# BharathMasetty/DPG-SLAM

Hardware: AMD Instinct MI355X
Metric: ICP edges/sec + ms/GN-iter on 5k-node/20k-edge synthetic graph, 1->8 GPU (higher is better)
Workload: dtype fp32 (ICP) + fp64 (GN)

## Files before the change

dpg-slam_amd/csrc/dpg_chol.hip:

```cpp
#include "dpg_chol_dev.h"

using namespace dpg_chol;

namespace {
void take_sym(CholDev* c, dpg_chol_sym* S) {
    c->has_factor = false;
    if (c->track && c->sym_is_fac) {
        std::swap(c->fac_sym, c->sym);
        c->fac_G.swap(c->plan.cur_G);
        c->sym_is_fac = false;
    }
    std::swap(c->sym, *S);
}

int chol_upload(CholDev* c) {
    const dpg_chol_sym& S = c->sym;
    const CholPlan& H = c->plan;
    const int64_t n = H.n;
    ++c->build_gen;
    c->has_factor = false;
    auto al = [](size_t b) { return (b + 255) & ~size_t(255); };
    struct Piece { void** d; const void* h; size_t bytes; };
    Piece pieces[24];
    int np = 0;
// ... 212 lines not shown
    int64_t* gat = reinterpret_cast<int64_t*>(c->pstage.p + keep_bytes);
    int64_t* sca = gat + 4 * nruns;
    for (int64_t r = 0, off = 0; r < nruns; ++r) {
        const int64_t* q = K.runs.data() + 4 * r;
        const int64_t g4[4] = {q[0], off, q[2], q[3]}, s4[4] = {off, q[1], q[2], q[3]};
        std::copy(g4, g4 + 4, gat + 4 * r);
        std::copy(s4, s4 + 4, sca + 4 * r);
        off += q[2];
    }
    if (c->pev.ensure(hipEventDisableTiming)) return DPG_ERR_HIP;
    if (hipMemcpyAsync(c->dpart.p, c->pstage.p, bytes, hipMemcpyHostToDevice, st) != hipSuccess ||
        hipEventRecord(c->pev.e, st) != hipSuccess)
        return DPG_ERR_HIP;
    c->pev_set = true;
    const uint8_t* keep_dev = reinterpret_cast<const uint8_t*>(c->dpart.p);
    const int64_t* gat_dev = reinterpret_cast<const int64_t*>(c->dpart.p + keep_bytes);
    launch_copy_runs(c, st, gat_dev, gat_dev + 4 * nruns, nruns, K.max_run);
    if (hipMemsetAsync(c->status.p, 0, sizeof(int32_t), st) != hipSuccess ||
        hipMemsetAsync(c->sync.p, 0, P.sync_bytes, st) != hipSuccess)
        return DPG_ERR_HIP;
    launch_factor(c, st, hb, nullptr, keep_dev);
    launch_backward(c, st, nullptr, nullptr, nullptr, nullptr, nullptr);
    note_factored(c, ns - K.kept, K.kept, K.moved, (int64_t)((now_ms() - t_pick) * 1e6));
    c->inv_valid = false;
    return hipGetLastError() == hipSuccess ? DPG_OK : DPG_ERR_HIP;
}

extern "C" int dpg_chol_resolve(void* h, const double* hb, void* stream) {
    CholDev* c = reinterpret_cast<CholDev*>(h);
    hipStream_t st = reinterpret_cast<hipStream_t>(stream);
    if (hipMemsetAsync(c->sync.p, 0, c->plan.sync_bytes, st) != hipSuccess) return DPG_ERR_HIP;
    const double* di = c->plan.use_dinv ? c->dinv.p : nullptr;
    const double* li = c->inv_valid ? c->linv.p : nullptr;
    launch_forward(c, st, hb, di, nullptr, li);
    launch_backward(c, st, di, nullptr, nullptr, nullptr, li);
    return hipGetLastError() == hipSuccess ? DPG_OK : DPG_ERR_HIP;
}

extern "C" int dpg_chol_gated_ok(void* h) {
    const CholDev* c = reinterpret_cast<const CholDev*>(h);
    return c && c->plan.fused && !(c->plan.use_dinv && c->plan.n_dblocks > 0) ? 1 : 0;
}

extern "C" void dpg_chol_sync_dev(void* h, int32_t** sync, int64_t* n_words) {
    CholDev* c = reinterpret_cast<CholDev*>(h);
    *sync = c->sync.p;
    *n_words = (int64_t)(c->plan.sync_bytes / sizeof(int32_t));
}

extern "C" int dpg_chol_solve_gated(void* h, const double* hb, const int32_t* gate, int prezeroed, double* X,
                                    double* max_out, void* stream) {
    CholDev* c = reinterpret_cast<CholDev*>(h);
    if (!dpg_chol_gated_ok(h)) return DPG_ERR_STATE;
    c->fac_valid = false;
    c->has_factor = true;
    hipStream_t st = reinterpret_cast<hipStream_t>(stream);
    if (!prezeroed && (hipMemsetAsync(c->status.p, 0, sizeof(int32_t), st) != hipSuccess ||
                       hipMemsetAsync(c->sync.p, 0, c->plan.sync_bytes, st) != hipSuccess))
        return DPG_ERR_HIP;
    const bool inv = c->plan.n_inv_tasks > 0;
    if (inv) {
        if (!c->aux.s) {
            if (hipStreamCreateWithFlags(&c->aux.s, hipStreamNonBlocking) != hipSuccess ||
                c->ev_fac.ensure(hipEventDisableTiming) || c->ev_inv[0].ensure(hipEventDisableTiming) ||
                c->ev_inv[1].ensure(hipEventDisableTiming) || hipEventRecord(c->ev_inv[0].e, c->aux.s) != hipSuccess ||
                hipEventRecord(c->ev_inv[1].e, c->aux.s) != hipSuccess)
                return DPG_ERR_HIP;
        }
        if (hipStreamWaitEvent(st, c->ev_inv[c->inv_par ^ 1].e, 0) != hipSuccess) return DPG_ERR_HIP;
    }
    launch_factor(c, st, hb, gate, nullptr);
    if (inv) {
        if (hipEventRecord(c->ev_fac.e, st) != hipSuccess || hipStreamWaitEvent(c->aux.s, c->ev_fac.e, 0) != hipSuccess)
            return DPG_ERR_HIP;
        launch_inv(c, c->aux.s, gate);
        if (hipEventRecord(c->ev_inv[c->inv_par].e, c->aux.s) != hipSuccess) return DPG_ERR_HIP;
        c->inv_par ^= 1;
    }
    launch_forward(c, st, hb, nullptr, gate, c->linv.p);
    launch_backward(c, st, nullptr, gate, X, max_out, c->linv.p);
    return hipGetLastError() == hipSuccess ? DPG_OK : DPG_ERR_HIP;
}

extern "C" void dpg_chol_keep_inverse(void* h, int on) {
    if (h) reinterpret_cast<CholDev*>(h)->keep_inv = on != 0;
}

extern "C" int dpg_chol_join_aux(void* h, void* stream) {
    CholDev* c = reinterpret_cast<CholDev*>(h);
    if (!c || !c->aux.s) return DPG_OK;
    return hipStreamWaitEvent(reinterpret_cast<hipStream_t>(stream), c->ev_inv[c->inv_par ^ 1].e, 0) == hipSuccess ? DPG_OK
                                                                                                       : DPG_ERR_HIP;
}

extern "C" const int32_t* dpg_chol_pos_dev(void* h) { return reinterpret_cast<CholDev*>(h)->pos; }
extern "C" const double* dpg_chol_x_dev(void* h) { return reinterpret_cast<CholDev*>(h)->xsol.p; }
extern "C" const int32_t* dpg_chol_status_dev(void* h) { return reinterpret_cast<CholDev*>(h)->status.p; }
extern "C" void dpg_chol_stats(void* h, double out[6]) {
    const dpg_chol_sym& S = reinterpret_cast<CholDev*>(h)->sym;
    out[0] = S.ns;
    out[1] = S.n_levels;
    out[2] = S.max_front;
    out[3] = S.flops;
    out[4] = (double)S.front_off[(size_t)S.ns] * 8.0;
    out[5] = (double)S.n;
}

#ifdef DPG_CHOL_TIMING
extern "C" void dpg_chol_tree(void* h, int32_t* parent, int32_t* m3, int32_t* k3) {
    const dpg_chol_sym& S = reinterpret_cast<CholDev*>(h)->sym;
    for (int32_t s = 0; s < S.ns; ++s) {
        parent[s] = S.sn_parent[(size_t)s];
        k3[s] = 3 * (S.sn_c0[(size_t)s + 1] - S.sn_c0[(size_t)s]);
        m3[s] = k3[s] + 3 * (int32_t)(S.sn_rows_ptr[(size_t)s + 1] - S.sn_rows_ptr[(size_t)s]);
    }
}
#endif
```

dpg-slam_amd/csrc/dpg_ctx.h:

```cpp
#ifndef DPG_CTX_H
#define DPG_CTX_H

#include <hip/hip_runtime.h>
#include <rccl/rccl.h>
#include <string.h>
#include <time.h>

#include <algorithm>
#include <atomic>
#include <condition_variable>
#include <deque>
#include <memory>
#include <mutex>
#include <thread>
#include <unordered_map>
#include <utility>
#include <vector>

#include "../../include/dpg_slam_c.h"
#include "dpg_buf.h"
#include "dpg_chol.h"
#include "dpg_gn_pipe.h"
#include "dpg_internal.h"

// ... 6 lines not shown
        hipError_t _e = (expr);                                                              \
        if (_e != hipSuccess) return fail(DPG_ERR_HIP, "%s: %s", #expr, hipGetErrorString(_e)); \
    } while (0)

inline double now_ms() {
    struct timespec ts;
    clock_gettime(CLOCK_MONOTONIC, &ts);
    return (double)ts.tv_sec * 1e3 + (double)ts.tv_nsec * 1e-6;
}

template <typename T>
T or_default(const T* p, void (*def)(T*)) {
    T v;
    if (p) v = *p;
    else def(&v);
    return v;
}

struct DevMem {
    typedef hipStream_t stream_t;
    static int alloc(void** p, size_t bytes) { return hipMalloc(p, bytes) != hipSuccess; }
    static void free(void* p) { (void)hipFree(p); }
    static int copy(void* dst, const void* src, size_t bytes, hipStream_t s) {
        return hipMemcpyAsync(dst, src, bytes, hipMemcpyDeviceToDevice, s) != hipSuccess ||
               hipStreamSynchronize(s) != hipSuccess;
    }
};
struct PinMem {
    typedef hipStream_t stream_t;
    static int alloc(void** p, size_t bytes) { return hipHostMalloc(p, bytes, hipHostMallocDefault) != hipSuccess; }
    static void free(void* p) { (void)hipHostFree(p); }
    static int copy(void* dst, const void* src, size_t bytes, hipStream_t) {
        memcpy(dst, src, bytes);
        return 0;
    }
};
struct MappedMem : PinMem {
    static int alloc(void** p, size_t bytes) { return hipHostMalloc(p, bytes, hipHostMallocMapped | hipHostMallocCoherent) != hipSuccess; }
};
template <typename T>
using DevBuf = OwnedBuf<T, DevMem>;
template <typename T>
using PinBuf = OwnedBuf<T, PinMem>;
template <typename T>
using MappedBuf = OwnedBuf<T, MappedMem>;

struct DevEvent {
    hipEvent_t e = nullptr;
    DevEvent() = default;
    DevEvent(const DevEvent&) = delete;
    DevEvent& operator=(const DevEvent&) = delete;
    DevEvent(DevEvent&& o) noexcept : e(o.e) { o.e = nullptr; }
    DevEvent& operator=(DevEvent&& o) noexcept {
        std::swap(e, o.e);
        return *this;
    }
    ~DevEvent() {
        if (e) (void)hipEventDestroy(e);
    }
    int ensure(unsigned flags) { return e || hipEventCreateWithFlags(&e, flags) == hipSuccess ? 0 : -1; }
};
struct DevStream {
    hipStream_t s = nullptr;
    DevStream() = default;
    DevStream(const DevStream&) = delete;
    DevStream& operator=(const DevStream&) = delete;
    ~DevStream() { release(); }
    void release() {
        if (s) (void)hipStreamDestroy(s);
        s = nullptr;
    }
};
struct CholDestroy { void operator()(void* h) const { dpg_chol_destroy(h); } };
typedef std::unique_ptr<void, CholDestroy> CholPtr;

struct GnGraph {
    dpg_gn_dev v{};
    DevBuf<dpg_factor> factors;
    DevBuf<int32_t> up_cptr, up_clist, rowptr, colidx, src_up;
    DevBuf<double> bsr, minv, poses, x, r, z, p0, p1, q, partials, scal, hb_own, scal3;
    PinBuf<double> scal3_host;
    DevBuf<uint8_t> mine;
    DevBuf<double> hb_part;
    CholPtr chol;
    int build(int64_t n_nodes, const dpg_factor* factors, int64_t n_factors, int64_t shard_begin, int64_t shard_end,
              const dpg_chol_opts* opts, hipStream_t sync_stream);
};

struct dpg_ctx {
    int device = 0;
    DevStream own;
    hipStream_t stream = nullptr;
    DevStream aux;
    DevEvent ev[8];
    bool cov_pending = false, cov_on_aux = false;
    int32_t icp_variant = DPG_ICP_ANGULAR;
    int32_t defer_cap = 256;
    int32_t cov_wg = 256;
    int32_t kernel_variant = 0;
    float map_ms = 0.f;
    DevEvent map_ev[2];
    DevBuf<float> full, ds;
    DevBuf<int64_t> ds_off_dev;
    DevBuf<int64_t> full_off_dev;
    DevBuf<float> tree_pts;
    DevBuf<uint16_t> tree_idx;
    DevBuf<uint16_t> buckets;
    DevBuf<unsigned char> icp_scratch;
    std::vector<int64_t> full_off, ds_off;
    int64_t n_nodes = 0;
    int64_t idx_valid = 0;
    int32_t ratio = 1;
    int32_t max_ds = 0;
    std::vector<dpg_icp_edge> h_edges;
    DevBuf<dpg_icp_edge> edges;
    DevBuf<dpg_icp_result> res;
    DevBuf<double> hess;
    DevBuf<int32_t> trace;
    int64_t n_edges = 0;
    int32_t max_src = 0, max_tgt = 0;
    int32_t trace_iters = 0;
    dpg_icp_kparams kp{};
    bool have_cov = false;
    DevBuf<float> s_pts;
    DevBuf<dpg_icp_edge> s_edge;
    DevBuf<dpg_icp_result> s_res;
    DevBuf<double> s_hess;
    DevBuf<int64_t> s_off;
    DevBuf<float> s_tree_pts;
    DevBuf<uint16_t> s_tree_idx;
    DevBuf<uint16_t> s_buckets;
    GnGraph gn;
    bool gn_ready = false;
    dpg_gn_params gp{};
    float asm_ms = 0.f, solve_ms = 0.f;
    std::vector<uint64_t> gn_pairs;
    bool gn_pairs_valid = false;
    DevBuf<dpg_gn_ctl> pipe_ctl;
    MappedBuf<dpg_gn_slot> pipe_slot;
    uint32_t pipe_loop = 0;
    std::vector<dpg_ctx*> peers;
    std::vector<std::pair<void*, void (*)(void*)>> children;
    std::vector<ncclComm_t> comms;
    dpg_coll_ops host_ops{};
    std::vector<double> host_hb;
    struct HostColl;
    std::unique_ptr<HostColl> hc;
    int32_t coll = 0;
    int32_t world = 1, rank0 = 0;
    int32_t rank = 0;
    std::vector<dpg_icp_edge> batch;
    std::vector<int32_t> batch_owner;
    std::vector<std::vector<int64_t>> shard;
    bool batch_measured = false;
    int32_t batch_runs = 0;
    int32_t schedule = DPG_ICP_SCHEDULE_MEASURED;
    std::unordered_map<uint64_t, float> cost;
    DevBuf<int32_t> shard_idx;
    DevBuf<float> cost_dev;
    dpg_chol_opts copts;
    DevBuf<dpg_csm_pair> csm_pairs;
    DevBuf<float> csm_rot;
    DevBuf<int32_t> csm_stencil;
    DevBuf<dpg_csm_result> csm_res;
    DevBuf<int32_t> csm_diag;
    DevEvent csm_ev[2];
    bool csm_timed = false;
};

struct dpg_ctx::HostColl {
    PinBuf<double> buf;
    MappedBuf<uint32_t> flag;
    DevEvent ev[2];
    uint32_t next_tag = 0;
    std::thread th;
    std::mutex mu;
    std::condition_variable cv;
    std::deque<std::pair<uint32_t, hipEvent_t>> jobs;
    size_t count = 0;
    uint64_t posted = 0, done = 0;
    bool stop = false;
    std::atomic<int> failed{0};
    static int create(const dpg_ctx* c, std::unique_ptr<HostColl>& out);
    ~HostColl();
};

enum { kCollNone = 0, kCollRccl = 1, kCollVirtual = 2, kCollHost = 3, kMaxVirtual = 16 };
inline int n_dev(const dpg_ctx* c) { return 1 + (int)c->peers.size(); }
inline bool is_rank_form(const dpg_ctx* c) {
    return (c->coll == kCollRccl || c->coll == kCollHost) && c->peers.empty() && c->world > 1;
}
inline dpg_ctx* dev_ctx(dpg_ctx* c, int k) { return k == 0 ? c : c->peers[(size_t)k - 1]; }
inline bool is_multi(const dpg_ctx* c) { return c->coll != kCollNone; }
inline int join_cov(dpg_ctx* c) {
    if (!c->cov_pending) return DPG_OK;
    c->cov_pending = false;
    return hipStreamWaitEvent(c->stream, c->ev[2].e, 0) == hipSuccess ? DPG_OK : DPG_ERR_HIP;
}

extern dpg_ctx* g_default_ctx;
void scans_truncate(dpg_ctx* c, int64_t V);
int icp_batch_run_from(dpg_ctx* c, int64_t tree_from);
int batch_fetch(dpg_ctx* c, dpg_icp_result* results, double* hess, bool learn);
int gn_loop(dpg_ctx* c, const dpg_gn_params& P, double* poses, double t0, double t1, dpg_gn_stats* st);

#pragma GCC visibility pop

#endif
```

dpg-slam_amd/csrc/dpg_ctx.hip:

```cpp

#include <stdarg.h>
#include <stdio.h>
#include <string.h>

#include <string>

#include "dpg_ctx.h"

namespace {
thread_local std::string g_err;
}

int fail(int code, const char* fmt, ...) {
    char buf[512];
    va_list ap;
    va_start(ap, fmt);
    vsnprintf(buf, sizeof(buf), fmt, ap);
    va_end(ap);
    g_err = buf;
    return code;
}

dpg_ctx* g_default_ctx = nullptr;

// ... 203 lines not shown
    if (!c || !o || o->order < DPG_ORDER_AUTO || o->order > DPG_ORDER_ND || o->max_supernode_cols < 1 || o->solve_inv_cols < 0 ||
        !(o->relax_fraction >= 0.0))
        return fail(DPG_ERR_ARG, "bad solver options");
    for (int k = 0; k < n_dev(c); ++k) {
        dpg_chol_opts& d = dev_ctx(c, k)->copts;
        d.order = o->order;
        d.fused = o->fused ? 1 : 0;
        d.solve_stage = o->solve_stage;
        d.solve_maxseg = o->solve_maxseg;
        d.solve_dinv = o->solve_dinv ? 1 : 0;
        d.merge_single = o->merge_single ? 1 : 0;
        d.max_supernode_cols = o->max_supernode_cols;
        d.relax_fraction = o->relax_fraction;
        d.solve_inv_cols = o->solve_inv_cols;
    }
    return DPG_OK;
}

int dpg_ctx_set_icp_schedule(dpg_ctx* c, int32_t schedule) {
    if (!c || (schedule != DPG_ICP_SCHEDULE_CALLER && schedule != DPG_ICP_SCHEDULE_MEASURED))
        return fail(DPG_ERR_ARG, "bad ICP schedule");
    c->schedule = schedule;
    return DPG_OK;
}

int dpg_ctx_set_icp_variant(dpg_ctx* c, int32_t variant) {
    if (!c || (variant != DPG_ICP_ANGULAR && variant != DPG_ICP_KDTREE && variant != DPG_ICP_GRID))
        return fail(DPG_ERR_ARG, "bad ICP variant");
    for (int k = 0; k < n_dev(c); ++k) {
        if (dev_ctx(c, k)->icp_variant != variant) dev_ctx(c, k)->idx_valid = 0;
        dev_ctx(c, k)->icp_variant = variant;
    }
    return DPG_OK;
}

int dpg_ctx_set_icp_defer_cap(dpg_ctx* c, int32_t cap) {
    if (!c || cap < 0) return fail(DPG_ERR_ARG, "bad defer cap");
    for (int k = 0; k < n_dev(c); ++k) dev_ctx(c, k)->defer_cap = cap;
    return DPG_OK;
}

int dpg_ctx_set_cov_workgroups(dpg_ctx* c, int32_t n) {
    if (!c || n < 0) return fail(DPG_ERR_ARG, "bad covariance workgroup count");
    for (int k = 0; k < n_dev(c); ++k) dev_ctx(c, k)->cov_wg = n;
    return DPG_OK;
}

int dpg_ctx_set_icp_kernel_variant(dpg_ctx* c, int32_t v) {
    if (!c || v < 0) return fail(DPG_ERR_ARG, "bad kernel variant");
    for (int k = 0; k < n_dev(c); ++k) {
        if ((dev_ctx(c, k)->kernel_variant == 2) != (v == 2)) dev_ctx(c, k)->idx_valid = 0;
        dev_ctx(c, k)->kernel_variant = v;
    }
    return DPG_OK;
}

void dpg_ctx_adopt(dpg_ctx* c, void* child, void (*destroy)(void*)) {
    if (c && child) c->children.emplace_back(child, destroy);
}
void dpg_ctx_release_child(dpg_ctx* c, void* child) {
    if (!c) return;
    for (size_t k = 0; k < c->children.size(); ++k)
        if (c->children[k].first == child) {
            c->children.erase(c->children.begin() + (std::ptrdiff_t)k);
            return;
        }
}

void dpg_ctx_destroy(dpg_ctx* c) {
    if (!c) return;
    while (!c->children.empty()) {
        const auto ch = c->children.back();
        ch.second(ch.first);
        if (!c->children.empty() && c->children.back().first == ch.first) c->children.pop_back();
    }
    if (c->coll == kCollVirtual) (void)hipStreamSynchronize(c->stream);
    for (dpg_ctx* q : c->peers) dpg_ctx_destroy(q);
    c->peers.clear();
    for (ncclComm_t m : c->comms)
        if (m) (void)ncclCommDestroy(m);
    c->comms.clear();
    (void)hipSetDevice(c->device);
    (void)join_cov(c);
    (void)hipStreamSynchronize(c->stream);
    c->hc.reset();
    if (c == g_default_ctx) g_default_ctx = nullptr;
    delete c;
}

int dpg_ctx_set_stream(dpg_ctx* c, void* s) {
    if (!c) return fail(DPG_ERR_ARG, "ctx is NULL");
    if (join_cov(c)) return fail(DPG_ERR_HIP, "stream wait failed");
    HIP_TRY(hipStreamSynchronize(c->stream));
    c->own.release();
    c->stream = reinterpret_cast<hipStream_t>(s);
    if (c->coll == kCollVirtual)
        for (dpg_ctx* q : c->peers) q->stream = c->stream;
    return DPG_OK;
}

int dpg_ctx_synchronize(dpg_ctx* c) {
    if (!c) return fail(DPG_ERR_ARG, "ctx is NULL");
    for (int k = 0; k < n_dev(c); ++k) {
        HIP_TRY(hipSetDevice(dev_ctx(c, k)->device));
        if (join_cov(dev_ctx(c, k))) return fail(DPG_ERR_HIP, "stream wait failed");
        HIP_TRY(hipStreamSynchronize(dev_ctx(c, k)->stream));
    }
    HIP_TRY(hipSetDevice(c->device));
    return DPG_OK;
}

}
```

dpg-slam_amd/csrc/dpg_gn.hip:

```cpp

#include <hip/hip_runtime.h>
#include <math.h>
#include <stdint.h>
#include <stdlib.h>
#include <string.h>

#include <algorithm>
#include <future>
#include <vector>

#include "dpg_ctx.h"

namespace {

constexpr int kRowThreads = 256;

__device__ __forceinline__ void between_lin(const double* a, const double* b, double h[4], double H1[9]) {
    const double c1 = cos(a[2]), s1 = sin(a[2]), c2 = cos(b[2]), s2 = sin(b[2]);
    const double c = c1 * c2 + s1 * s2, s = -s1 * c2 + c1 * s2;
    const double dx = b[0] - a[0], dy = b[1] - a[1];
    h[0] = c1 * dx + s1 * dy;
    h[1] = -s1 * dx + c1 * dy;
    h[2] = c;
    h[3] = s;
// ... 279 lines not shown
            const double* B = bsr + 9 * (int64_t)s;
            acc[0] += B[0] * pc[0] + B[1] * pc[1] + B[2] * pc[2];
            acc[1] += B[3] * pc[0] + B[4] * pc[1] + B[5] * pc[2];
            acc[2] += B[6] * pc[0] + B[7] * pc[1] + B[8] * pc[2];
        }
#pragma unroll
        for (int k = 0; k < 3; ++k) {
            const double pv = it > 0 ? z[3 * v + k] + beta * p_old[3 * v + k] : p_old[3 * v + k];
            p_new[3 * v + k] = pv;
            q[3 * v + k] = acc[k];
            pq += pv * acc[k];
        }
    }
    pq = block_sum(pq, red);
    if (threadIdx.x == 0) part_pq[blockIdx.x] = pq;
}

__global__ void pcg_update_kernel(int it, int64_t n, const double* __restrict__ minv,
                                  const double* __restrict__ p, const double* __restrict__ q,
                                  double* __restrict__ x, double* __restrict__ r, double* __restrict__ z,
                                  const double* __restrict__ part_rz_in, const double* __restrict__ part_pq,
                                  double* __restrict__ part_rz_out, double* __restrict__ part_rr, int nb) {
    __shared__ double red[16];
    const double rz = sum_partials(part_rz_in, nb);
    const double pq = sum_partials(part_pq, nb);
    const double alpha = pq != 0.0 ? rz / pq : 0.0;
    const int64_t v = (int64_t)blockIdx.x * blockDim.x + threadIdx.x;
    double rz_n = 0.0, rr = 0.0;
    if (v < n) {
        double rv[3], zv[3];
#pragma unroll
        for (int k = 0; k < 3; ++k) {
            x[3 * v + k] += alpha * p[3 * v + k];
            rv[k] = r[3 * v + k] - alpha * q[3 * v + k];
            r[3 * v + k] = rv[k];
        }
        mv3(minv + 9 * v, rv, zv);
#pragma unroll
        for (int k = 0; k < 3; ++k) {
            z[3 * v + k] = zv[k];
            rz_n += rv[k] * zv[k];
            rr += rv[k] * rv[k];
        }
    }
    rz_n = block_sum(rz_n, red);
    rr = block_sum(rr, red);
    if (threadIdx.x == 0) { part_rz_out[blockIdx.x] = rz_n; part_rr[blockIdx.x] = rr; }
}

__global__ void retract_kernel(double* __restrict__ X, const double* __restrict__ d, int64_t n,
                               const int32_t* __restrict__ pos, double* __restrict__ max_out, const int32_t* gate) {
    if (gate && !gate[0]) return;
    const int64_t v = (int64_t)blockIdx.x * blockDim.x + threadIdx.x;
    double m = 0.0;
    if (v < n) {
        const int64_t di = 3 * (int64_t)(pos ? pos[v] : v);
        m = pose_retract(X + 3 * v, d[di], d[di + 1], d[di + 2]);
    }
#pragma unroll
    for (int off = 32; off >= 1; off >>= 1) m = fmax(m, __shfl_down(m, off, 64));
    if ((threadIdx.x & 63) == 0)
        atomicMax(reinterpret_cast<unsigned long long*>(max_out), (unsigned long long)__double_as_longlong(m));
}

__global__ void scalars_kernel(const double* __restrict__ chi2, const int32_t* __restrict__ status,
                               double* __restrict__ scal3) {
    scal3[1] = *chi2;
    scal3[2] = status ? (double)*status : 0.0;
}

__device__ __forceinline__ void icp_factor_write(dpg_factor& f, const dpg_icp_result& r, int64_t e, int64_t n_always,
                                                 double ix, double iy, double ith) {
    const bool keep = e < n_always || (r.converged && r.status == DPG_ICP_OK);
    f.z[0] = r.z[0];
    f.z[1] = r.z[1];
    f.z[2] = r.z[2];
    f.info[0] = keep ? ix : 0.0;
    f.info[1] = keep ? iy : 0.0;
    f.info[2] = keep ? ith : 0.0;
}

__global__ void icp_to_factor_kernel(const dpg_icp_result* __restrict__ res, dpg_factor* __restrict__ F,
                                     int64_t first, int64_t count, int64_t n_always, double ix, double iy,
                                     double ith) {
    const int64_t e = (int64_t)blockIdx.x * blockDim.x + threadIdx.x;
    if (e >= count) return;
    dpg_factor& f = F[first + e];
    const dpg_icp_result r = res[e];
    icp_factor_write(f, r, e, n_always, ix, iy, ith);
}

template <typename B, typename T>
int take(B& b, T*& view, size_t n) {
    const int rc = b.reserve(n);
    view = b.p;
    return rc;
}

template <typename T>
int up(T* dst, const std::vector<T>& src) {
    if (src.empty()) return 0;
    return hipMemcpy(dst, src.data(), src.size() * sizeof(T), hipMemcpyHostToDevice) == hipSuccess ? 0 : DPG_ERR_HIP;
}

inline unsigned nblk(int64_t n) { return (unsigned)((n + kRowThreads - 1) / kRowThreads); }

}

extern "C" int64_t dpg_gn_dev_vote_offset(const dpg_gn_dev* g) { return 9 * g->nnzb_upper + 3 * g->n_nodes + 2; }
extern "C" int64_t dpg_gn_dev_hb_size(const dpg_gn_dev* g) { return dpg_gn_dev_vote_offset(g) + g->n_vote; }

int GnGraph::build(int64_t n, const dpg_factor* F, int64_t nf, int64_t shard_begin, int64_t shard_end,
                   const dpg_chol_opts* opts, hipStream_t sync_stream) {
    dpg_gn_dev* g = &v;
    if (n <= 0 || nf < 0 || n > (int64_t)1 << 28) return DPG_ERR_ARG;
    const double t0 = now_ms();
    std::vector<uint64_t> fkey((size_t)nf, ~0ull);
    std::vector<uint64_t> pk;
    pk.reserve((size_t)nf);
    for (int64_t k = 0; k < nf; ++k) {
        const dpg_factor& f = F[k];
        if (f.kind == DPG_FACTOR_PRIOR) {
            if (f.i < 0 || f.i >= n) return DPG_ERR_ARG;
            continue;
        }
        if (f.kind != DPG_FACTOR_BETWEEN || f.i < 0 || f.j < 0 || f.i >= n || f.j >= n || f.i == f.j)
            return DPG_ERR_ARG;
        fkey[(size_t)k] = (uint64_t)std::min(f.i, f.j) << 32 | (uint64_t)std::max(f.i, f.j);
        pk.push_back(fkey[(size_t)k]);
    }
    const size_t n_between = pk.size();
    std::sort(pk.begin(), pk.end());
    pk.erase(std::unique(pk.begin(), pk.end()), pk.end());
    const int64_t P = (int64_t)pk.size();
    const int64_t nu = n + P;
    std::vector<int32_t> plo((size_t)P), phi((size_t)P);
    for (int64_t p = 0; p < P; ++p) { plo[(size_t)p] = (int32_t)(pk[(size_t)p] >> 32); phi[(size_t)p] = (int32_t)(pk[(size_t)p] & 0xffffffffu); }
    const dpg_chol_opts copt = opts ? *opts : dpg_chol_opts{};
    double sym_ms = 0.0;
    std::future<void*> sym_job = std::async(std::launch::async, [&]() -> void* {
        const double ts = now_ms();
        void* ch = nullptr;
        dpg_chol_opts o = copt;
        dpg_chol_sym S;
        if (dpg_chol_symbolic(n, plo.data(), phi.data(), P, &o, &S) ||
            dpg_chol_create_sym_plan(&ch, n, plo.data(), phi.data(), P, &S, &o))
            ch = nullptr;
        sym_ms = now_ms() - ts;
        return ch;
    });
    std::vector<int32_t> fpair((size_t)nf, -1);
    for (int64_t k = 0; k < nf; ++k)
        if (fkey[(size_t)k] != ~0ull)
            fpair[(size_t)k] = (int32_t)(std::lower_bound(pk.begin(), pk.end(), fkey[(size_t)k]) - pk.begin());
    std::vector<int32_t> cptr((size_t)nu + 1), clist((size_t)nf + 2 * n_between);
    dpg_contribution_lists(F, nf, n, fpair.data(), P, cptr.data(), clist.data());
    std::vector<int32_t> rowptr((size_t)n + 1, 0);
    for (int64_t v = 0; v < n; ++v) rowptr[(size_t)v + 1] = 1;
    for (uint64_t key : pk) { rowptr[(size_t)(key >> 32) + 1]++; rowptr[(size_t)(key & 0xffffffffu) + 1]++; }
    for (int64_t v = 0; v < n; ++v) rowptr[(size_t)v + 1] += rowptr[(size_t)v];
    std::vector<int32_t> colidx((size_t)rowptr[(size_t)n]), srcup((size_t)rowptr[(size_t)n]);
    {
        std::vector<int32_t> at(rowptr.begin(), rowptr.end() - 1);
        for (int64_t p = 0; p < P; ++p) {
            const int32_t lo = (int32_t)(pk[(size_t)p] >> 32), hi = (int32_t)(pk[(size_t)p] & 0xffffffffu);
            colidx[(size_t)at[(size_t)hi]] = lo;
            srcup[(size_t)at[(size_t)hi]++] = (int32_t)(-1 - (n + p));
        }
        for (int64_t v = 0; v < n; ++v) {
            colidx[(size_t)at[(size_t)v]] = (int32_t)v;
            srcup[(size_t)at[(size_t)v]++] = (int32_t)v;
        }
        for (int64_t p = 0; p < P; ++p) {
            const int32_t lo = (int32_t)(pk[(size_t)p] >> 32), hi = (int32_t)(pk[(size_t)p] & 0xffffffffu);
            colidx[(size_t)at[(size_t)lo]] = hi;
            srcup[(size_t)at[(size_t)lo]++] = (int32_t)(n + p);
        }
    }
    const double t1 = now_ms();
    CholPtr ch(sym_job.get());
    const double t2 = now_ms();
    if (sync_stream && hipStreamSynchronize(sync_stream) != hipSuccess) return DPG_ERR_HIP;
    g->n_nodes = n;
    g->n_factors = nf;
    g->nnzb_upper = nu;
    g->nnzb_full = (int64_t)colidx.size();
    g->shard_begin = shard_begin < 0 ? 0 : shard_begin;
    g->shard_end = shard_end > nf ? nf : shard_end;
    g->n_blocks_rows = (int32_t)nblk(n);
    int rc = 0;
    rc |= take(factors, g->factors, std::max<size_t>((size_t)nf, 1));
    rc |= take(up_cptr, g->up_cptr, cptr.size());
    rc |= take(up_clist, g->up_clist, std::max<size_t>(clist.size(), 1));
    rc |= take(this->rowptr, g->rowptr, rowptr.size());
    rc |= take(this->colidx, g->colidx, colidx.size());
    rc |= take(src_up, g->src_up, srcup.size());
    rc |= take(bsr, g->bsr, 9 * colidx.size());
    rc |= take(minv, g->minv, 9 * (size_t)n);
    rc |= take(poses, g->poses, 3 * (size_t)n);
    rc |= take(x, g->x, 3 * (size_t)n);
    rc |= take(r, g->r, 3 * (size_t)n);
    rc |= take(z, g->z, 3 * (size_t)n);
    rc |= take(p0, g->p0, 3 * (size_t)n);
    rc |= take(p1, g->p1, 3 * (size_t)n);
    rc |= take(q, g->q, 3 * (size_t)n);
    rc |= take(partials, g->partials, 6 * (size_t)g->n_blocks_rows + (size_t)n);
    rc |= take(scal, g->scal, 2 * (size_t)65536);
    rc |= take(hb_own, g->hb_own, (size_t)dpg_gn_dev_hb_size(g));
    rc |= take(scal3, g->scal3, 4);
    rc |= take(scal3_host, g->scal3_host, 4);
    if (!rc && nf && hipMemcpy(g->factors, F, (size_t)nf * sizeof(dpg_factor), hipMemcpyHostToDevice) != hipSuccess) rc = -1;
    if (!rc)
        rc = up(g->up_cptr, cptr) | up(g->up_clist, clist) | up(g->rowptr, rowptr) | up(g->colidx, colidx) |
             up(g->src_up, srcup);
    if (rc) { *this = GnGraph(); return DPG_ERR_HIP; }
    g->chol = ch.release();
    if (g->chol && dpg_chol_create_sym_upload(&g->chol)) g->chol = nullptr;
    chol.reset(g->chol);
    if (g->chol) dpg_chol_keep_inverse(g->chol, 1);
    const double t3 = now_ms();
    double bt[2] = {0.0, 0.0};
    if (g->chol) dpg_chol_build_times(g->chol, bt);
    g->setup_ms[0] = t1 - t0;
    g->setup_ms[1] = std::max(0.0, sym_ms - bt[0]);
    g->setup_ms[2] = bt[0];
    g->setup_ms[3] = std::max(0.0, (t3 - t2) - bt[1]);
    g->setup_ms[4] = bt[1];
    return DPG_OK;
}

extern "C" int dpg_gn_dev_icp_to_factors(dpg_gn_dev* g, const dpg_icp_result* res, int64_t first, int64_t count,
                                         int64_t n_always, double ix, double iy, double ith, void* stream) {
    if (count <= 0) return DPG_OK;
    if (first < 0 || first + count > g->n_factors) return DPG_ERR_ARG;
    hipLaunchKernelGGL(icp_to_factor_kernel, dim3(nblk(count)), dim3(kRowThreads), 0,
                       reinterpret_cast<hipStream_t>(stream), res, g->factors, first, count, n_always, ix, iy, ith);
    return hipGetLastError() == hipSuccess ? DPG_OK : DPG_ERR_HIP;
}

static int assemble_gated(dpg_gn_dev* g, double* hb, hipStream_t s, const int32_t* gate, bool chi2 = true) {
    double* chi2_node = g->partials + 6 * (size_t)g->n_blocks_rows;
    const int64_t ng = lg_groups(g->n_nodes, g->nnzb_upper);
    if (ng > 0)
        hipLaunchKernelGGL(lin_gather_kernel, dim3((unsigned)ng), dim3(kLgLanes), 0, s, g->factors, g->poses, g->up_cptr,
                           g->up_clist, g->n_nodes, g->nnzb_upper, g->shard_begin, g->shard_end, g->mine, hb, chi2_node, gate);
    if (chi2) {
        const bool vote = hb == g->hb_part && g->n_vote > 0;
        hipLaunchKernelGGL(chi2_kernel, dim3(1), dim3(1024), 0, s, chi2_node, g->n_nodes,
                           hb + 9 * g->nnzb_upper + 3 * g->n_nodes, gate, vote ? hb + dpg_gn_dev_vote_offset(g) : nullptr,
                           g->scal3, vote && g->chol ? dpg_chol_status_dev(g->chol) : nullptr, g->world, g->rank);
    }
    return hipGetLastError() == hipSuccess ? DPG_OK : DPG_ERR_HIP;
}

extern "C" int dpg_gn_dev_assemble(dpg_gn_dev* g, double* hb, void* stream) {
    return assemble_gated(g, hb, reinterpret_cast<hipStream_t>(stream), nullptr);
}

__global__ void own_kernel(uint8_t* __restrict__ mine, int64_t nf, int32_t world, int32_t rank) {
    const int64_t f = (int64_t)blockIdx.x * blockDim.x + threadIdx.x;
    if (f < nf) mine[f] = (f % world) == rank ? 1 : 0;
}

__global__ void icp_to_factor_scatter_kernel(const dpg_icp_result* __restrict__ res, const int32_t* __restrict__ idx,
                                             dpg_factor* __restrict__ F, uint8_t* __restrict__ mine, int64_t first,
                                             int64_t n_local, int64_t n_always, double ix, double iy, double ith) {
    const int64_t j = (int64_t)blockIdx.x * blockDim.x + threadIdx.x;
    if (j >= n_local) return;
    const int64_t e = idx[j];
    dpg_factor& f = F[first + e];
    const dpg_icp_result r = res[j];
    icp_factor_write(f, r, e, n_always, ix, iy, ith);
    mine[first + e] = 1;
}

struct VsumArgs {
    const double* parts[16];
    double* outs[16];
};
__global__ void vsum_kernel(VsumArgs a, int32_t k, int64_t n) {
    for (int64_t i = (int64_t)blockIdx.x * blockDim.x + threadIdx.x; i < n; i += (int64_t)gridDim.x * blockDim.x) {
        double s = a.parts[0][i];
        for (int32_t q = 1; q < k; ++q) s += a.parts[q][i];
        for (int32_t q = 0; q < k; ++q) a.outs[q][i] = s;
    }
}

extern "C" int dpg_gn_dev_set_ownership(GnGraph* o, int32_t world, int32_t rank, void* stream) {
    if (world < 1 || rank < 0 || rank >= world) return DPG_ERR_ARG;
    dpg_gn_dev* g = &o->v;
    hipStream_t s = reinterpret_cast<hipStream_t>(stream);
    const int32_t nv = world > 1 ? 2 * world : 0;
    if (nv != g->n_vote) {
        if (hipStreamSynchronize(s) != hipSuccess) return DPG_ERR_HIP;
        o->hb_own.release();
        o->hb_part.release();
        g->hb_part = nullptr;
        g->n_vote = nv;
        if (take(o->hb_own, g->hb_own, (size_t)dpg_gn_dev_hb_size(g))) return DPG_ERR_HIP;
    }
    if (!o->mine.p && take(o->mine, g->mine, std::max<size_t>((size_t)g->n_factors, 1))) return DPG_ERR_HIP;
    if (!o->hb_part.p && take(o->hb_part, g->hb_part, (size_t)dpg_gn_dev_hb_size(g))) return DPG_ERR_HIP;
    if (hipMemsetAsync(g->hb_part, 0, sizeof(double) * (size_t)dpg_gn_dev_hb_size(g), s) != hipSuccess) return DPG_ERR_HIP;
    g->world = world;
    g->rank = rank;
    if (g->n_factors > 0)
        hipLaunchKernelGGL(own_kernel, dim3(nblk(g->n_factors)), dim3(kRowThreads), 0, reinterpret_cast<hipStream_t>(stream),
                           g->mine, g->n_factors, world, rank);
    return hipGetLastError() == hipSuccess ? DPG_OK : DPG_ERR_HIP;
}

extern "C" int dpg_gn_dev_icp_to_factors_scatter(dpg_gn_dev* g, const dpg_icp_result* res, const int32_t* idx,
                                                 int64_t n_local, int64_t first, int64_t count, int64_t n_always,
                                                 double ix, double iy, double ith, void* stream) {
    if (!g->mine || first < 0 || count < n_local || first + count > g->n_factors) return DPG_ERR_ARG;
    hipStream_t s = reinterpret_cast<hipStream_t>(stream);
    if (count > 0 && hipMemsetAsync(g->mine + first, 0, (size_t)count, s) != hipSuccess) return DPG_ERR_HIP;
    if (n_local > 0)
        hipLaunchKernelGGL(icp_to_factor_scatter_kernel, dim3(nblk(n_local)), dim3(kRowThreads), 0, s, res, idx, g->factors,
                           g->mine, first, n_local, n_always, ix, iy, ith);
    return hipGetLastError() == hipSuccess ? DPG_OK : DPG_ERR_HIP;
}

extern "C" int dpg_gn_dev_assemble_part(dpg_gn_dev* g, const int32_t* gate, void* stream) {
    if (!g->hb_part) return DPG_ERR_STATE;
    return assemble_gated(g, g->hb_part, reinterpret_cast<hipStream_t>(stream), gate, true);
}

extern "C" int dpg_launch_vsum(const double* const* parts, double* const* outs, int32_t k, int64_t n, void* stream) {
    if (k < 1 || k > 16 || n <= 0) return k >= 1 && k <= 16 ? DPG_OK : DPG_ERR_ARG;
    VsumArgs a;
    for (int q = 0; q < 16; ++q) {
        a.parts[q] = q < k ? parts[q] : nullptr;
        a.outs[q] = q < k ? outs[q] : nullptr;
    }
    const unsigned blocks = (unsigned)std::min<int64_t>((n + 1023) / 1024, 2048);
    hipLaunchKernelGGL(vsum_kernel, dim3(blocks), dim3(1024), 0, reinterpret_cast<hipStream_t>(stream), a, k, n);
    return hipGetLastError() == hipSuccess ? DPG_OK : DPG_ERR_HIP;
}

static int pcg_solve(dpg_gn_dev* g, const double* hb, const dpg_gn_params* gp, hipStream_t s);

extern "C" int dpg_gn_dev_solve_async(dpg_gn_dev* g, const double* hb, const dpg_gn_params* gp, void* stream) {
    hipStream_t s = reinterpret_cast<hipStream_t>(stream);
    const double* xout = g->x;
    const int32_t* xpos = nullptr;
    g->last_pcg_iters = 0;
    g->last_used_chol = gp->linear_solver == DPG_SOLVER_CHOLESKY && g->chol;
    if (g->last_used_chol) {
        const bool slow = g->last_was_chord && g->last_delta_inf > 0.1 * g->prev_delta_inf;
        const bool reuse = gp->reuse_factorization && g->have_factor && g->last_delta_inf < gp->refactor_delta && !slow;
        g->last_was_chord = reuse ? 1 : 0;
        const int rc = reuse ? dpg_chol_resolve(g->chol, hb, stream) : dpg_chol_solve(g->chol, hb, stream);
        if (rc) return rc;
        if (!reuse) {
            g->have_factor = 1;
            ++g->n_factorizations;
        }
        xout = dpg_chol_x_dev(g->chol);
        xpos = dpg_chol_pos_dev(g->chol);
    } else {
        const int it = pcg_solve(g, hb, gp, s);
        if (it < 0) return DPG_ERR_HIP;
        g->last_pcg_iters = it;
    }
    if (hipMemsetAsync(g->scal3, 0, sizeof(double), s) != hipSuccess) return DPG_ERR_HIP;
    hipLaunchKernelGGL(retract_kernel, dim3(g->n_blocks_rows), dim3(kRowThreads), 0, s, g->poses, xout, g->n_nodes,
                       xpos, g->scal3, nullptr);
    return hipGetLastError() == hipSuccess ? DPG_OK : DPG_ERR_HIP;
}

__device__ __forceinline__ void clear_sync(int32_t* sync, int64_t n_words, int32_t* status) {
    int4* s4 = reinterpret_cast<int4*>(sync);
    for (int64_t k = threadIdx.x; k < n_words / 4; k += blockDim.x) s4[k] = make_int4(0, 0, 0, 0);
    if (threadIdx.x == 0) *status = 0;
}

__device__ __forceinline__ void sys_st64(void* p, uint64_t v) {
    __hip_atomic_store(reinterpret_cast<uint64_t*>(p), v, __ATOMIC_RELAXED, __HIP_MEMORY_SCOPE_SYSTEM);
}
static_assert(offsetof(dpg_gn_slot, reuse) == 24 && offsetof(dpg_gn_slot, active) == 28 &&
              offsetof(dpg_gn_slot, final_) == 32 && offsetof(dpg_gn_slot, it) == 36 && offsetof(dpg_gn_slot, tag) == 40,
              "post_slot stores the int pairs as 8-byte words");
__device__ __forceinline__ void post_slot(dpg_gn_slot* slot, const dpg_gn_slot& o, uint64_t tag) {
    sys_st64(&slot->dinf, (uint64_t)__double_as_longlong(o.dinf));
    sys_st64(&slot->error, (uint64_t)__double_as_longlong(o.error));
    sys_st64(&slot->status, (uint64_t)__double_as_longlong(o.status));
    sys_st64(&slot->reuse, (uint64_t)(uint32_t)o.reuse | (uint64_t)(uint32_t)o.active << 32);
    sys_st64(&slot->final_, (uint64_t)(uint32_t)o.final_ | (uint64_t)(uint32_t)o.it << 32);
    asm volatile("s_waitcnt vmcnt(0)" ::: "memory");
    sys_st64(&slot->tag, tag);
}

__global__ void pipe_init_kernel(dpg_gn_ctl* ctl, int32_t reuse, int32_t last_was_chord, int32_t have_factor,
                                 double last_dinf, double prev_dinf, const double* cur_dev, dpg_gn_slot* init,
                                 double* max_out, int32_t* sync, int64_t n_words, int32_t* status, uint32_t loop) {
    clear_sync(sync, n_words, status);
    if (threadIdx.x != 0) return;
    const double cur = *cur_dev;
    {
        dpg_gn_slot o{};
        o.error = cur;
        post_slot(init, o, (uint64_t)loop << 32);
    }
    ctl->loop = loop;
    ctl->active = !(cur <= 0.0) ? 1 : 0;
    ctl->reuse = reuse;
    ctl->last_was_chord = last_was_chord;
    ctl->have_factor = have_factor;
    ctl->it = 0;
    ctl->last_dinf = last_dinf;
    ctl->prev_dinf = prev_dinf;
    ctl->cur_error = cur;
    *max_out = 0.0;
}

__global__ __launch_bounds__(1024) void pipe_ctl_kernel(dpg_gn_ctl* ctl, const double* __restrict__ chi2_node, int64_t n,
                                                        double* chi2, const double* chi2_sum, int32_t* status,
                                                        double* max_out, dpg_gn_params P, dpg_gn_slot* slot,
                                                        int32_t* sync, int64_t n_words, const double* __restrict__ vote,
                                                        int32_t world) {
    __shared__ double red[16];
    if (!ctl->active) return;
    double sum = 0.0;
    if (chi2_sum) {
        sum = *chi2_sum;
    } else {
        sum = block_sum(strided_sum(chi2_node, n, threadIdx.x, blockDim.x), red);
    }
    const double st_word = (double)*status;
    __syncthreads();
    clear_sync(sync, n_words, status);
    if (threadIdx.x != 0) return;
    *chi2 = sum;
    dpg_gn_slot o;
    o.reuse = ctl->reuse;
    o.active = ctl->active;
    o.it = ctl->it;
    o.final_ = 1;
    o.dinf = 0.0;
    o.error = 0.0;
    o.status = 0.0;
    if (ctl->active) {
        double dinf = *max_out, st = st_word;
        if (vote) {
            const unsigned long long d0 = (unsigned long long)__double_as_longlong(vote[0]);
            bool diverged = false;
            dinf = vote[0];
            st = vote[world];
            for (int32_t r = 1; r < world; ++r) {
                diverged |= (unsigned long long)__double_as_longlong(vote[r]) != d0;
                dinf = fmax(dinf, vote[r]);
                st = fmax(st, vote[world + r]);
            }
            if (diverged) st = (double)DPG_GN_STATUS_DIVERGED;
        }
        const double nw = sum;
        const int it = ctl->it + 1;
        o.dinf = dinf;
        o.error = nw;
        o.status = st;
        o.it = it;
        bool fin = st != 0.0 || it >= P.max_iterations;
        if (!fin) {
            const double cur = ctl->cur_error;
            if (P.use_error_criteria) {
                bool conv = nw <= 0.0;
                if (!conv) {
                    const double abs_dec = cur - nw, rel_dec = abs_dec / cur;
                    conv = (P.relative_error_tol != 0.0 && rel_dec <= P.relative_error_tol) ||
                           abs_dec <= P.absolute_error_tol;
                }
                fin = conv || !isfinite(cur);
            } else {
                fin = dinf < P.delta_tol;
            }
        }
        o.final_ = fin ? 1 : 0;
        ctl->prev_dinf = ctl->last_dinf;
        ctl->last_dinf = dinf;
        ctl->last_was_chord = ctl->reuse;
        ctl->have_factor = 1;
        ctl->cur_error = nw;
        ctl->it = it;
        const bool slow = ctl->last_was_chord && ctl->last_dinf > 0.1 * ctl->prev_dinf;
        ctl->reuse = (P.reuse_factorization && ctl->have_factor && ctl->last_dinf < P.refactor_delta && !slow) ? 1 : 0;
        ctl->active = fin ? 0 : 1;
        *max_out = 0.0;
    }
    post_slot(slot, o, ((uint64_t)ctl->loop << 32) | (uint32_t)o.it);
}

extern "C" int dpg_gn_pipe_init(dpg_gn_dev* g, const dpg_gn_params* gp, dpg_gn_ctl* ctl, const double* cur_dev,
                                dpg_gn_slot* init, uint32_t loop, void* stream) {
    hipStream_t s = reinterpret_cast<hipStream_t>(stream);
    const bool slow = g->last_was_chord && g->last_delta_inf > 0.1 * g->prev_delta_inf;
    const bool reuse = gp->reuse_factorization && g->have_factor && g->last_delta_inf < gp->refactor_delta && !slow;
    int32_t* sync;
    int64_t n_words;
    dpg_chol_sync_dev(g->chol, &sync, &n_words);
    hipLaunchKernelGGL(pipe_init_kernel, dim3(1), dim3(1024), 0, s, ctl, reuse ? 1 : 0, g->last_was_chord, g->have_factor,
                       g->last_delta_inf, g->prev_delta_inf, cur_dev, init, g->scal3, sync, n_words,
                       const_cast<int32_t*>(dpg_chol_status_dev(g->chol)), loop);
    return hipGetLastError() == hipSuccess ? DPG_OK : DPG_ERR_HIP;
}

extern "C" int dpg_gn_pipe_issue_solve(dpg_gn_dev* g, dpg_gn_ctl* ctl, int part, void* stream) {
    hipStream_t s = reinterpret_cast<hipStream_t>(stream);
    const int32_t* gate = &ctl->active;
    if (!g->chol || !dpg_chol_gated_ok(g->chol) || (part && !g->hb_part)) return DPG_ERR_STATE;
    int rc = dpg_chol_solve_gated(g->chol, g->hb_own, gate, 1, g->poses, g->scal3, stream);
    if (rc) return rc;
    return part ? assemble_gated(g, g->hb_part, s, gate, true) : assemble_gated(g, g->hb_own, s, gate, false);
}

extern "C" int dpg_gn_pipe_issue_ctl(dpg_gn_dev* g, const dpg_gn_params* gp, dpg_gn_ctl* ctl, dpg_gn_slot* slot,
                                     int part, void* stream) {
    hipStream_t s = reinterpret_cast<hipStream_t>(stream);
    int32_t* sync;
    int64_t n_words;
    if (dpg_chol_join_aux(g->chol, stream)) return DPG_ERR_HIP;
    dpg_chol_sync_dev(g->chol, &sync, &n_words);
    double* chi2 = g->hb_own + 9 * g->nnzb_upper + 3 * g->n_nodes;
    hipLaunchKernelGGL(pipe_ctl_kernel, dim3(1), dim3(1024), 0, s, ctl, g->partials + 6 * (size_t)g->n_blocks_rows,
                       g->n_nodes, chi2, part ? chi2 : nullptr, const_cast<int32_t*>(dpg_chol_status_dev(g->chol)),
                       g->scal3, *gp, slot, sync, n_words,
                       part && g->n_vote > 0 ? g->hb_own + dpg_gn_dev_vote_offset(g) : nullptr, g->world);
    return hipGetLastError() == hipSuccess ? DPG_OK : DPG_ERR_HIP;
}

extern "C" int dpg_gn_pipe_issue(dpg_gn_dev* g, const dpg_gn_params* gp, dpg_gn_ctl* ctl, dpg_gn_slot* slot,
                                 void* stream) {
    const int rc = dpg_gn_pipe_issue_solve(g, ctl, 0, stream);
    return rc ? rc : dpg_gn_pipe_issue_ctl(g, gp, ctl, slot, 0, stream);
}

extern "C" int dpg_gn_dev_fetch(dpg_gn_dev* g, const double* hb, void* stream, double out[3]) {
    hipStream_t s = reinterpret_cast<hipStream_t>(stream);
    const bool chol = g->chol != nullptr && g->last_used_chol;
    hipLaunchKernelGGL(scalars_kernel, dim3(1), dim3(1), 0, s, hb + 9 * g->nnzb_upper + 3 * g->n_nodes,
                       chol ? dpg_chol_status_dev(g->chol) : nullptr, g->scal3);
    if (hipMemcpyAsync(g->scal3_host, g->scal3, 3 * sizeof(double), hipMemcpyDeviceToHost, s) != hipSuccess ||
        hipStreamSynchronize(s) != hipSuccess)
        return DPG_ERR_HIP;
    out[0] = g->scal3_host[0];
    out[1] = g->scal3_host[1];
    out[2] = g->scal3_host[2];
    g->prev_delta_inf = g->last_delta_inf;
    g->last_delta_inf = out[0];
    return DPG_OK;
}

extern "C" int dpg_gn_dev_solve(dpg_gn_dev* g, const double* hb, const dpg_gn_params* gp, void* stream,
                                double* delta_inf, double* error, int32_t* pcg_iters) {
    int rc = dpg_gn_dev_solve_async(g, hb, gp, stream);
    if (rc) return rc;
    double sc[3];
    if ((rc = dpg_gn_dev_fetch(g, hb, stream, sc))) return rc;
    if (gp->linear_solver == DPG_SOLVER_CHOLESKY && g->chol && sc[2] != 0.0) return DPG_ERR_NUMERIC;
    if (delta_inf) *delta_inf = sc[0];
    if (error) *error = sc[1];
    if (pcg_iters) *pcg_iters = g->last_pcg_iters;
    return DPG_OK;
}

static int pcg_solve(dpg_gn_dev* g, const double* hb, const dpg_gn_params* gp, hipStream_t s) {
    const int nb = g->n_blocks_rows;
    const int64_t n = g->n_nodes;
    double* part_rz_a = g->partials;
    double* part_rz_b = g->partials + nb;
    double* part_rr = g->partials + 2 * (size_t)nb;
    double* part_pq = g->partials + 3 * (size_t)nb;
    hipLaunchKernelGGL(pcg_init_kernel, dim3(nb), dim3(kRowThreads), 0, s, hb, g->rowptr, g->src_up, n, g->nnzb_upper,
                       g->bsr, g->minv, g->x, g->r, g->z, g->p0, part_rz_a, part_rr);
    double host_scal[2] = {0, 0};
    double rr0 = -1.0;
    const int check = gp->pcg_check_every > 0 ? gp->pcg_check_every : 16;
    const int max_it = std::min(gp->pcg_max_iterations > 0 ? gp->pcg_max_iterations : 20000, 65535);
    const double tol2 = gp->pcg_rel_tol * gp->pcg_rel_tol;
    int it = 0;
    double* pbuf[2] = {g->p0, g->p1};
    double* rzbuf[2] = {part_rz_a, part_rz_b};
    for (; it < max_it; ++it) {
        double* p_old = pbuf[it & 1];
        double* p_new = pbuf[(it + 1) & 1];
        hipLaunchKernelGGL(pcg_spmv_kernel, dim3(nb), dim3(kRowThreads), 0, s, it, g->bsr, g->rowptr, g->colidx, n,
// ... 33 lines not shown
```

dpg-slam_amd/csrc/dpg_gn_api.hip:

```cpp

#include <string.h>

#include <chrono>
#include <cmath>

#include "dpg_ctx.h"

static int gn_setup_1(dpg_ctx* c, int64_t V, const dpg_factor* F, int64_t nf, int64_t b, int64_t e,
                      const dpg_gn_params* gp) {
    HIP_TRY(hipSetDevice(c->device));
    GnGraph ng;
    int rc = ng.build(V, F, nf, b, e, &c->copts, c->stream);
    if (rc) return fail(rc, "pose-graph setup failed (invalid factor or out of memory)");
    c->gn = std::move(ng);
    c->gn_ready = true;
    c->gn_pairs_valid = false;
    c->gp = or_default(gp, dpg_gn_params_default);
    return DPG_OK;
}

static int gn_set_poses_1(dpg_ctx* c, const double* poses) {
    if (!c->gn_ready) return fail(DPG_ERR_STATE, "graph not set up");
    HIP_TRY(hipSetDevice(c->device));
    HIP_TRY(hipMemcpyAsync(c->gn.v.poses, poses, sizeof(double) * 3 * (size_t)c->gn.v.n_nodes, hipMemcpyHostToDevice,
                           c->stream));
    HIP_TRY(hipStreamSynchronize(c->stream));
    c->gn.v.have_factor = 0;
    c->gn.v.last_delta_inf = 1e300;
    c->gn.v.prev_delta_inf = 1e300;
    c->gn.v.last_was_chord = 0;
    c->gn.v.n_factorizations = 0;
    return DPG_OK;
}

#define DPG_STEP_API_1(c)                                                                                        \
    do {                                                                                                         \
        if (!(c) || !(c)->gn_ready) return fail(DPG_ERR_STATE, "graph not set up");                             \
        if (is_multi(c)) return fail(DPG_ERR_STATE, "the step API is per device: a multi-device context runs "   \
                                                    "dpg_gn_run / dpg_optimize_graph / dpg_reoptimize");         \
    } while (0)

static int solve_retract_async_1(dpg_ctx* c, const double* hb_dev) {
    if (!hb_dev) hb_dev = c->gn.v.hb_own;
    HIP_TRY(hipEventRecord(c->ev[4].e, c->stream));
    int rc = dpg_gn_dev_solve_async(&c->gn.v, hb_dev, &c->gp, c->stream);
    if (rc) return fail(rc, "solve launch failed: %s", hipGetErrorString(hipGetLastError()));
    HIP_TRY(hipEventRecord(c->ev[5].e, c->stream));
    return DPG_OK;
}

static int fetch_1(dpg_ctx* c, const double* hb_dev, double out[3]) {
    if (!hb_dev) hb_dev = c->gn.v.hb_own;
    int rc = dpg_gn_dev_fetch(&c->gn.v, hb_dev, c->stream, out);
    if (rc) return fail(rc, "fetch failed");
    float s = 0.f;
    if (hipEventElapsedTime(&s, c->ev[4].e, c->ev[5].e) == hipSuccess) c->solve_ms = s;
    return DPG_OK;
}

static int read_error(dpg_ctx* c, double* err) {
    HIP_TRY(hipSetDevice(c->device));
    HIP_TRY(hipMemcpyAsync(err, c->gn.v.hb_own + 9 * c->gn.v.nnzb_upper + 3 * c->gn.v.n_nodes, sizeof(double),
                           hipMemcpyDeviceToHost, c->stream));
    HIP_TRY(hipStreamSynchronize(c->stream));
    return DPG_OK;
}

static int check_conv(const dpg_gn_params* gp, double cur, double nw) {
    if (nw <= 0.0) return 1;
    const double abs_dec = cur - nw;
    const double rel_dec = abs_dec / cur;
    return (gp->relative_error_tol != 0.0 && rel_dec <= gp->relative_error_tol) || (abs_dec <= gp->absolute_error_tol);
}

static int coll_sum_hb(dpg_ctx* c) {
    const size_t count = (size_t)dpg_gn_dev_hb_size(&c->gn.v);
    if (c->coll == kCollVirtual) {
        const double* parts[kMaxVirtual];
        double* outs[kMaxVirtual];
        for (int k = 0; k < n_dev(c); ++k) {
            parts[k] = dev_ctx(c, k)->gn.v.hb_part;
            outs[k] = dev_ctx(c, k)->gn.v.hb_own;
        }
        const int rc = dpg_launch_vsum(parts, outs, n_dev(c), (int64_t)count, c->stream);
        return rc ? fail(rc, "virtual all-reduce launch failed") : DPG_OK;
    }
    if (c->coll == kCollHost) {
        c->host_hb.resize(count);
        HIP_TRY(hipSetDevice(c->device));
        HIP_TRY(hipMemcpyAsync(c->host_hb.data(), c->gn.v.hb_part, sizeof(double) * count, hipMemcpyDeviceToHost, c->stream));
        HIP_TRY(hipStreamSynchronize(c->stream));
        if (c->host_ops.allreduce_sum_f64(c->host_ops.user, c->host_hb.data(), (int64_t)count))
            return fail(DPG_ERR_HIP, "the caller's all-reduce of the packed system failed");
        HIP_TRY(hipMemcpyAsync(c->gn.v.hb_own, c->host_hb.data(), sizeof(double) * count, hipMemcpyHostToDevice, c->stream));
        HIP_TRY(hipStreamSynchronize(c->stream));
        return DPG_OK;
    }
    if (ncclGroupStart() != ncclSuccess) return fail(DPG_ERR_HIP, "ncclGroupStart failed");
    for (int k = 0; k < n_dev(c); ++k) {
        dpg_ctx* q = dev_ctx(c, k);
        const ncclResult_t r = ncclAllReduce(q->gn.v.hb_part, q->gn.v.hb_own, count, ncclDouble, ncclSum, c->comms[(size_t)k],
                                             q->stream);
        if (r != ncclSuccess) {
            (void)ncclGroupEnd();
            return fail(DPG_ERR_HIP, "ncclAllReduce failed: %s", ncclGetErrorString(r));
        }
    }
    if (ncclGroupEnd() != ncclSuccess) return fail(DPG_ERR_HIP, "ncclGroupEnd failed");
    return DPG_OK;
}

static void host_coll_thread(dpg_ctx::HostColl* hp, int device, dpg_coll_ops ops) {
    dpg_ctx::HostColl& h = *hp;
    (void)hipSetDevice(device);
    for (;;) {
        std::pair<uint32_t, hipEvent_t> job;
        {
            std::unique_lock<std::mutex> lk(h.mu);
            h.cv.wait(lk, [&] { return h.stop || !h.jobs.empty(); });
            if (h.jobs.empty()) return;
            job = h.jobs.front();
            h.jobs.pop_front();
// ... 13 lines not shown

int dpg_ctx::HostColl::create(const dpg_ctx* c, std::unique_ptr<HostColl>& out) {
    std::unique_ptr<HostColl> h(new HostColl());
    if (h->flag.reserve(2) || h->ev[0].ensure(hipEventDisableTiming) || h->ev[1].ensure(hipEventDisableTiming))
        return fail(DPG_ERR_HIP, "the collective thread's flag words and events could not be created");
    h->flag.p[0] = h->flag.p[1] = 0;
    h->th = std::thread(host_coll_thread, h.get(), c->device, c->host_ops);
    out = std::move(h);
    return DPG_OK;
}

dpg_ctx::HostColl::~HostColl() {
    {
        std::lock_guard<std::mutex> lk(mu);
        stop = true;
    }
    cv.notify_all();
    if (th.joinable()) th.join();
}

static int coll_sum_hb_host_async(dpg_ctx* c) {
    const size_t count = (size_t)dpg_gn_dev_hb_size(&c->gn.v);
    HIP_TRY(hipSetDevice(c->device));
    int rc;
    if (!c->hc && (rc = dpg_ctx::HostColl::create(c, c->hc))) return rc;
    dpg_ctx::HostColl& h = *c->hc;
    if (h.buf.cap < count && h.buf.reserve(count)) return fail(DPG_ERR_HIP, "hipHostMalloc(collective buffer) failed");
    h.count = count;
    const uint32_t tag = ++h.next_tag;
    hipEvent_t ev = h.ev[tag & 1].e;
    HIP_TRY(hipMemcpyAsync(h.buf.p, c->gn.v.hb_part, sizeof(double) * count, hipMemcpyDeviceToHost, c->stream));
    HIP_TRY(hipEventRecord(ev, c->stream));
    {
        std::lock_guard<std::mutex> lk(h.mu);
        h.jobs.emplace_back(tag, ev);
        ++h.posted;
    }
    h.cv.notify_all();
    rc = dpg_launch_host_wait(h.flag.p, tag, h.flag.p + 1, c->stream);
    if (rc) return fail(rc, "host-collective wait launch failed");
    HIP_TRY(hipMemcpyAsync(c->gn.v.hb_own, h.buf.p, sizeof(double) * count, hipMemcpyHostToDevice, c->stream));
    return DPG_OK;
}

static void hc_drain(dpg_ctx* c) {
    if (!c->hc) return;
    std::unique_lock<std::mutex> lk(c->hc->mu);
    c->hc->cv.wait(lk, [&] { return c->hc->done == c->hc->posted; });
}

static int ensure_pipe(dpg_ctx* q) {
    if (q->pipe_slot.p) return DPG_OK;
    HIP_TRY(hipSetDevice(q->device));
    if (q->pipe_ctl.reserve(1) || q->pipe_slot.reserve(3))
        return fail(DPG_ERR_HIP, "GN pipeline: allocating the control block and report slots failed");
    memset(q->pipe_slot.p, 0, 3 * sizeof(dpg_gn_slot));
    return DPG_OK;
}

static int wait_slot(dpg_ctx* q, const dpg_gn_slot* slot, uint64_t tag) {
    const volatile uint64_t* t = &slot->tag;
    auto t0 = std::chrono::steady_clock::now(), last = t0;
    for (unsigned n = 0;; ++n) {
        if (*t == tag) {
            std::atomic_thread_fence(std::memory_order_acquire);
            return DPG_OK;
        }
        if (n < 4096) {
            __builtin_ia32_pause();
            continue;
        }
        std::this_thread::yield();
        const auto now = std::chrono::steady_clock::now();
        if (now - last > std::chrono::milliseconds(2)) {
            last = now;
            const hipError_t e = hipStreamQuery(q->stream);
            if (e != hipSuccess && e != hipErrorNotReady) return fail(DPG_ERR_HIP, "GN pipeline: %s", hipGetErrorString(e));
            if (e == hipSuccess && *t != tag) return fail(DPG_ERR_STATE, "GN pipeline: the stream drained without the report");
            if (now - t0 > std::chrono::seconds(60)) return fail(DPG_ERR_HIP, "GN pipeline: no report after 60 s");
        }
    }
}

static int gn_loop_pipe_body(dpg_ctx* c, const dpg_gn_params& P, dpg_gn_stats& S, double& nw, double& dinf, int& it);
static int gn_loop_pipe(dpg_ctx* c, const dpg_gn_params& P, dpg_gn_stats& S, double& nw, double& dinf, int& it) {
    int rc = gn_loop_pipe_body(c, P, S, nw, dinf, it);
    if (c->coll == kCollHost && c->hc) {
        hc_drain(c);
        if (!rc && c->hc->failed.exchange(0)) rc = fail(DPG_ERR_HIP, "the caller's all-reduce of the packed system failed");
        if (!rc && __atomic_load_n(c->hc->flag.p + 1, __ATOMIC_ACQUIRE))
            rc = fail(DPG_ERR_HIP, "GN pipeline: no all-reduce from the collective thread in 120 s");
    }
    return rc;
}
static int gn_loop_pipe_body(dpg_ctx* c, const dpg_gn_params& P, dpg_gn_stats& S, double& nw, double& dinf, int& it) {
    const int L = n_dev(c);
    const int part = is_multi(c) ? 1 : 0;
    int rc;
    for (int k = 0; k < L; ++k) {
        dpg_ctx* q = dev_ctx(c, k);
        if ((rc = ensure_pipe(q))) return rc;
        ++q->pipe_loop;
        const double* cur_dev = q->gn.v.hb_own + 9 * q->gn.v.nnzb_upper + 3 * q->gn.v.n_nodes;
        if ((rc = dpg_gn_pipe_init(&q->gn.v, &P, q->pipe_ctl.p, cur_dev, q->pipe_slot.p + 2, q->pipe_loop, q->stream)))
            return fail(rc, "GN pipeline launch failed");
    }
    auto issue = [&](int i) -> int {
        int r;
        for (int k = 0; k < L; ++k) {
            dpg_ctx* q = dev_ctx(c, k);
            HIP_TRY(hipSetDevice(q->device));
            if ((r = dpg_gn_pipe_issue_solve(&q->gn.v, q->pipe_ctl.p, part, q->stream)))
                return fail(r, "GN pipeline launch failed: %s", hipGetErrorString(hipGetLastError()));
        }
        if (part && (r = (c->coll == kCollHost ? coll_sum_hb_host_async(c) : coll_sum_hb(c)))) return r;
        for (int k = 0; k < L; ++k) {
            dpg_ctx* q = dev_ctx(c, k);
            HIP_TRY(hipSetDevice(q->device));
            if ((r = dpg_gn_pipe_issue_ctl(&q->gn.v, &P, q->pipe_ctl.p, q->pipe_slot.p + (i & 1), part, q->stream)))
                return fail(r, "GN pipeline launch failed: %s", hipGetErrorString(hipGetLastError()));
        }
        return DPG_OK;
    };
    if ((rc = issue(1))) return rc;
    int issued = 1;
    std::vector<int> nfact((size_t)L, 0), reuse_last((size_t)L, 0);
    for (int k = 0; k < L; ++k) reuse_last[(size_t)k] = dev_ctx(c, k)->gn.v.last_was_chord;
    for (int i = 1;; ++i) {
        if (issued < P.max_iterations) {
            if ((rc = issue(i + 1))) return rc;
            ++issued;
        }
        dpg_gn_slot o0{};
        for (int k = 0; k < L; ++k) {
            dpg_ctx* q = dev_ctx(c, k);
            HIP_TRY(hipSetDevice(q->device));
            if (i == 1) {
                if ((rc = wait_slot(q, q->pipe_slot.p + 2, (uint64_t)q->pipe_loop << 32))) return rc;
                const double e0 = static_cast<const volatile dpg_gn_slot*>(q->pipe_slot.p + 2)->error;
                if (e0 <= 0.0) {
                    for (int j = 0; j < L; ++j) (void)hipStreamSynchronize(dev_ctx(c, j)->stream);
                    S.initial_error = e0;
                    nw = e0;
                    dinf = 0.0;
                    it = 0;
                    HIP_TRY(hipSetDevice(c->device));
                    return DPG_OK;
                }
            }
            if ((rc = wait_slot(q, q->pipe_slot.p + (i & 1), ((uint64_t)q->pipe_loop << 32) | (uint32_t)i))) return rc;
            dpg_gn_slot o;
            {
                const volatile dpg_gn_slot* v = q->pipe_slot.p + (i & 1);
                o.dinf = v->dinf;
                o.error = v->error;
                o.status = v->status;
                o.reuse = v->reuse;
                o.active = v->active;
                o.final_ = v->final_;
                o.it = v->it;
            }
            if (i == 1 && k == 0) S.initial_error = static_cast<const volatile dpg_gn_slot*>(q->pipe_slot.p + 2)->error;
            if (!o.active || o.it != i) return fail(DPG_ERR_STATE, "GN pipeline out of step (device %d, iteration %d)", k, i);
            if (k == 0) {
                o0 = o;
            } else if (memcmp(&o.dinf, &o0.dinf, sizeof(double)) || memcmp(&o.error, &o0.error, sizeof(double)) ||
                       o.status != o0.status || o.reuse != o0.reuse || o.final_ != o0.final_) {
                for (int j = 0; j < L; ++j) (void)hipStreamSynchronize(dev_ctx(c, j)->stream);
                return fail(DPG_ERR_INTERNAL, "devices diverged at GN iteration %d (device %d: |d| %.17g error %.17g, "
                            "device 0: %.17g %.17g)", i, k, o.dinf, o.error, o0.dinf, o0.error);
            }
            if (!o.reuse) ++nfact[(size_t)k];
            q->gn.v.prev_delta_inf = q->gn.v.last_delta_inf;
            q->gn.v.last_delta_inf = o.dinf;
            reuse_last[(size_t)k] = o.reuse;
        }
        if (c->hc && c->hc->failed.load()) {
            for (int j = 0; j < L; ++j) (void)hipStreamSynchronize(dev_ctx(c, j)->stream);
            return fail(DPG_ERR_HIP, "the caller's all-reduce of the packed system failed (GN iteration %d)", i);
        }
        if (o0.status != 0.0) {
            for (int j = 0; j < L; ++j) (void)hipStreamSynchronize(dev_ctx(c, j)->stream);
            if (o0.status == (double)DPG_GN_STATUS_DIVERGED)
                return fail(DPG_ERR_INTERNAL, "ranks diverged at GN iteration %d (different max |delta| in the vote words)", i);
            return fail(DPG_ERR_NUMERIC, "Cholesky failed (status %d)", (int)o0.status);
        }
        it = i;
        dinf = o0.dinf;
        nw = o0.error;
        if (o0.final_) break;
    }
    for (int k = 0; k < L; ++k) {
        dpg_gn_dev* g = &dev_ctx(c, k)->gn.v;
        g->last_was_chord = reuse_last[(size_t)k];
        g->have_factor = 1;
        g->n_factorizations += nfact[(size_t)k];
        g->last_used_chol = 1;
    }
    S.pcg_iterations = 0;
    HIP_TRY(hipSetDevice(c->device));
    return DPG_OK;
}

static bool pipe_ok(dpg_ctx* c, const dpg_gn_params& P) {
    if (P.linear_solver != DPG_SOLVER_CHOLESKY) return false;
    for (int k = 0; k < n_dev(c); ++k) {
        const dpg_gn_dev& g = dev_ctx(c, k)->gn.v;
        if (!g.chol || !dpg_chol_gated_ok(g.chol)) return false;
    }
    return true;
}

int gn_loop(dpg_ctx* c, const dpg_gn_params& P, double* poses, double t0, double t1, dpg_gn_stats* st) {
    dpg_gn_stats S;
    memset(&S, 0, sizeof(S));
    const int L = n_dev(c);
    const bool multi = is_multi(c);
    int rc;
    for (int k = 0; k < L; ++k) {
        dpg_ctx* q = dev_ctx(c, k);
        HIP_TRY(hipSetDevice(q->device));
        if (multi) rc = dpg_gn_dev_assemble_part(&q->gn.v, nullptr, q->stream);
        else rc = dpg_gn_dev_assemble(&q->gn.v, q->gn.v.hb_own, q->stream);
        if (rc) return fail(rc, "assembly launch failed");
    }
    if (multi && (rc = coll_sum_hb(c))) return rc;
    double cur = 0.0, nw = 0.0, dinf = 0.0;
    int it = 0;
    const bool pipe = pipe_ok(c, P) && P.max_iterations > 0;
    if (!pipe) {
        if ((rc = read_error(c, &S.initial_error))) return rc;
        cur = nw = S.initial_error;
    }
    if (pipe) {
        if ((rc = gn_loop_pipe(c, P, S, nw, dinf, it))) return rc;
    } else if (!(cur <= 0.0) && P.max_iterations > 0) {
        for (;;) {
            for (int k = 0; k < L; ++k) {
                dpg_ctx* q = dev_ctx(c, k);
                HIP_TRY(hipSetDevice(q->device));
                if ((rc = solve_retract_async_1(q, nullptr))) return rc;
                if (multi) rc = dpg_gn_dev_assemble_part(&q->gn.v, nullptr, q->stream);
                else rc = dpg_gn_dev_assemble(&q->gn.v, q->gn.v.hb_own, q->stream);
                if (rc) return fail(rc, "assembly launch failed");
            }
            if (multi && (rc = coll_sum_hb(c))) return rc;
            double sc0[3] = {0, 0, 0};
            for (int k = 0; k < L; ++k) {
                dpg_ctx* q = dev_ctx(c, k);
                double sc[3];
                HIP_TRY(hipSetDevice(q->device));
                if ((rc = fetch_1(q, nullptr, sc))) return rc;
                if (k == 0) memcpy(sc0, sc, sizeof(sc));
                else if (memcmp(sc, sc0, sizeof(sc)))
                    return fail(DPG_ERR_INTERNAL, "devices diverged at GN iteration %d (device %d)", it + 1, k);
            }
            if (multi && c->gn.v.n_vote > 0) {
                const int W = c->gn.v.world;
                std::vector<double> vw((size_t)(2 * W));
                HIP_TRY(hipSetDevice(c->device));
                HIP_TRY(hipMemcpyAsync(vw.data(), c->gn.v.hb_own + dpg_gn_dev_vote_offset(&c->gn.v), sizeof(double) * vw.size(),
                                       hipMemcpyDeviceToHost, c->stream));
                HIP_TRY(hipStreamSynchronize(c->stream));
                for (int r = 0; r < W; ++r) {
                    if (memcmp(&vw[(size_t)r], &vw[0], sizeof(double)))
                        return fail(DPG_ERR_INTERNAL, "ranks diverged at GN iteration %d (rank %d: |d| %.17g, rank 0: %.17g)",
                                    it + 1, r, vw[(size_t)r], vw[0]);
                    sc0[2] = std::max(sc0[2], vw[(size_t)(W + r)]);
                }
                sc0[0] = vw[0];
            }
            if (sc0[2] != 0.0) return fail(DPG_ERR_NUMERIC, "Cholesky failed (status %d)", (int)sc0[2]);
            S.pcg_iterations += c->gn.v.last_pcg_iters;
            ++it;
            dinf = sc0[0];
            nw = sc0[1];
            if (it >= P.max_iterations) break;
            if (P.use_error_criteria) {
                if (check_conv(&P, cur, nw) || !std::isfinite(cur)) break;
            } else if (dinf < P.delta_tol) {
                break;
            }
            cur = nw;
        }
    }
    if (multi && (rc = dpg_ctx_synchronize(c))) return rc;
    if (poses && (rc = dpg_gn_get_poses(c, poses))) return rc;
    if (!poses) {
        HIP_TRY(hipSetDevice(c->device));
        HIP_TRY(hipStreamSynchronize(c->stream));
    }
    const double t2 = now_ms();
    S.iterations = it;
    S.final_error = nw;
    S.last_delta_inf = dinf;
    S.ms_total = t2 - t0;
    S.ms_per_iteration = it ? (t2 - t1) / it : 0.0;
    if (st) *st = S;
    return DPG_OK;
}

static int gn_marginals_state(dpg_ctx* c, const char* fn) {
    if (!c || !c->gn_ready) return fail(DPG_ERR_STATE, "%s: graph not set up", fn);
    if (is_multi(c)) return fail(DPG_ERR_STATE, "%s: marginals are single-device (this context has several ranks)", fn);
    if (c->gp.linear_solver != DPG_SOLVER_CHOLESKY || !c->gn.v.chol)
        return fail(DPG_ERR_STATE, "%s: the graph has no Cholesky factorization (linear_solver)", fn);
    return DPG_OK;
}

static int gn_factor_at_current_poses(dpg_ctx* c, const char* fn, bool timed) {
    HIP_TRY(hipSetDevice(c->device));
    dpg_gn_dev* g = &c->gn.v;
    int rc;
    if (timed) HIP_TRY(hipEventRecord(c->ev[3].e, c->stream));
    if ((rc = dpg_gn_dev_assemble(g, g->hb_own, c->stream))) return fail(rc, "%s: assembly launch failed", fn);
    if (timed) HIP_TRY(hipEventRecord(c->ev[4].e, c->stream));
    if ((rc = dpg_chol_solve(g->chol, g->hb_own, c->stream))) return fail(rc, "%s: factorization launch failed", fn);
    if (timed) HIP_TRY(hipEventRecord(c->ev[5].e, c->stream));
    return DPG_OK;
}

static int gn_marginals_blocks(dpg_ctx* c, const char* fn, const int32_t* nodes, int64_t n, const int32_t* pairs,
                               int64_t n_pairs, double* out, double* ms) {
    int rc = gn_marginals_state(c, fn);
    if (rc) return rc;
    if (!out || n < 0 || n_pairs < 0) return fail(DPG_ERR_ARG, "%s: bad arguments", fn);
    if (dpg_chol_selinv_check(c->gn.v.chol, nodes, n, pairs, n_pairs))
        return fail(DPG_ERR_ARG, "%s: a node is out of range or a pair's block is outside the factor's pattern", fn);
    if ((rc = gn_factor_at_current_poses(c, fn, ms != nullptr))) return rc;
    rc = dpg_chol_marginals(c->gn.v.chol, nodes, n, pairs, n_pairs, out, c->stream);
    if (rc == DPG_ERR_NUMERIC) return fail(rc, "%s: H is not positive definite", fn);
    if (rc) return fail(rc, "%s: selected inversion failed", fn);
    if (ms) {
        float a = 0.f, f = 0.f;
        HIP_TRY(hipEventElapsedTime(&a, c->ev[3].e, c->ev[4].e));
        HIP_TRY(hipEventElapsedTime(&f, c->ev[4].e, c->ev[5].e));
        ms[0] = a;
        ms[1] = f;
    }
    return DPG_OK;
}

static int gn_pairs_share_factor(dpg_ctx* c, const int32_t* pairs, int64_t n) {
    const dpg_gn_dev& g = c->gn.v;
    if (!c->gn_pairs_valid) {
        HIP_TRY(hipSetDevice(c->device));
        std::vector<dpg_factor> F((size_t)g.n_factors);
        if (g.n_factors > 0) {
            HIP_TRY(hipMemcpyAsync(F.data(), g.factors, sizeof(dpg_factor) * F.size(), hipMemcpyDeviceToHost, c->stream));
            HIP_TRY(hipStreamSynchronize(c->stream));
        }
        c->gn_pairs.clear();
        for (const dpg_factor& f : F)
            if (f.kind == DPG_FACTOR_BETWEEN && f.i != f.j)
                c->gn_pairs.push_back((uint64_t)(uint32_t)std::min(f.i, f.j) << 32 | (uint32_t)std::max(f.i, f.j));
        std::sort(c->gn_pairs.begin(), c->gn_pairs.end());
        c->gn_pairs.erase(std::unique(c->gn_pairs.begin(), c->gn_pairs.end()), c->gn_pairs.end());
        c->gn_pairs_valid = true;
    }
    for (int64_t q = 0; q < n; ++q) {
        const int32_t i = pairs[2 * q], j = pairs[2 * q + 1];
        if (i < 0 || j < 0 || i >= g.n_nodes || j >= g.n_nodes)
            return fail(DPG_ERR_ARG, "dpg_gn_marginal_pairs: pair %lld has a node out of range", (long long)q);
        if (i != j && !std::binary_search(c->gn_pairs.begin(), c->gn_pairs.end(),
                                          (uint64_t)(uint32_t)std::min(i, j) << 32 | (uint32_t)std::max(i, j)))
            return fail(DPG_ERR_ARG, "dpg_gn_marginal_pairs: nodes %d and %d share no factor", i, j);
    }
    return DPG_OK;
}

static int gn_joint_blocks(dpg_ctx* c, const char* fn, int by_nodes, const int32_t* idx, int64_t n, double* out, float* ms) {
    int rc = gn_marginals_state(c, fn);
    if (rc) return rc;
    if (n < 0 || (n > 0 && (!idx || !out))) return fail(DPG_ERR_ARG, "%s: bad arguments", fn);
    for (int64_t q = 0, e = by_nodes ? n : 2 * n; q < e; ++q)
        if (idx[q] < 0 || idx[q] >= c->gn.v.n_nodes) return fail(DPG_ERR_ARG, "%s: node %d is out of range", fn, idx[q]);
    if (n == 0) return DPG_OK;
    if ((rc = gn_factor_at_current_poses(c, fn, false))) return rc;
    rc = dpg_chol_joint(c->gn.v.chol, by_nodes, idx, n, out, c->stream, ms);
    if (rc == DPG_ERR_NUMERIC) return fail(rc, "%s: H is not positive definite", fn);
    if (rc) return fail(rc, "%s: the path solve failed", fn);
    return DPG_OK;
}

extern "C" {

int dpg_gn_setup(dpg_ctx* c, int64_t V, const dpg_factor* F, int64_t nf, int64_t b, int64_t e,
                 const dpg_gn_params* gp) {
    if (!c || !F || V <= 0 || nf < 0) return fail(DPG_ERR_ARG, "dpg_gn_setup: bad arguments");
    if (!is_multi(c)) return gn_setup_1(c, V, F, nf, b, e, gp);
    if (b != 0 || e != nf) return fail(DPG_ERR_ARG, "dpg_gn_setup: a multi-device context shards the factors itself (0, n_factors)");
    for (int k = 0; k < n_dev(c); ++k) {
        dpg_ctx* q = dev_ctx(c, k);
        int rc = gn_setup_1(q, V, F, nf, 0, nf, gp);
// ... 8 lines not shown
int dpg_gn_take_icp_measurements(dpg_ctx* c, int64_t first, int64_t count, int64_t n_always,
                                 const dpg_icp_params* p) {
    if (!c || !c->gn_ready || !p) return fail(DPG_ERR_STATE, "graph not set up");
    const double ix = 1.0 / (double)p->laser_x_variance, iy = 1.0 / (double)p->laser_y_variance,
                 ith = 1.0 / (double)p->laser_theta_variance;
    if (!is_multi(c)) {
        if (count > c->n_edges) return fail(DPG_ERR_ARG, "only %lld ICP results available", (long long)c->n_edges);
        int rc = dpg_gn_dev_icp_to_factors(&c->gn.v, c->res.p, first, count, n_always, ix, iy, ith, c->stream);
        return rc ? fail(rc, "dpg_gn_take_icp_measurements failed") : DPG_OK;
    }
    if (count != (int64_t)c->batch.size())
        return fail(DPG_ERR_ARG, "a multi-device context takes the whole batch (%lld results), not %lld",
                    (long long)c->batch.size(), (long long)count);
    for (int k = 0; k < n_dev(c); ++k) {
        dpg_ctx* q = dev_ctx(c, k);
        HIP_TRY(hipSetDevice(q->device));
        if (!q->gn_ready || !q->gn.v.mine) return fail(DPG_ERR_STATE, "graph not set up on device %d", k);
        const int64_t nl = (int64_t)c->shard[(size_t)k].size();
        const int rc = dpg_gn_dev_icp_to_factors_scatter(&q->gn.v, q->res.p, q->shard_idx.p, nl, first, count, n_always,
                                                         ix, iy, ith, q->stream);
        if (rc) return fail(rc, "dpg_gn_take_icp_measurements failed");
    }
    HIP_TRY(hipSetDevice(c->device));
    return DPG_OK;
}

int64_t dpg_gn_hb_size(dpg_ctx* c) { return (c && c->gn_ready) ? dpg_gn_dev_hb_size(&c->gn.v) : -1; }

int dpg_gn_setup_profile(dpg_ctx* c, double out[5]) {
    if (!c || !c->gn_ready || !out) return fail(DPG_ERR_STATE, "graph not set up");
    for (int k = 0; k < 5; ++k) out[k] = c->gn.v.setup_ms[k];
    return DPG_OK;
}

int dpg_gn_set_poses(dpg_ctx* c, const double* poses) {
    if (!c || !c->gn_ready || !poses) return fail(DPG_ERR_STATE, "graph not set up");
    for (int k = 0; k < n_dev(c); ++k) {
        const int rc = gn_set_poses_1(dev_ctx(c, k), poses);
        if (rc) return rc;
    }
    HIP_TRY(hipSetDevice(c->device));
    return DPG_OK;
}

int dpg_gn_get_poses(dpg_ctx* c, double* poses) {
    if (!c || !c->gn_ready || !poses) return fail(DPG_ERR_STATE, "graph not set up");
    HIP_TRY(hipSetDevice(c->device));
    HIP_TRY(hipMemcpyAsync(poses, c->gn.v.poses, sizeof(double) * 3 * (size_t)c->gn.v.n_nodes, hipMemcpyDeviceToHost,
                           c->stream));
    HIP_TRY(hipStreamSynchronize(c->stream));
    return DPG_OK;
}

int dpg_gn_assemble(dpg_ctx* c, double* hb_dev) {
    DPG_STEP_API_1(c);
    if (!hb_dev) hb_dev = c->gn.v.hb_own;
    HIP_TRY(hipEventRecord(c->ev[3].e, c->stream));
    int rc = dpg_gn_dev_assemble(&c->gn.v, hb_dev, c->stream);
    if (rc) return fail(rc, "assembly launch failed");
    HIP_TRY(hipEventRecord(c->ev[4].e, c->stream));
    return DPG_OK;
}

int dpg_gn_solve_retract(dpg_ctx* c, const double* hb_dev, double* delta_inf, double* error, int32_t* pcg_iters) {
    DPG_STEP_API_1(c);
    if (!hb_dev) hb_dev = c->gn.v.hb_own;
    int rc = dpg_gn_dev_solve(&c->gn.v, hb_dev, &c->gp, c->stream, delta_inf, error, pcg_iters);
    if (rc) return fail(rc, "PCG solve failed: %s", hipGetErrorString(hipGetLastError()));
    HIP_TRY(hipEventRecord(c->ev[5].e, c->stream));
    float a = 0.f, s = 0.f;
    if (hipEventSynchronize(c->ev[5].e) == hipSuccess) {
        (void)hipEventElapsedTime(&a, c->ev[3].e, c->ev[4].e);
        (void)hipEventElapsedTime(&s, c->ev[4].e, c->ev[5].e);
    }
    c->asm_ms = a;
    c->solve_ms = s;
    return DPG_OK;
}

int dpg_gn_solve_retract_async(dpg_ctx* c, const double* hb_dev) {
    DPG_STEP_API_1(c);
    return solve_retract_async_1(c, hb_dev);
}

int32_t dpg_gn_factorizations(dpg_ctx* c) { return (c && c->gn_ready) ? c->gn.v.n_factorizations : -1; }

int dpg_gn_fetch(dpg_ctx* c, const double* hb_dev, double out[3]) {
    DPG_STEP_API_1(c);
    if (!out) return fail(DPG_ERR_ARG, "dpg_gn_fetch: out is NULL");
    return fetch_1(c, hb_dev, out);
}

float dpg_gn_last_assemble_ms(dpg_ctx* c) { return c ? c->asm_ms : -1.f; }
float dpg_gn_last_solve_ms(dpg_ctx* c) { return c ? c->solve_ms : -1.f; }

int dpg_gn_run(dpg_ctx* c, double* poses_out, dpg_gn_stats* st) {
    if (!c || !c->gn_ready) return fail(DPG_ERR_STATE, "dpg_gn_run: graph not set up");
    HIP_TRY(hipSetDevice(c->device));
    const double t0 = now_ms();
    return gn_loop(c, c->gp, poses_out, t0, t0, st);
}

int dpg_optimize_graph(dpg_ctx* c, double* poses, int64_t V, const dpg_factor* F, int64_t nf, const dpg_gn_params* gp,
                       dpg_gn_stats* st) {
    const double t0 = now_ms();
    const dpg_gn_params P = or_default(gp, dpg_gn_params_default);
    if (!c || !F || !poses || V <= 0 || nf < 0) return fail(DPG_ERR_ARG, "dpg_optimize_graph: bad arguments");
    int rc = dpg_gn_setup(c, V, F, nf, 0, nf, &P);
    if (rc) return rc;
    if ((rc = dpg_gn_set_poses(c, poses))) return rc;
    return gn_loop(c, P, poses, t0, now_ms(), st);
}

int dpg_gn_marginals(dpg_ctx* c, const int32_t* nodes, int64_t n, double* cov_out) {
    if (c && c->gn_ready && !nodes && n != c->gn.v.n_nodes)
        return fail(DPG_ERR_ARG, "dpg_gn_marginals: nodes == NULL asks for every node (n = %lld)", (long long)c->gn.v.n_nodes);
    return gn_marginals_blocks(c, "dpg_gn_marginals", nodes, n, nullptr, 0, cov_out, nullptr);
}

int dpg_gn_marginal_pairs(dpg_ctx* c, const int32_t* pairs, int64_t n, double* cov_out) {
    if (n > 0 && !pairs) return fail(DPG_ERR_ARG, "dpg_gn_marginal_pairs: pairs is NULL");
    int rc = gn_marginals_state(c, "dpg_gn_marginal_pairs");
    if (rc) return rc;
    if (n < 0 || !cov_out) return fail(DPG_ERR_ARG, "dpg_gn_marginal_pairs: bad arguments");
    if ((rc = gn_pairs_share_factor(c, pairs, n))) return rc;
    return gn_marginals_blocks(c, "dpg_gn_marginal_pairs", nullptr, 0, pairs, n, cov_out, nullptr);
}

int dpg_gn_cross_covariances(dpg_ctx* c, const int32_t* pairs, int64_t n, double* cov_out) {
    return gn_joint_blocks(c, "dpg_gn_cross_covariances", 0, pairs, n, cov_out, nullptr);
}

int dpg_gn_joint_marginal(dpg_ctx* c, const int32_t* nodes, int64_t n, double* cov_out) {
    return gn_joint_blocks(c, "dpg_gn_joint_marginal", 1, nodes, n, cov_out, nullptr);
}

int dpg_gn_relative_covariances(dpg_ctx* c, const int32_t* pairs, int64_t n, double* cov_out) {
    const char* fn = "dpg_gn_relative_covariances";
    int rc = gn_marginals_state(c, fn);
    if (rc) return rc;
    if (n < 0 || (n > 0 && (!pairs || !cov_out))) return fail(DPG_ERR_ARG, "%s: bad arguments", fn);
    if (n == 0) return DPG_OK;
    for (int64_t q = 0; q < 2 * n; ++q)
        if (pairs[q] < 0 || pairs[q] >= c->gn.v.n_nodes) return fail(DPG_ERR_ARG, "%s: node %d is out of range", fn, pairs[q]);
    std::vector<int32_t> tri((size_t)(6 * n));
    dpg_relative_triples(pairs, n, tri.data());
    std::vector<double> blocks((size_t)(27 * n)), X((size_t)(3 * c->gn.v.n_nodes));
    if ((rc = gn_joint_blocks(c, fn, 0, tri.data(), 3 * n, blocks.data(), nullptr))) return rc;
    if ((rc = dpg_gn_get_poses(c, X.data()))) return rc;
    dpg_relative_from_blocks(pairs, n, X.data(), blocks.data(), cov_out);
    return DPG_OK;
}

int dpg_gn_joint_profile(dpg_ctx* c, const int32_t* pairs, int64_t n, double* out, int64_t cap) {
    if (!out || cap < 4 || n <= 0) return fail(DPG_ERR_ARG, "dpg_gn_joint_profile: bad arguments");
    std::vector<double> cov((size_t)(9 * n));
    float ms[2] = {0.f, 0.f};
    const int rc = gn_joint_blocks(c, "dpg_gn_joint_profile", 0, pairs, n, cov.data(), ms);
    if (rc) return rc;
    int64_t st[2];
    dpg_chol_path_stats(c->gn.v.chol, st);
    out[0] = ms[0];
    out[1] = ms[1];
    out[2] = (double)st[0];
    out[3] = (double)st[1];
    return DPG_OK;
// ... 39 lines not shown
```

dpg-slam_amd/csrc/dpg_gn_pipe.h:

```cpp
#ifndef DPG_GN_PIPE_H
#define DPG_GN_PIPE_H

#include <hip/hip_runtime.h>
#include <math.h>
#include <stdint.h>

#include "../../include/dpg_slam_c.h"

struct dpg_gn_dev;

#define DPG_GN_STATUS_DIVERGED 3

struct dpg_gn_ctl {
    int32_t active, reuse;
    int32_t last_was_chord, have_factor, it;
    uint32_t loop;
    int32_t pad[2];
    double last_dinf, prev_dinf, cur_error, pad2;
};
struct dpg_gn_slot {
    double dinf, error, status;
    int32_t reuse, active, final_, it;
    uint64_t tag;
};

__device__ __forceinline__ double pose_retract(double* __restrict__ Xv, double d0, double d1, double d2) {
    const double c = cos(Xv[2]), s = sin(Xv[2]);
    const double cd = cos(d2), sd = sin(d2);
    const double nx = Xv[0] + (c * d0 - s * d1);
    const double ny = Xv[1] + (s * d0 + c * d1);
    const double nc = c * cd - s * sd, ns = s * cd + c * sd;
    Xv[0] = nx;
    Xv[1] = ny;
    Xv[2] = atan2(ns, nc);
    double m = fmax(fabs(d0), fmax(fabs(d1), fabs(d2)));
    if (!(m == m)) m = __longlong_as_double(0x7ff0000000000000ll);
    return m;
}

extern "C" {
int dpg_chol_gated_ok(void* chol);
int dpg_chol_solve_gated(void* chol, const double* hb, const int32_t* gate, int prezeroed, double* X, double* max_out,
                         void* stream);
int dpg_chol_join_aux(void* chol, void* stream);
void dpg_chol_sync_dev(void* chol, int32_t** sync, int64_t* n_words);
int dpg_gn_pipe_init(dpg_gn_dev* g, const dpg_gn_params* gp, dpg_gn_ctl* ctl, const double* cur_dev, dpg_gn_slot* init,
                     uint32_t loop, void* stream);
int dpg_gn_pipe_issue(dpg_gn_dev* g, const dpg_gn_params* gp, dpg_gn_ctl* ctl, dpg_gn_slot* slot, void* stream);
int dpg_gn_pipe_issue_solve(dpg_gn_dev* g, dpg_gn_ctl* ctl, int part, void* stream);
int dpg_gn_pipe_issue_ctl(dpg_gn_dev* g, const dpg_gn_params* gp, dpg_gn_ctl* ctl, dpg_gn_slot* slot, int part,
                          void* stream);
}

#endif
```

dpg-slam_amd/csrc/dpg_icp_api.hip:

```cpp

#include <math.h>
#include <string.h>

#include "../../include/dpg_icp_cov.h"
#include "dpg_ctx.h"

namespace {

int set_kparams(dpg_icp_kparams* kp, const dpg_icp_params* p) {
    if (!p) return fail(DPG_ERR_ARG, "params is NULL");
    if (!(p->icp_max_correspondence_distance > 0.0)) return fail(DPG_ERR_ARG, "icp_max_correspondence_distance must be > 0");
    memset(kp, 0, sizeof(*kp));
    const double r = p->icp_max_correspondence_distance;
    kp->r2 = r * r;
    float f = (float)kp->r2;
    if ((double)f > kp->r2) f = nextafterf(f, 0.0f);
    kp->r2_f = f;
    kp->h_min = (float)(r * 1.05);
    kp->eps = p->icp_maximum_transformation_epsilon;
    kp->rot_thr = 1.0 - p->icp_maximum_transformation_epsilon;
    kp->mse_abs = p->mse_threshold_absolute;
    kp->max_iter = p->icp_maximum_iterations;
    kp->min_corr = p->min_number_correspondences;
    kp->reciprocal = p->icp_use_reciprocal_correspondences ? 1 : 0;
// ... 39 lines not shown
        if (rc) return fail(rc, "angle index build launch failed (%d)", rc);
    }
    if (v.ds == c->ds.p)
        c->idx_valid = c->icp_variant != DPG_ICP_ANGULAR ? 0 : tree_from <= c->idx_valid ? v.n_nodes : c->idx_valid;
    if (timed) HIP_TRY(hipEventRecord(c->ev[0].e, c->stream));
    if (c->icp_variant == DPG_ICP_ANGULAR) {
        kp.lds_tgt = round_up(std::max<int32_t>(maxp, 1), 16);
        kp.defer_cap = c->defer_cap;
        kp.kernel_variant = c->kernel_variant;
        const size_t per_edge = dpg_icp_ang_scratch_per_edge(kp.lds_tgt);
        size_t sbytes = 0;
        if (per_edge) {
            sbytes = per_edge * (size_t)std::min<int64_t>(ne, 2048);
            if (c->icp_scratch.reserve(sbytes)) return fail(DPG_ERR_HIP, "out of device memory for the ICP scratch");
        }
        rc = dpg_launch_icp_ang(v.ds, v.idx_pts, v.idx_ids, v.buckets, edges_dev, ne, &kp, maxp, res_dev, trace_dev,
                                per_edge ? c->icp_scratch.p : nullptr, sbytes, c->stream);
    } else if (c->icp_variant == DPG_ICP_KDTREE) {
        kp.lds_tgt = round_up(std::max<int32_t>(maxp, 1), 64);
        rc = dpg_launch_icp_kd(v.ds, v.idx_pts, v.idx_ids, edges_dev, ne, &kp, maxp, res_dev, trace_dev, c->stream);
    } else {
        kp.lds_tgt = round_up(std::max<int32_t>(maxp, 1), 64);
        rc = dpg_launch_icp(v.ds, edges_dev, ne, &kp, maxp, res_dev, trace_dev, c->stream);
    }
    if (rc) return fail(rc, "ICP kernel launch failed (%d): %s", rc, hipGetErrorString(hipGetLastError()));
    if (timed) HIP_TRY(hipEventRecord(c->ev[1].e, c->stream));
    if (hess_dev && timed) {
        if (!c->aux.s) HIP_TRY(hipStreamCreateWithFlags(&c->aux.s, hipStreamNonBlocking));
        HIP_TRY(hipStreamWaitEvent(c->aux.s, c->ev[1].e, 0));
        rc = dpg_launch_cov(v.full, edges_dev, ne, res_dev, hess_dev, c->cov_wg, c->aux.s);
        if (rc) return fail(rc, "covariance kernel launch failed");
        HIP_TRY(hipEventRecord(c->ev[2].e, c->aux.s));
        c->cov_pending = true;
        c->cov_on_aux = true;
        return DPG_OK;
    }
    if (timed) c->cov_on_aux = false;
    if (hess_dev) {
        rc = dpg_launch_cov(v.full, edges_dev, ne, res_dev, hess_dev, 0, c->stream);
        if (rc) return fail(rc, "covariance kernel launch failed");
    }
    if (timed) HIP_TRY(hipEventRecord(c->ev[2].e, c->stream));
    return DPG_OK;
}

void const_cov(float vx, float vy, float vth, double cov[9]) {
    memset(cov, 0, 9 * sizeof(double));
    cov[0] = (double)vx;
    cov[4] = (double)vy;
    cov[8] = (double)vth;
}

dpg_ctx* ctx_or_default(dpg_ctx* c) {
    if (c) return c;
    if (!g_default_ctx) g_default_ctx = dpg_ctx_create(0);
    return g_default_ctx;
}

}

void scans_truncate(dpg_ctx* c, int64_t V) {
    if (!c) return;
    for (int k = 0; k < n_dev(c); ++k) {
        dpg_ctx* q = dev_ctx(c, k);
        if (V < 0 || V >= q->n_nodes) continue;
        q->full_off.resize((size_t)V + 1);
        q->ds_off.resize((size_t)V + 1);
        q->n_nodes = V;
        q->idx_valid = std::min(q->idx_valid, V);
    }
}

extern "C" __global__ void downsample_kernel(const float2* __restrict__ full, const int64_t* __restrict__ full_off,
                                  const int64_t* __restrict__ ds_off, int32_t ratio, float2* __restrict__ ds) {
    const int64_t v = blockIdx.x;
    const int64_t f0 = full_off[v], d0 = ds_off[v], nd = ds_off[v + 1] - d0;
    for (int64_t k = threadIdx.x; k < nd; k += blockDim.x) ds[d0 + k] = full[f0 + k * ratio];
}

static int scans_upload_1(dpg_ctx* c, const float* pts, const int64_t* off, int64_t V, int32_t ratio) {
    if (!c || !pts || !off || V <= 0) return fail(DPG_ERR_ARG, "dpg_scans_upload: bad arguments");
    if (ratio < 1) ratio = 1;
    HIP_TRY(hipSetDevice(c->device));
    if (c->cov_pending) {
        HIP_TRY(hipEventSynchronize(c->ev[2].e));
        c->cov_pending = false;
    }
    const int64_t total = off[V];
    if (total >= ((int64_t)1 << 31)) return fail(DPG_ERR_SIZE, "too many points (%lld)", (long long)total);
    c->full_off.assign(off, off + V + 1);
    c->ds_off.assign((size_t)V + 1, 0);
    for (int64_t v = 0; v < V; ++v) {
        const int64_t n = off[v + 1] - off[v];
        if (n < 0) return fail(DPG_ERR_ARG, "node offsets must be non-decreasing");
        c->ds_off[(size_t)v + 1] = c->ds_off[(size_t)v] + (n + ratio - 1) / ratio;
    }
    const size_t n_ds = (size_t)(2 * std::max<int64_t>(c->ds_off[(size_t)V], 1));
    int64_t mx = 0;
    for (int64_t v = 0; v < V; ++v) mx = std::max(mx, c->ds_off[(size_t)v + 1] - c->ds_off[(size_t)v]);
    if (mx > 16384) return fail(DPG_ERR_SIZE, "a downsampled cloud has %lld points (max 16384)", (long long)mx);
    if (c->full.reserve((size_t)(2 * std::max<int64_t>(total, 1))) || c->ds.reserve(n_ds) ||
        c->ds_off_dev.reserve((size_t)V + 1) || c->full_off_dev.reserve((size_t)V + 1) || c->tree_pts.reserve(n_ds) ||
        c->tree_idx.reserve(n_ds / 2) || c->buckets.reserve((size_t)V * (size_t)(dpg_angle_buckets() + 1)))
        return fail(DPG_ERR_HIP, "out of device memory for scans");
    HIP_TRY(hipMemcpyAsync(c->full.p, pts, sizeof(float) * 2 * (size_t)total, hipMemcpyHostToDevice, c->stream));
    HIP_TRY(hipMemcpyAsync(c->full_off_dev.p, off, sizeof(int64_t) * ((size_t)V + 1), hipMemcpyHostToDevice, c->stream));
    HIP_TRY(hipMemcpyAsync(c->ds_off_dev.p, c->ds_off.data(), sizeof(int64_t) * ((size_t)V + 1), hipMemcpyHostToDevice,
                           c->stream));
    hipLaunchKernelGGL(downsample_kernel, dim3((unsigned)V), dim3(256), 0, c->stream, reinterpret_cast<const float2*>(c->full.p),
                       c->full_off_dev.p, c->ds_off_dev.p, ratio, reinterpret_cast<float2*>(c->ds.p));
    HIP_TRY(hipGetLastError());
    HIP_TRY(hipStreamSynchronize(c->stream));
    c->n_nodes = V;
    c->idx_valid = 0;
    c->ratio = ratio;
    c->max_ds = (int32_t)mx;
    return DPG_OK;
}

static int scans_append_1(dpg_ctx* c, const float* pts, const int64_t* off, int64_t k, int32_t ratio) {
    if (!c || !pts || !off || k <= 0) return fail(DPG_ERR_ARG, "dpg_scans_append: bad arguments");
    if (ratio < 1) ratio = 1;
    if (c->n_nodes == 0) return scans_upload_1(c, pts, off, k, ratio);
    if (c->cov_pending) {
        HIP_TRY(hipSetDevice(c->device));
        HIP_TRY(hipEventSynchronize(c->ev[2].e));
        c->cov_pending = false;
    }
    if (ratio != c->ratio) return fail(DPG_ERR_STATE, "scans were uploaded with downsample ratio %d", c->ratio);
    HIP_TRY(hipSetDevice(c->device));
    const int64_t V0 = c->n_nodes, V1 = V0 + k;
    const int64_t P0 = c->full_off[(size_t)V0], D0 = c->ds_off[(size_t)V0];
    const int64_t add = off[k] - off[0];
    if (P0 + add >= ((int64_t)1 << 31)) return fail(DPG_ERR_SIZE, "too many points");
    std::vector<int64_t> foff((size_t)k + 1), doff((size_t)k + 1);
    foff[0] = P0;
    doff[0] = D0;
    int64_t mx = c->max_ds;
    for (int64_t v = 0; v < k; ++v) {
        const int64_t n = off[v + 1] - off[v];
        if (n < 0) return fail(DPG_ERR_ARG, "node offsets must be non-decreasing");
        foff[(size_t)v + 1] = foff[(size_t)v] + n;
        doff[(size_t)v + 1] = doff[(size_t)v] + (n + ratio - 1) / ratio;
        mx = std::max(mx, (n + ratio - 1) / ratio);
    }
    if (mx > 16384) return fail(DPG_ERR_SIZE, "a downsampled cloud has %lld points (max 16384)", (long long)mx);
    const int64_t nds = doff[(size_t)k] - D0;
    std::vector<float> ds((size_t)(2 * std::max<int64_t>(nds, 1)));
    for (int64_t v = 0; v < k; ++v)
        dpg_downsample_cloud(pts + 2 * (off[v] - off[0]), off[v + 1] - off[v], ratio, ds.data() + 2 * (doff[(size_t)v] - D0));
    const size_t B = (size_t)(dpg_angle_buckets() + 1);
    if (c->full.grow((size_t)(2 * (P0 + add)), (size_t)(2 * P0), c->stream) ||
        c->ds.grow((size_t)(2 * (D0 + nds)), (size_t)(2 * D0), c->stream) ||
        c->ds_off_dev.grow((size_t)V1 + 1, (size_t)V0 + 1, c->stream) ||
        c->tree_pts.grow((size_t)(2 * (D0 + nds)), (size_t)(2 * D0), c->stream) ||
        c->tree_idx.grow((size_t)(D0 + nds), (size_t)D0, c->stream) ||
        c->buckets.grow((size_t)V1 * B, (size_t)V0 * B, c->stream))
        return fail(DPG_ERR_HIP, "out of device memory for scans");
    HIP_TRY(hipMemcpyAsync(c->full.p + 2 * P0, pts, sizeof(float) * 2 * (size_t)add, hipMemcpyHostToDevice, c->stream));
    if (nds > 0)
        HIP_TRY(hipMemcpyAsync(c->ds.p + 2 * D0, ds.data(), sizeof(float) * 2 * (size_t)nds, hipMemcpyHostToDevice, c->stream));
    HIP_TRY(hipMemcpyAsync(c->ds_off_dev.p + V0 + 1, doff.data() + 1, sizeof(int64_t) * (size_t)k, hipMemcpyHostToDevice,
                           c->stream));
    HIP_TRY(hipStreamSynchronize(c->stream));
    c->full_off.insert(c->full_off.end(), foff.begin() + 1, foff.end());
    c->ds_off.insert(c->ds_off.end(), doff.begin() + 1, doff.end());
    c->n_nodes = V1;
    c->max_ds = (int32_t)mx;
    return DPG_OK;
}

static int build_batch(dpg_ctx* c, const int32_t* edges, int64_t ne, const float* poses, const float* guesses,
                       const dpg_icp_params* p, std::vector<dpg_icp_edge>& out, dpg_icp_kparams& kp, int32_t& ms, int32_t& mt) {
    if (!c || (!edges && ne > 0) || ne < 0 || (!poses && !guesses) || !p) return fail(DPG_ERR_ARG, "dpg_icp_batch_prepare: bad arguments");
    if (c->n_nodes <= 0) return fail(DPG_ERR_STATE, "no scans uploaded");
    if (p->downsample_icp_points_ratio != c->ratio && !(p->downsample_icp_points_ratio < 1 && c->ratio == 1))
        return fail(DPG_ERR_STATE, "scans were uploaded with downsample ratio %d", c->ratio);
    int rc = set_kparams(&kp, p);
    if (rc) return rc;
    out.resize((size_t)ne);
    ms = mt = 0;
    for (int64_t e = 0; e < ne; ++e) {
        const int32_t t = edges[2 * e], s = edges[2 * e + 1];
        if (t < 0 || s < 0 || t >= c->n_nodes || s >= c->n_nodes)
            return fail(DPG_ERR_ARG, "edge %lld references a missing node", (long long)e);
        dpg_icp_edge& E = out[(size_t)e];
        memset(&E, 0, sizeof(E));
        E.src_node = s;
        E.tgt_node = t;
        E.src_ds_off = (int32_t)c->ds_off[(size_t)s];
        E.n_src_ds = (int32_t)(c->ds_off[(size_t)s + 1] - c->ds_off[(size_t)s]);
        E.tgt_ds_off = (int32_t)c->ds_off[(size_t)t];
        E.n_tgt_ds = (int32_t)(c->ds_off[(size_t)t + 1] - c->ds_off[(size_t)t]);
        E.src_full_off = (int32_t)c->full_off[(size_t)s];
        E.n_src_full = (int32_t)(c->full_off[(size_t)s + 1] - c->full_off[(size_t)s]);
        E.tgt_full_off = (int32_t)c->full_off[(size_t)t];
        E.n_tgt_full = (int32_t)(c->full_off[(size_t)t + 1] - c->full_off[(size_t)t]);
        if (guesses) memcpy(E.guess, guesses + 6 * e, sizeof(E.guess));
        else dpg_icp_guess(poses + 3 * s, poses + 3 * t, E.guess);
        E.pad[0] = (int32_t)e;
        ms = std::max(ms, E.n_src_ds);
        mt = std::max(mt, E.n_tgt_ds);
    }
    return DPG_OK;
}

// ... 217 lines not shown

static float batch_ms(dpg_ctx* c, int a, int b) {
    float worst = -1.f;
    for (int k = 0; k < (c ? n_dev(c) : 0); ++k) {
        dpg_ctx* q = dev_ctx(c, k);
        float ms = -1.f;
        if (hipSetDevice(q->device) != hipSuccess || hipEventSynchronize(q->ev[b].e) != hipSuccess ||
            hipEventElapsedTime(&ms, q->ev[a].e, q->ev[b].e) != hipSuccess)
            return -1.f;
        worst = std::max(worst, ms);
    }
    if (c) (void)hipSetDevice(c->device);
    return worst;
}

static double batch_bytes_1(dpg_ctx* c) {
    if (!c || c->n_edges <= 0) return 0.0;
    std::vector<dpg_icp_result> r((size_t)c->n_edges);
    if (hipMemcpy(r.data(), c->res.p, sizeof(dpg_icp_result) * r.size(), hipMemcpyDeviceToHost) != hipSuccess) return -1.0;
    double bytes = 0.0;
    for (int64_t e = 0; e < c->n_edges; ++e) {
        const dpg_icp_edge& E = c->h_edges[(size_t)e];
        bytes += (double)r[(size_t)E.pad[0]].iterations * (16.0 * E.n_src_ds + 8.0 * E.n_tgt_ds);
    }
    return bytes;
}

extern "C" {

int dpg_scans_upload(dpg_ctx* c, const float* pts, const int64_t* off, int64_t V, int32_t ratio) {
    if (!c) return fail(DPG_ERR_ARG, "dpg_scans_upload: bad arguments");
    c->cost.clear();
    for (int k = 0; k < n_dev(c); ++k) {
        const int rc = scans_upload_1(dev_ctx(c, k), pts, off, V, ratio);
        if (rc) return rc;
    }
    return hipSetDevice(c->device) == hipSuccess ? DPG_OK : DPG_ERR_HIP;
}

int dpg_scans_append(dpg_ctx* c, const float* pts, const int64_t* off, int64_t k, int32_t ratio) {
    if (!c) return fail(DPG_ERR_ARG, "dpg_scans_append: bad arguments");
    for (int d = 0; d < n_dev(c); ++d) {
        const int rc = scans_append_1(dev_ctx(c, d), pts, off, k, ratio);
        if (rc) return rc;
    }
    return hipSetDevice(c->device) == hipSuccess ? DPG_OK : DPG_ERR_HIP;
}

int dpg_scans_export(dpg_ctx* c, int64_t* n_nodes, int32_t* ratio, int64_t* off, float* pts) {
    if (!c || !n_nodes || !ratio) return fail(DPG_ERR_ARG, "dpg_scans_export: bad arguments");
    *n_nodes = c->n_nodes;
    *ratio = c->ratio;
    if (c->n_nodes <= 0) return DPG_OK;
    if (off) std::copy(c->full_off.begin(), c->full_off.begin() + c->n_nodes + 1, off);
    if (pts) {
        HIP_TRY(hipSetDevice(c->device));
        const size_t total = (size_t)c->full_off[(size_t)c->n_nodes];
        if (total) HIP_TRY(hipMemcpyAsync(pts, c->full.p, sizeof(float) * 2 * total, hipMemcpyDeviceToHost, c->stream));
        HIP_TRY(hipStreamSynchronize(c->stream));
    }
    return DPG_OK;
}

int dpg_scans_index_all(dpg_ctx* c) {
    if (!c) return fail(DPG_ERR_ARG, "dpg_scans_index_all: ctx is NULL");
    if (c->n_nodes <= 0 || c->icp_variant != DPG_ICP_ANGULAR) return DPG_OK;
    HIP_TRY(hipSetDevice(c->device));
    const int rc = dpg_launch_angle_index(c->ds.p, c->ds_off_dev.p, c->n_nodes, c->max_ds, c->tree_pts.p, c->tree_idx.p,
                                          c->buckets.p, c->kernel_variant == 2, c->stream);
    if (rc) return fail(rc, "angle index build failed");
    c->idx_valid = c->n_nodes;
    HIP_TRY(hipStreamSynchronize(c->stream));
    return DPG_OK;
}

static int batch_prepare(dpg_ctx* c, const int32_t* edges, int64_t ne, const float* poses, const float* guesses,
                         const dpg_icp_params* p) {
    if (!c) return fail(DPG_ERR_ARG, "dpg_icp_batch_prepare: bad arguments");
    int32_t ms = 0, mt = 0;
    dpg_icp_kparams kp;
    std::vector<dpg_icp_edge> all;
    int rc = build_batch(c, edges, ne, poses, guesses, p, all, kp, ms, mt);
    if (rc) return rc;
    c->batch.swap(all);
    c->kp = kp;
    c->max_src = ms;
    c->max_tgt = mt;
    c->batch_runs = 0;
    return plan_and_stage(c, c->schedule == DPG_ICP_SCHEDULE_MEASURED && ne > 0 && batch_costs_known(c));
}

int dpg_icp_batch_prepare(dpg_ctx* c, const int32_t* edges, int64_t ne, const float* poses, const dpg_icp_params* p) {
    if (!poses) return fail(DPG_ERR_ARG, "dpg_icp_batch_prepare: bad arguments");
    return batch_prepare(c, edges, ne, poses, nullptr, p);
}

int dpg_icp_batch_prepare_guess(dpg_ctx* c, const int32_t* edges, int64_t ne, const float* guesses,
                                const dpg_icp_params* p) {
    if (!guesses) return fail(DPG_ERR_ARG, "dpg_icp_batch_prepare_guess: guesses is NULL");
    return batch_prepare(c, edges, ne, nullptr, guesses, p);
}

int dpg_icp_batch_run(dpg_ctx* c, int32_t compute_cov, int32_t trace_iters) {
    if (!c) return fail(DPG_ERR_ARG, "ctx is NULL");
    if (trace_iters > 0 && is_multi(c)) return fail(DPG_ERR_STATE, "the correspondence trace is a single-device diagnostic");
    int rc;
    if (c->schedule == DPG_ICP_SCHEDULE_MEASURED && !c->batch_measured && c->batch_runs > 0 && trace_iters <= 0 &&
        !c->batch.empty()) {
        if (!batch_costs_known(c) && (rc = harvest_costs(c))) return rc;
        if (batch_costs_known(c) && (rc = plan_and_stage(c, true))) return rc;
    }
    for (int k = 0; k < n_dev(c); ++k) {
        dpg_ctx* q = dev_ctx(c, k);
        if ((rc = batch_run_1(q, compute_cov, trace_iters, std::min(q->idx_valid, q->n_nodes)))) return rc;
    }
    c->have_cov = compute_cov != 0;
    ++c->batch_runs;
    HIP_TRY(hipSetDevice(c->device));
    return DPG_OK;
}

float dpg_kdtree_build_ms(dpg_ctx* c) {
    float ms = -1.f;
    if (!c || hipEventSynchronize(c->ev[0].e) != hipSuccess) return -1.f;
    if (hipEventElapsedTime(&ms, c->ev[6].e, c->ev[0].e) != hipSuccess) return -1.f;
    return ms;
}

int dpg_icp_batch_fetch(dpg_ctx* c, dpg_icp_result* results, double* hess, int64_t cap) {
    if (!c) return fail(DPG_ERR_ARG, "ctx is NULL");
    if ((results || hess) && cap < (int64_t)c->batch.size())
        return fail(DPG_ERR_SIZE, "result buffers hold fewer records than the staged batch (dpg_icp_batch_size)");
    return batch_fetch(c, results, hess, true);
}

int64_t dpg_icp_batch_size(dpg_ctx* c) { return c ? (int64_t)c->batch.size() : fail(DPG_ERR_ARG, "ctx is NULL"); }

int dpg_icp_batch_fetch_trace(dpg_ctx* c, int32_t* trace, int64_t trace_cap, int64_t* max_src_out) {
    if (!c) return fail(DPG_ERR_ARG, "ctx is NULL");
    if (is_multi(c)) return fail(DPG_ERR_STATE, "the correspondence trace is a single-device diagnostic");
    if (max_src_out) *max_src_out = std::max(c->max_src, 1);
    if (!trace) return DPG_OK;
    if (c->trace_iters <= 0) return fail(DPG_ERR_STATE, "last batch ran without a trace");
    const size_t n = (size_t)c->n_edges * (size_t)c->trace_iters * (size_t)std::max(c->max_src, 1);
    if (trace_cap < 0 || (size_t)trace_cap < n) return fail(DPG_ERR_SIZE, "trace buffer smaller than E * trace_iters * max_src");
    HIP_TRY(hipMemcpyAsync(trace, c->trace.p, n * sizeof(int32_t), hipMemcpyDeviceToHost, c->stream));
    HIP_TRY(hipStreamSynchronize(c->stream));
    return DPG_OK;
}

float dpg_icp_batch_kernel_ms(dpg_ctx* c) { return batch_ms(c, 0, 1); }

float dpg_cov_batch_kernel_ms(dpg_ctx* c) { return batch_ms(c, 1, 2); }

int32_t dpg_cov_batch_overlapped(dpg_ctx* c) { return c && c->cov_on_aux ? 1 : 0; }

double dpg_icp_batch_algorithmic_bytes(dpg_ctx* c) {
    if (!c) return 0.0;
    double b = 0.0;
    for (int k = 0; k < n_dev(c); ++k) {
        (void)hipSetDevice(dev_ctx(c, k)->device);
        const double x = batch_bytes_1(dev_ctx(c, k));
        if (x < 0) return x;
        b += x;
    }
    (void)hipSetDevice(c->device);
    return b;
}

int dpg_run_icp(dpg_ctx* c, const float* src, int64_t ns, const float* tgt, int64_t nt, const float pose_src[3],
                const float pose_tgt[3], const dpg_icp_params* p, dpg_icp_result* result, double cov_out[9],
                double hess_out[9]) {
    if (!c || !src || !tgt || ns < 0 || nt < 0 || !pose_src || !pose_tgt || !p || !result)
        return fail(DPG_ERR_ARG, "dpg_run_icp: bad arguments");
    HIP_TRY(hipSetDevice(c->device));
    dpg_icp_kparams kp;
    int rc = set_kparams(&kp, p);
    if (rc) return rc;
    const int32_t ratio = p->downsample_icp_points_ratio > 0 ? p->downsample_icp_points_ratio : 1;
    const int64_t nsd = (ns + ratio - 1) / ratio, ntd = (nt + ratio - 1) / ratio;
    std::vector<float> buf((size_t)(2 * (ns + nt + nsd + ntd) + 2));
    memcpy(buf.data(), src, sizeof(float) * 2 * (size_t)ns);
    memcpy(buf.data() + 2 * ns, tgt, sizeof(float) * 2 * (size_t)nt);
    dpg_downsample_cloud(src, ns, ratio, buf.data() + 2 * (ns + nt));
    dpg_downsample_cloud(tgt, nt, ratio, buf.data() + 2 * (ns + nt + nsd));
    dpg_icp_edge E;
    memset(&E, 0, sizeof(E));
    E.src_node = 0;
    E.tgt_node = 1;
    E.src_full_off = 0; E.n_src_full = (int32_t)ns;
    E.tgt_full_off = (int32_t)ns; E.n_tgt_full = (int32_t)nt;
    E.src_ds_off = 0; E.n_src_ds = (int32_t)nsd;
    E.tgt_ds_off = (int32_t)nsd; E.n_tgt_ds = (int32_t)ntd;
    dpg_icp_guess(pose_src, pose_tgt, E.guess);
    const int64_t offs[3] = {0, nsd, nsd + ntd};
    if (c->s_pts.reserve(buf.size()) || c->s_edge.reserve(1) || c->s_res.reserve(1) || c->s_hess.reserve(9) ||
        c->s_off.reserve(3) || c->s_tree_pts.reserve((size_t)(2 * (nsd + ntd) + 2)) ||
        c->s_tree_idx.reserve((size_t)(nsd + ntd + 1)) || c->s_buckets.reserve((size_t)(2 * (dpg_angle_buckets() + 1))))
        return fail(DPG_ERR_HIP, "out of device memory");
    HIP_TRY(hipMemcpyAsync(c->s_pts.p, buf.data(), sizeof(float) * buf.size(), hipMemcpyHostToDevice, c->stream));
    HIP_TRY(hipMemcpyAsync(c->s_edge.p, &E, sizeof(E), hipMemcpyHostToDevice, c->stream));
    HIP_TRY(hipMemcpyAsync(c->s_off.p, offs, sizeof(offs), hipMemcpyHostToDevice, c->stream));
    const ScanView two{c->s_pts.p + 2 * (ns + nt), c->s_pts.p, c->s_off.p, 2, (int32_t)std::max(nsd, ntd),
// ... 76 lines not shown
```

dpg-slam_amd/csrc/dpg_internal.h:

```cpp
#ifndef DPG_INTERNAL_H
#define DPG_INTERNAL_H

#include <stdint.h>

#include "../../include/dpg_slam_c.h"

#ifdef __cplusplus
extern "C" {
#endif

int dpg_set_error(int code, const char* msg);
dpg_ctx* dpg_inc_ctx(dpg_inc* g);
int dpg_inc_prepare(dpg_inc* g, int64_t n_new, const int32_t* pairs, int64_t n_pairs);
int dpg_inc_abort_prepare(dpg_inc* g);
int dpg_scans_export(dpg_ctx* c, int64_t* n_nodes, int32_t* ratio, int64_t* off, float* pts);
int dpg_scans_index_all(dpg_ctx* c);
void dpg_ctx_adopt(dpg_ctx* c, void* child, void (*destroy)(void*));
void dpg_ctx_release_child(dpg_ctx* c, void* child);
int dpg_launch_host_wait(const uint32_t* flag, uint32_t tag, uint32_t* timed_out, void* stream);

typedef struct dpg_icp_edge {
    int32_t src_ds_off, n_src_ds;
    int32_t tgt_ds_off, n_tgt_ds;
    int32_t src_full_off, n_src_full;
// ... 12 lines not shown
    float h_min;
    int32_t max_iter;
    int32_t min_corr;
    int32_t reciprocal;
    int32_t cells_max;
    int32_t lds_tgt;
    int32_t trace_iters;
    int32_t trace_stride;
    int32_t defer_cap;
    int32_t kernel_variant;
} dpg_icp_kparams;

int dpg_launch_icp(const float* ds_pts_dev, const dpg_icp_edge* edges_dev, int64_t n_edges,
                   const dpg_icp_kparams* kp, int32_t max_points, dpg_icp_result* results_dev,
                   int32_t* trace_dev, void* stream);
int dpg_launch_cov(const float* full_pts_dev, const dpg_icp_edge* edges_dev, int64_t n_edges,
                   const dpg_icp_result* results_dev, double* hess_dev, int32_t max_workgroups, void* stream);
size_t dpg_icp_lds_bytes(int32_t lds_tgt, int32_t cells_max);
int dpg_launch_cov6(const float* pts_dev, int32_t n_data, int32_t n_model, const float* T6_dev, double* out_dev,
                    void* stream);
__attribute__((visibility("hidden"))) int dpg_cov6_from_sums(const double* sm, int64_t nh, int64_t nb, double cov6[36]);
int dpg_launch_kdtree_build(const float* ds_pts_dev, const int64_t* ds_off_dev, int64_t n_nodes,
                            int32_t max_points, float* tree_pts_dev, uint16_t* tree_idx_dev, void* stream);
int dpg_launch_icp_kd(const float* ds_pts_dev, const float* tree_pts_dev, const uint16_t* tree_idx_dev,
                      const dpg_icp_edge* edges_dev, int64_t n_edges, const dpg_icp_kparams* kp,
                      int32_t max_points, dpg_icp_result* results_dev, int32_t* trace_dev, void* stream);
size_t dpg_icp_kd_lds_bytes(int32_t cap);
int32_t dpg_angle_buckets(void);
int dpg_launch_lc_count(const float* poses_dev, const int32_t* pass_dev, int64_t V, float within, float across,
                        int32_t* count_dev, void* stream);
int dpg_launch_lc_write(const float* poses_dev, const int32_t* pass_dev, int64_t V, float within, float across,
                        const int64_t* off_dev, int32_t* pairs_dev, void* stream);
int dpg_launch_map_points(const float* pts_dev, const int64_t* off_dev, const float* frames_dev, int64_t V,
                          int32_t fraction, float* out_dev, void* stream);
int dpg_launch_angle_index(const float* ds_pts_dev, const int64_t* ds_off_dev, int64_t n_nodes,
                           int32_t max_points, float* idx_pts_dev, uint16_t* idx_orig_dev,
                           uint16_t* buckets_dev, int32_t bitonic, void* stream);
int dpg_launch_icp_ang(const float* ds_pts_dev, const float* idx_pts_dev, const uint16_t* idx_orig_dev,
                       const uint16_t* buckets_dev, const dpg_icp_edge* edges_dev, int64_t n_edges,
                       const dpg_icp_kparams* kp, int32_t max_points, dpg_icp_result* results_dev,
                       int32_t* trace_dev, void* scratch, size_t scratch_bytes, void* stream);
size_t dpg_icp_ang_lds_bytes(int32_t cap);
size_t dpg_icp_ang_scratch_per_edge(int32_t cap);

typedef struct dpg_csm_pair {
    int32_t tgt_off, n_tgt;
    int32_t src_off, n_src;
    float tx, ty;
    int32_t pad[2];
} dpg_csm_pair;

typedef struct dpg_gn_dev {
    int64_t n_nodes, n_factors, nnzb_upper, nnzb_full;
    int64_t shard_begin, shard_end;
    dpg_factor* factors;
    int32_t* up_cptr;
    int32_t* up_clist;
    int32_t* rowptr;
    int32_t* colidx;
    int32_t* src_up;
    double* bsr;
    double* minv;
    double* poses;
    double* x, *r, *z, *p0, *p1, *q;
    double* partials;
    double* scal;
    double* hb_own;
    void* chol;
    double* scal3;
    double* scal3_host;
    int32_t n_blocks_rows;
    int32_t last_pcg_iters;
    int32_t last_used_chol;
    double last_delta_inf;
    double prev_delta_inf;
    int32_t have_factor;
    int32_t last_was_chord;
    int32_t n_factorizations;
    uint8_t* mine;
    double* hb_part;
    int32_t world, rank;
    int32_t n_vote;
    double setup_ms[5];
} dpg_gn_dev;

struct dpg_chol_opts;
int dpg_chol_create(void** chol, int64_t n, const int32_t* pair_lo, const int32_t* pair_hi, int64_t n_pairs,
                    const struct dpg_chol_opts* opts);
void dpg_chol_destroy(void* chol);
int dpg_chol_solve(void* chol, const double* hb, void* stream);
int dpg_chol_resolve(void* chol, const double* hb, void* stream);
void dpg_chol_keep_inverse(void* chol, int on);
void dpg_chol_track_factor(void* chol, int on);
void dpg_chol_forget_factor(void* chol);
int dpg_chol_solve_partial(void* chol, const double* hb, const int32_t* dirty_nodes, int64_t n_dirty, void* stream);
void dpg_chol_partial_stats(void* chol, int64_t out[4]);
const int32_t* dpg_chol_pos_dev(void* chol);
const double* dpg_chol_x_dev(void* chol);
const int32_t* dpg_chol_status_dev(void* chol);
void dpg_chol_stats(void* chol, double out[6]);
int dpg_chol_selinv(void* chol, void* stream);
int dpg_chol_selinv_timed(void* chol, void* stream, float* level_ms, int cap);
int dpg_chol_selinv_check(void* chol, const int32_t* nodes, int64_t n, const int32_t* pairs, int64_t n_pairs);
int dpg_chol_selinv_gather(void* chol, const int32_t* nodes, int64_t n, const int32_t* pairs, int64_t n_pairs,
                           double* out_dev, void* stream);
int dpg_chol_marginals(void* chol, const int32_t* nodes, int64_t n, const int32_t* pairs, int64_t n_pairs,
                       double* host_out, void* stream);
int64_t dpg_chol_selinv_bytes(void* chol);
int dpg_chol_joint(void* chol, int by_nodes, const int32_t* idx, int64_t n, double* host_out, void* stream, float* ms);
void dpg_chol_path_stats(void* chol, int64_t out[2]);
void dpg_relative_covariance(const double xi[3], const double xj[3], const double* Sii, const double* Sij,
                             const double* Sjj, double out[9]);
void dpg_relative_triples(const int32_t* pairs, int64_t n, int32_t* tri);
void dpg_relative_from_blocks(const int32_t* pairs, int64_t n, const double* X, const double* blocks, double* out);

__attribute__((visibility("hidden"))) void dpg_contribution_lists(const dpg_factor* factors, int64_t n_factors, int64_t n,
                                                                  const int32_t* pair, int64_t n_pairs, int32_t* cptr,
                                                                  int32_t* clist);
int64_t dpg_gn_dev_hb_size(const dpg_gn_dev* g);
int64_t dpg_gn_dev_vote_offset(const dpg_gn_dev* g);
int dpg_gn_dev_assemble(dpg_gn_dev* g, double* hb_dev, void* stream);
int dpg_gn_dev_solve_async(dpg_gn_dev* g, const double* hb_dev, const dpg_gn_params* gp, void* stream);
int dpg_gn_dev_fetch(dpg_gn_dev* g, const double* hb_dev, void* stream, double out[3]);
int dpg_gn_dev_solve(dpg_gn_dev* g, const double* hb_dev, const dpg_gn_params* gp, void* stream,
                     double* delta_inf, double* error, int32_t* pcg_iters);
int dpg_gn_dev_icp_to_factors(dpg_gn_dev* g, const dpg_icp_result* results_dev, int64_t first,
                              int64_t count, int64_t n_always, double info_x, double info_y,
                              double info_th, void* stream);
struct GnGraph;
int dpg_gn_dev_set_ownership(struct GnGraph* g, int32_t world, int32_t rank, void* stream);
int dpg_gn_dev_icp_to_factors_scatter(dpg_gn_dev* g, const dpg_icp_result* results_dev, const int32_t* idx_dev,
                                      int64_t n_local, int64_t first, int64_t count, int64_t n_always, double info_x,
                                      double info_y, double info_th, void* stream);
int dpg_gn_dev_assemble_part(dpg_gn_dev* g, const int32_t* gate, void* stream);
int dpg_launch_vsum(const double* const* parts, double* const* outs, int32_t k, int64_t n, void* stream);

#ifdef __cplusplus
}
#endif
#endif
```

dpg-slam_amd/csrc/dpg_sweep.hip:

```cpp

#include <math.h>
#include <string.h>

#include "dpg_ctx.h"

static int64_t lc_candidates(dpg_ctx* c, int64_t V, const int32_t* pass, const float* est, float within,
                             float across, std::vector<int32_t>& pairs) {
    DevBuf<float> dposes;
    DevBuf<int32_t> dpass, dcount, dpairs;
    DevBuf<int64_t> doff;
    if (dposes.reserve((size_t)(3 * V)) || dpass.reserve((size_t)V) || dcount.reserve((size_t)V) ||
        doff.reserve((size_t)V))
        return fail(DPG_ERR_HIP, "allocation failed");
    int64_t acc = 0;
    std::vector<int32_t> cnt((size_t)V);
    std::vector<int64_t> off((size_t)V);
    const auto search = [&]() -> int {
        HIP_TRY(hipMemcpyAsync(dposes.p, est, sizeof(float) * 3 * V, hipMemcpyHostToDevice, c->stream));
        HIP_TRY(hipMemcpyAsync(dpass.p, pass, sizeof(int32_t) * V, hipMemcpyHostToDevice, c->stream));
        if (dpg_launch_lc_count(dposes.p, dpass.p, V, within, across, dcount.p, c->stream)) return DPG_ERR_HIP;
        HIP_TRY(hipMemcpyAsync(cnt.data(), dcount.p, sizeof(int32_t) * V, hipMemcpyDeviceToHost, c->stream));
        HIP_TRY(hipStreamSynchronize(c->stream));
        for (int64_t i = 0; i < V; ++i) { off[(size_t)i] = acc; acc += cnt[(size_t)i]; }
        pairs.assign((size_t)(2 * acc), 0);
        if (acc == 0) return DPG_OK;
        if (dpairs.reserve((size_t)(2 * acc))) return DPG_ERR_HIP;
        HIP_TRY(hipMemcpyAsync(doff.p, off.data(), sizeof(int64_t) * V, hipMemcpyHostToDevice, c->stream));
        if (dpg_launch_lc_write(dposes.p, dpass.p, V, within, across, doff.p, dpairs.p, c->stream)) return DPG_ERR_HIP;
        HIP_TRY(hipMemcpyAsync(pairs.data(), dpairs.p, sizeof(int32_t) * 2 * acc, hipMemcpyDeviceToHost, c->stream));
        HIP_TRY(hipStreamSynchronize(c->stream));
        return DPG_OK;
    };
    if (search()) return fail(DPG_ERR_HIP, "loop-closure candidate search failed: %s", hipGetErrorString(hipGetLastError()));
    return acc;
}

namespace {
struct Sweep {
    dpg_icp_params I;
    dpg_reopt_params R;
    dpg_reopt_stats S;
    std::vector<int32_t> edges;
    std::vector<dpg_factor> F;
    std::vector<dpg_icp_result> res;
    int64_t first_icp = 0, n_succ = 0;
    double t1 = 0.0, t2 = 0.0;
};
}

static int reopt_sweep(dpg_ctx* c, int64_t V, const int32_t* pass, const float* est, const float* odom,
                       const dpg_icp_params* ip, const dpg_reopt_params* rp, Sweep& w) {
    if (c->n_nodes != V) return fail(DPG_ERR_STATE, "scans of %lld nodes uploaded, sweep over %lld",
                                     (long long)c->n_nodes, (long long)V);
    w.I = or_default(ip, dpg_icp_params_default);
    w.R = or_default(rp, dpg_reopt_params_default);
    const dpg_reopt_params& R = w.R;
    std::vector<int32_t>& edges = w.edges;
    std::vector<dpg_factor>& F = w.F;
    memset(&w.S, 0, sizeof(w.S));
    const double t0 = now_ms();
    std::vector<int32_t> lc;
    const int64_t K = lc_candidates(c, V, pass, est, R.max_node_dist_within_pass, R.max_node_dist_across_passes, lc);
    if (K < 0) return (int)K;
    w.t1 = now_ms();
    w.n_succ = V - 1;
    const int64_t E = w.n_succ + K;
    edges.assign((size_t)(2 * E), 0);
    for (int64_t i = 1; i < V; ++i) { edges[(size_t)(2 * (i - 1))] = (int32_t)(i - 1); edges[(size_t)(2 * (i - 1) + 1)] = (int32_t)i; }
    if (K > 0) memcpy(edges.data() + 2 * w.n_succ, lc.data(), sizeof(int32_t) * 2 * (size_t)K);
    F.clear();
    F.reserve((size_t)(V + E));
    int32_t cur_pass = -1;
    for (int64_t i = 0; i < V; ++i) {
        if (i == 0 || pass[i] != cur_pass) {
            dpg_factor f;
            memset(&f, 0, sizeof(f));
            f.kind = DPG_FACTOR_PRIOR;
            f.i = (int32_t)i;
            for (int k = 0; k < 3; ++k) {
                const double sd = (double)R.new_pass_std_dev[k];
                f.info[k] = 1.0 / (sd * sd);
            }
            F.push_back(f);
            cur_pass = pass[i];
        } else if (R.odometry_constraints) {
            dpg_factor f;
            const int rc = dpg_odometry_factor(odom + 3 * (i - 1), odom + 3 * i, (int32_t)(i - 1), (int32_t)i,
                                               R.motion_model[0], R.motion_model[1], R.motion_model[2],
                                               R.motion_model[3], &f);
            if (rc) return fail(rc, "odometry factor %lld has no motion (zero sigma)", (long long)i);
            F.push_back(f);
        }
    }
    w.first_icp = (int64_t)F.size();
    for (int64_t e = 0; e < E; ++e) {
        dpg_factor f;
        memset(&f, 0, sizeof(f));
        f.kind = DPG_FACTOR_BETWEEN;
        f.i = edges[(size_t)(2 * e)];
        f.j = edges[(size_t)(2 * e + 1)];
        F.push_back(f);
    }
    int rc = dpg_icp_batch_prepare(c, edges.data(), E, est, &w.I);
    if (!rc) rc = dpg_icp_batch_run(c, 0, 0);
    w.S.n_candidates = K;
    w.S.n_icp_edges = E;
    w.S.ms_candidates = w.t1 - t0;
    if (rc) return rc;
    w.res.resize((size_t)std::max<int64_t>(E, 1));
    if ((rc = dpg_icp_batch_fetch(c, w.res.data(), nullptr, (int64_t)w.res.size()))) return rc;
    w.t2 = now_ms();
    return DPG_OK;
}

static bool closure_ok(const dpg_icp_result& r) { return r.converged && r.status == DPG_ICP_OK; }

static int append_icp_factors(const char* fn, const dpg_icp_result* res, const std::vector<int32_t>& edges, int64_t n_succ,
                              const dpg_icp_params& I, std::vector<dpg_factor>& F, int64_t& n_loop_closures) {
    const int64_t E = (int64_t)edges.size() / 2;
    for (int64_t e = 0; e < E; ++e)
        if (res[e].status == DPG_ICP_INTERNAL)
            return fail(DPG_ERR_INTERNAL, "%s: alignment %lld failed its internal check", fn, (long long)e);
    for (int64_t e = 0; e < E; ++e) {
        if (e >= n_succ && !closure_ok(res[e])) continue;
        dpg_factor f;
        dpg_icp_factor(&res[e], edges[(size_t)(2 * e)], edges[(size_t)(2 * e + 1)], &I, &f);
        F.push_back(f);
        if (e >= n_succ) ++n_loop_closures;
    }
    return DPG_OK;
}

extern "C" {

void dpg_reopt_params_default(dpg_reopt_params* p) {
    if (!p) return;
    p->max_node_dist_within_pass = 5.0f;
    p->max_node_dist_across_passes = 2.0f;
    p->new_pass_std_dev[0] = 0.2f;
    p->new_pass_std_dev[1] = 0.2f;
    p->new_pass_std_dev[2] = 0.15f;
    for (int k = 0; k < 4; ++k) p->motion_model[k] = 0.4f;
    p->odometry_constraints = 1;
}

int64_t dpg_loop_closure_candidates(dpg_ctx* c, int64_t V, const int32_t* pass, const float* est, float within,
                                    float across, int32_t* pairs_out, int64_t cap) {
    if (!c || V < 0 || (V > 0 && (!pass || !est))) return fail(DPG_ERR_ARG, "bad arguments");
    std::vector<int32_t> pairs;
    const int64_t K = lc_candidates(c, V, pass, est, within, across, pairs);
    if (K < 0) return K;
    if (pairs_out && cap > 0) memcpy(pairs_out, pairs.data(), sizeof(int32_t) * 2 * (size_t)std::min(K, cap));
    return K;
}

int64_t dpg_get_map(dpg_ctx* c, const float* est, int32_t fraction, float* out, int64_t cap) {
    if (!c || !est || fraction <= 0) return fail(DPG_ERR_ARG, "bad arguments");
    const int64_t V = c->n_nodes;
    if (V <= 0 || (int64_t)c->full_off.size() != V + 1) return fail(DPG_ERR_STATE, "no scans uploaded");
    const int64_t P = c->full_off[(size_t)V];
    const int64_t K = (P + fraction - 1) / fraction;
    if (!out || cap <= 0 || K == 0) return K;
    std::vector<float> fr((size_t)(4 * V));
    for (int64_t v = 0; v < V; ++v) {
        fr[(size_t)(4 * v)] = est[3 * v];
        fr[(size_t)(4 * v + 1)] = est[3 * v + 1];
        fr[(size_t)(4 * v + 2)] = cosf(est[3 * v + 2]);
        fr[(size_t)(4 * v + 3)] = sinf(est[3 * v + 2]);
    }
    DevBuf<float> dfr, dout;
    DevBuf<int64_t> doff;
    const auto assemble = [&]() -> int {
        if (dfr.reserve((size_t)(4 * V)) || dout.reserve((size_t)(2 * K)) || doff.reserve((size_t)(V + 1))) return DPG_ERR_HIP;
        HIP_TRY(hipMemcpyAsync(dfr.p, fr.data(), sizeof(float) * 4 * V, hipMemcpyHostToDevice, c->stream));
        HIP_TRY(hipMemcpyAsync(doff.p, c->full_off.data(), sizeof(int64_t) * (V + 1), hipMemcpyHostToDevice, c->stream));
        if (c->map_ev[0].ensure(hipEventDefault) || c->map_ev[1].ensure(hipEventDefault)) return DPG_ERR_HIP;
        HIP_TRY(hipEventRecord(c->map_ev[0].e, c->stream));
        if (dpg_launch_map_points(c->full.p, doff.p, dfr.p, V, fraction, dout.p, c->stream)) return DPG_ERR_HIP;
        HIP_TRY(hipEventRecord(c->map_ev[1].e, c->stream));
        HIP_TRY(hipMemcpyAsync(out, dout.p, sizeof(float) * 2 * std::min(K, cap), hipMemcpyDeviceToHost, c->stream));
        HIP_TRY(hipStreamSynchronize(c->stream));
        float ms = 0.f;
        if (hipEventElapsedTime(&ms, c->map_ev[0].e, c->map_ev[1].e) == hipSuccess) c->map_ms = ms;
        return DPG_OK;
    };
    if (assemble()) return fail(DPG_ERR_HIP, "map assembly failed: %s", hipGetErrorString(hipGetLastError()));
    return K;
// ... 150 lines not shown
```

dpg-slam_amd/dpgslam/_abi.py:

```python
from __future__ import annotations

import ctypes as C
import os

import numpy as np

_HERE = os.path.dirname(os.path.abspath(__file__))
LIB_PATH = os.environ.get("DPGSLAM_LIB") or os.path.join(os.path.dirname(_HERE), "lib", "libdpg.so")

DPG_OK = 0
DPG_FACTOR_PRIOR = 0
DPG_FACTOR_BETWEEN = 1
DPG_ICP_OK = 0
DPG_ICP_TOO_FEW_CORR = 1
DPG_ICP_LANES = 512


class IcpParams(C.Structure):

    _fields_ = [
        ("icp_maximum_iterations", C.c_int32),
        ("icp_use_reciprocal_correspondences", C.c_int32),
        ("icp_maximum_transformation_epsilon", C.c_double),
        ("icp_max_correspondence_distance", C.c_double),
# ... 253 lines not shown

ALLREDUCE_F64 = C.CFUNCTYPE(C.c_int, C.c_void_p, C.POINTER(C.c_double), C.c_int64)
ALLREDUCE_F32 = C.CFUNCTYPE(C.c_int, C.c_void_p, C.POINTER(C.c_float), C.c_int64)
ALLGATHER = C.CFUNCTYPE(C.c_int, C.c_void_p, C.c_void_p, C.c_void_p, C.c_int64)


class CollOps(C.Structure):

    _fields_ = [("user", C.c_void_p), ("allreduce_sum_f64", ALLREDUCE_F64), ("allreduce_sum_f32", ALLREDUCE_F32),
                ("allgather", ALLGATHER)]


SIGNATURES = {
    "dpg_last_error": (C.c_char_p, []),
    "dpg_version": (C.c_char_p, []),
    "dpg_icp_params_default": (None, [C.POINTER(IcpParams)]),
    "dpg_gn_params_default": (None, [C.POINTER(GnParams)]),
    "dpg_ctx_create": (P, [C.c_int]),
    "dpg_ctx_create_multi": (P, [C.c_int32, I32P]),
    "dpg_ctx_num_gpus": (C.c_int32, [P]),
    "dpg_ctx_create_virtual": (P, [C.c_int32, C.c_int32]),
    "dpg_ctx_create_rank": (P, [C.c_int32, P, C.c_int32, C.c_int32]),
    "dpg_ctx_create_rank_ops": (P, [C.c_int32, C.POINTER(CollOps), C.c_int32, C.c_int32]),
    "dpg_shard_plan": (C.c_int, [F32P, C.c_int64, C.c_int32, I32P, I64P, I64P]),
    "dpg_shard_reassemble": (C.c_int, [I32P, C.c_int64, C.c_int32, C.c_int64, C.c_int64, P, P]),
    "dpg_nccl_unique_id": (C.c_int, [P]),
    "dpg_ctx_num_ranks": (C.c_int32, [P]),
    "dpg_ctx_rank": (C.c_int32, [P]),
    "dpg_ctx_set_icp_schedule": (C.c_int, [P, C.c_int32]),
    "dpg_solver_options_default": (None, [C.POINTER(SolverOptions)]),
    "dpg_ctx_set_solver_options": (C.c_int, [P, C.POINTER(SolverOptions)]),
    "dpg_ctx_destroy": (None, [P]),
    "dpg_ctx_set_stream": (C.c_int, [P, P]),
    "dpg_ctx_synchronize": (C.c_int, [P]),
    "dpg_scan_to_cloud": (C.c_int64, [F32P, C.c_int64, C.c_float, C.c_float, C.c_float, C.c_float,
                                      C.c_float, C.c_float, F32P]),
    "dpg_scans_to_clouds": (C.c_int64, [F32P, C.c_int64, C.c_int64, C.c_float, C.c_float, C.c_float,
                                        C.c_float, C.c_float, C.c_float, F32P, I64P]),
    "dpg_downsample_cloud": (C.c_int64, [F32P, C.c_int64, C.c_int32, F32P]),
    "dpg_inverse_transform_point": (None, [F32P, F32P, F32P]),
    "dpg_transform_point": (None, [F32P, F32P, F32P]),
    "dpg_icp_guess": (None, [F32P, F32P, F32P]),
    "dpg_odometry_factors": (C.c_int, [F32P, C.c_int64, I32P, I32P, C.c_int64, C.c_float, C.c_float, C.c_float,
                                      C.c_float, C.c_void_p]),
    "dpg_odometry_factor": (C.c_int, [F32P, F32P, C.c_int32, C.c_int32, C.c_float, C.c_float, C.c_float,
                                      C.c_float, C.POINTER(Factor)]),
    "dpg_icp_factor": (None, [C.POINTER(IcpResult), C.c_int32, C.c_int32, C.POINTER(IcpParams),
                              C.POINTER(Factor)]),
    "dpg_synth_world": (C.c_int64, [C.c_uint64, C.c_float, F32P, C.c_int64]),
    "dpg_synth_trajectory": (C.c_int, [C.c_uint64, C.c_int64, F32P, C.c_int64, C.c_float, C.c_float, F64P]),
    "dpg_synth_scans": (C.c_int, [F64P, C.c_int64, F32P, C.c_int64, C.c_int32, C.c_float, C.c_float,
                                  C.c_float, C.c_float, C.c_float, C.c_float, C.c_float, C.c_uint64,
                                  C.c_int32, F32P]),
    "dpg_run_icp": (C.c_int, [P, F32P, C.c_int64, F32P, C.c_int64, F32P, F32P, C.POINTER(IcpParams),
                              C.POINTER(IcpResult), F64P, F64P]),
    "dpg_scans_upload": (C.c_int, [P, F32P, I64P, C.c_int64, C.c_int32]),
    "dpg_icp_batch_prepare": (C.c_int, [P, I32P, C.c_int64, F32P, C.POINTER(IcpParams)]),
    "dpg_icp_batch_run": (C.c_int, [P, C.c_int32, C.c_int32]),
    "dpg_icp_batch_fetch": (C.c_int, [P, P, F64P, C.c_int64]),
    "dpg_icp_batch_fetch_trace": (C.c_int, [P, I32P, C.c_int64, I64P]),
    "dpg_icp_batch_size": (C.c_int64, [P]),
    "dpg_icp_batch_kernel_ms": (C.c_float, [P]),
    "dpg_cov_batch_kernel_ms": (C.c_float, [P]),
    "dpg_cov_batch_overlapped": (C.c_int32, [P]),
    "dpg_kdtree_build_ms": (C.c_float, [P]),
    "dpg_ctx_set_icp_variant": (C.c_int, [P, C.c_int32]),
    "dpg_ctx_set_icp_defer_cap": (C.c_int, [P, C.c_int32]),
    "dpg_ctx_set_cov_workgroups": (C.c_int, [P, C.c_int32]),
    "dpg_ctx_set_icp_kernel_variant": (C.c_int, [P, C.c_int32]),
    "dpg_icp_batch_algorithmic_bytes": (C.c_double, [P]),
    "dpg_optimize_graph": (C.c_int, [P, F64P, C.c_int64, P, C.c_int64, C.POINTER(GnParams),
                                     C.POINTER(GnStats)]),
    "dpg_gn_setup": (C.c_int, [P, C.c_int64, P, C.c_int64, C.c_int64, C.c_int64, C.POINTER(GnParams)]),
    "dpg_gn_take_icp_measurements": (C.c_int, [P, C.c_int64, C.c_int64, C.c_int64, C.POINTER(IcpParams)]),
    "dpg_gn_hb_size": (C.c_int64, [P]),
    "dpg_gn_setup_profile": (C.c_int, [P, F64P]),
    "dpg_gn_set_poses": (C.c_int, [P, F64P]),
    "dpg_gn_get_poses": (C.c_int, [P, F64P]),
    "dpg_gn_assemble": (C.c_int, [P, P]),
    "dpg_gn_solve_retract": (C.c_int, [P, P, F64P, F64P, I32P]),
    "dpg_gn_solve_retract_async": (C.c_int, [P, P]),
    "dpg_gn_fetch": (C.c_int, [P, P, F64P]),
    "dpg_gn_factorizations": (C.c_int32, [P]),
    "dpg_gn_run": (C.c_int, [P, F64P, C.POINTER(GnStats)]),
    "dpg_gn_last_assemble_ms": (C.c_float, [P]),
    "dpg_gn_last_solve_ms": (C.c_float, [P]),
    "dpg_gn_marginals": (C.c_int, [P, I32P, C.c_int64, F64P]),
    "dpg_gn_marginal_pairs": (C.c_int, [P, I32P, C.c_int64, F64P]),
    "dpg_gn_cross_covariances": (C.c_int, [P, I32P, C.c_int64, F64P]),
    "dpg_gn_joint_marginal": (C.c_int, [P, I32P, C.c_int64, F64P]),
    "dpg_gn_relative_covariances": (C.c_int, [P, I32P, C.c_int64, F64P]),
    "dpg_gn_joint_profile": (C.c_int, [P, I32P, C.c_int64, F64P, C.c_int64]),
    "dpg_marginal_covariances": (C.c_int, [P, F64P, C.c_int64, P, C.c_int64, I32P, C.c_int64, F64P]),
    "dpg_gn_marginals_profile": (C.c_int64, [P, F64P, C.c_int64]),
    "icp_cov_calculate": (C.c_int, [P, F32P, C.c_int64, F32P, C.c_int64, F32P, C.c_float, C.c_float,
                                    C.c_float, F64P, F64P]),
    "icp_cov_sandwich": (C.c_int, [P, F32P, C.c_int64, F32P, C.c_int64, F32P, F64P, F64P]),
    "dpg_reopt_params_default": (None, [C.POINTER(ReoptParams)]),
    "dpg_get_map": (C.c_int64, [P, F32P, C.c_int32, F32P, C.c_int64]),
    "dpg_get_map_kernel_ms": (C.c_float, [P]),
    "dpg_loop_closure_candidates": (C.c_int64, [P, C.c_int64, I32P, F32P, C.c_float, C.c_float, I32P, C.c_int64]),
    "dpg_change_params_default": (None, [C.POINTER(ChangeParams)]),
    "dpg_dpg_create": (P, [P, C.c_int64, I64P, F32P, F32P, C.POINTER(ChangeParams)]),
    "dpg_dpg_destroy": (None, [P]),
    "dpg_dpg_append": (C.c_int, [P, C.c_int64, I64P, F32P, F32P]),
    "dpg_execute_dpg": (C.c_int, [P, C.c_int64, C.c_int64, F32P, C.POINTER(ChangeStats)]),
    "dpg_execute_dpg_chain": (C.c_int, [P, C.c_int64, C.c_int64, F32P, F32P, C.POINTER(ChangeStats)]),
    "dpg_dpg_fetch": (C.c_int, [P, U8P, U8P, U8P]),
    "dpg_dpg_load": (C.c_int, [P, U8P, U8P, U8P]),
    "dpg_active_dynamic_points": (C.c_int64, [P, C.c_int64, F32P, F32P, C.c_int64, I64P]),
    "dpg_grid_params_default": (None, [C.POINTER(GridParams)]),
    "dpg_occupancy_grid": (C.c_int, [P, C.c_int64, F32P, C.POINTER(GridParams), I32P, I32P, I8P, C.c_int64,
                                     C.POINTER(GridInfo)]),
    "dpg_dpg_beam_geometry": (C.c_int, [P, C.c_int64, F32P, F32P, F32P, C.c_int64]),
    "dpg_occupancy_from_counts": (None, [I32P, I32P, C.c_int64, I8P]),
    "dpg_grid_box": (C.c_int, [F32P, F32P, U8P, C.c_int64, C.c_double, C.c_int32, I32P]),
    "dpg_csm_params_default": (None, [C.POINTER(CsmParams)]),
    "dpg_csm_lds_bytes": (C.c_int64, [C.POINTER(CsmParams)]),
    "dpg_csm_lut": (C.c_int, [C.POINTER(CsmParams), U8P]),
    "dpg_csm_rotations": (C.c_int, [F32P, C.POINTER(CsmParams), F32P]),
    "dpg_csm_batch": (C.c_int, [P, I32P, C.c_int64, F32P, F32P, C.POINTER(CsmParams), P, C.c_int64]),
    "dpg_csm_table": (C.c_int, [P, C.c_int32, C.POINTER(CsmParams), U8P, C.c_int64]),
    "dpg_csm_scores": (C.c_int, [P, C.c_int32, C.c_int32, F32P, C.POINTER(CsmParams), I32P, C.c_int64]),
    "dpg_csm_kernel_ms": (C.c_float, [P]),
    "dpg_icp_batch_prepare_guess": (C.c_int, [P, I32P, C.c_int64, F32P, C.POINTER(IcpParams)]),
    "dpg_loc_params_default": (None, [C.POINTER(LocParams)]),
    "dpg_loc_params_check": (C.c_int, [C.POINTER(LocParams)]),
    "dpg_loc_rotations": (C.c_int, [C.c_float, C.POINTER(LocParams), F32P]),
    "dpg_map_localize": (C.c_int, [P, C.c_int64, F32P, F32P, C.c_int64, F32P, C.POINTER(LocParams),
                                   C.POINTER(LocResult)]),
    "dpg_map_field": (C.c_int, [P, C.c_int64, F32P, C.POINTER(LocParams), C.c_int32, U8P, C.c_int64, I32P]),
    "dpg_map_localize_bounds": (C.c_int, [P, C.c_int64, F32P, F32P, C.c_int64, F32P, C.POINTER(LocParams), I32P,
                                          C.c_int64]),
    "dpg_map_localize_scores": (C.c_int, [P, C.c_int64, F32P, F32P, C.c_int64, F32P, C.POINTER(LocParams), I32P,
                                          C.c_int64]),
    "dpg_reoptimize": (C.c_int, [P, C.c_int64, I32P, F32P, F32P, C.POINTER(IcpParams), C.POINTER(GnParams),
                                 C.POINTER(ReoptParams), F64P, C.POINTER(ReoptStats)]),
    "dpg_reoptimize_inc": (C.c_int, [P, C.c_int64, I32P, F32P, F32P, C.POINTER(IcpParams), C.POINTER(ReoptParams),
                                     F64P, C.POINTER(ReoptStats)]),
    "dpg_inc_params_default": (None, [C.POINTER(IncParams)]),
    "dpg_inc_create": (P, [P, C.POINTER(IncParams)]),
    "dpg_inc_destroy": (None, [P]),
    "dpg_inc_reset": (C.c_int, [P]),
    "dpg_inc_update": (C.c_int, [P, C.c_int64, F64P, P, C.c_int64, C.POINTER(IncStats)]),
    "dpg_inc_num_nodes": (C.c_int64, [P]),
    "dpg_inc_get_poses": (C.c_int, [P, F64P, C.c_int64]),
    "dpg_inc_marginals": (C.c_int, [P, I32P, C.c_int64, F64P]),
    "dpg_inc_cross_covariances": (C.c_int, [P, I32P, C.c_int64, F64P]),
    "dpg_inc_joint_marginal": (C.c_int, [P, I32P, C.c_int64, F64P]),
    "dpg_inc_relative_covariances": (C.c_int, [P, I32P, C.c_int64, F64P]),
    "dpg_inc_save": (C.c_int, [P, C.c_char_p]),
    "dpg_inc_load": (P, [P, C.c_char_p]),
    "dpg_inc_export": (C.c_int64, [P, I64P, P, I32P, C.c_int64, F64P, F64P, F64P]),
    "dpg_scans_append": (C.c_int, [P, F32P, I64P, C.c_int64, C.c_int32]),
    "dpg_add_node": (C.c_int, [P, F32P, C.c_int64, I32P, F32P, P, C.c_int64, C.POINTER(IcpParams),
                               C.POINTER(ReoptParams), C.c_int32, C.POINTER(AddNodeStats)]),
    "dpg_add_node_pairs": (C.c_int, [P, F32P, C.c_int64, F32P, P, C.c_int64, I32P, C.c_int64, C.c_int32,
                                     C.POINTER(IcpParams), C.POINTER(AddNodeStats)]),
}


def default_inc_params() -> IncParams:
    p = IncParams()
    lib().dpg_inc_params_default(C.byref(p))
    return p

# ... 95 lines not shown
```

dpg-slam_amd/dpgslam/api.py:

```python
from __future__ import annotations

import ctypes as C
import os
import weakref
from dataclasses import dataclass

import numpy as np

from . import _abi
from ._abi import (FACTOR_DTYPE, RESULT_DTYPE, F32P, F64P, I32P, I64P, check, lib, ptr, vptr)


@dataclass
class Node:

    pose: np.ndarray
    cloud: np.ndarray


def _f32(a) -> np.ndarray:
    return np.ascontiguousarray(np.asarray(a, dtype=np.float32))


def _f64(a) -> np.ndarray:
# ... 446 lines not shown

    def gn_cross_covariances(self, pairs) -> np.ndarray:
        return _joint_pairs("dpg_gn_cross_covariances", self.handle, pairs)

    def gn_joint_marginal(self, nodes) -> np.ndarray:
        return _joint_nodes("dpg_gn_joint_marginal", self.handle, nodes)

    def gn_relative_covariances(self, pairs) -> np.ndarray:
        return _joint_pairs("dpg_gn_relative_covariances", self.handle, pairs)

    def gn_joint_profile(self, pairs) -> dict:
        pr = _pair_list(pairs)
        out = np.zeros(4, np.float64)
        check(lib().dpg_gn_joint_profile(self.handle, ptr(pr, C.c_int32), len(pr), ptr(out, C.c_double), len(out)),
              "dpg_gn_joint_profile")
        return {"path_ms": float(out[0]), "dot_ms": float(out[1]), "path_fronts": int(out[2]),
                "path_scalars": int(out[3])}

    def gn_marginals_profile(self) -> dict:
        out = np.zeros(4 + 4096, np.float64)
        k = int(lib().dpg_gn_marginals_profile(self.handle, ptr(out, C.c_double), len(out)))
        if k < 0:
            check(k, "dpg_gn_marginals_profile")
        return {"assemble_ms": float(out[0]), "factor_ms": float(out[1]), "levels": int(out[2]),
                "sigma_bytes": int(out[3]), "level_ms": [float(x) for x in out[4:k]]}

    def gn_setup(self, V: int, factors: np.ndarray, shard=(0, None), params=None):
        F = np.ascontiguousarray(factors, FACTOR_DTYPE)
        b, e = shard[0], (len(F) if shard[1] is None else shard[1])
        gp = params or _abi.default_gn_params()
        check(lib().dpg_gn_setup(self.handle, V, vptr(F), len(F), b, e, C.byref(gp)), "dpg_gn_setup")
        self._gn_V = int(V)
        return int(lib().dpg_gn_hb_size(self.handle))

    def gn_take_icp(self, first: int, count: int, n_always: int, params=None):
        p = params or _abi.default_icp_params()
        check(lib().dpg_gn_take_icp_measurements(self.handle, first, count, n_always, C.byref(p)),
              "dpg_gn_take_icp_measurements")

    def gn_set_poses(self, poses):
        X = _f64(poses).reshape(-1, 3)
        check(lib().dpg_gn_set_poses(self.handle, ptr(X, C.c_double)), "dpg_gn_set_poses")

    def gn_setup_profile(self) -> dict:
        out = np.zeros(5, np.float64)
        check(lib().dpg_gn_setup_profile(self.handle, ptr(out, C.c_double)), "dpg_gn_setup_profile")
        return dict(zip(("pattern_lists_bsr", "chol_symbolic", "chol_plan", "wait_alloc_upload", "chol_upload"),
                        (float(x) for x in out)))

    def gn_run(self, V: int | None = None):
        X = np.empty((V, 3), np.float64) if V else None
        st = _abi.GnStats()
        check(lib().dpg_gn_run(self.handle, ptr(X, C.c_double) if X is not None else None, C.byref(st)),
              "dpg_gn_run")
        return {k: getattr(st, k) for k, _ in _abi.GnStats._fields_}, X

    def gn_get_poses(self, V: int) -> np.ndarray:
        X = np.empty((V, 3), np.float64)
        check(lib().dpg_gn_get_poses(self.handle, ptr(X, C.c_double)), "dpg_gn_get_poses")
        return X

    def gn_assemble(self, hb_dev_ptr: int | None = None):
        check(lib().dpg_gn_assemble(self.handle, C.c_void_p(hb_dev_ptr) if hb_dev_ptr else None), "dpg_gn_assemble")

    def gn_solve_retract(self, hb_dev_ptr: int | None = None):
        d, e, it = C.c_double(0), C.c_double(0), C.c_int32(0)
        check(lib().dpg_gn_solve_retract(self.handle, C.c_void_p(hb_dev_ptr) if hb_dev_ptr else None, C.byref(d),
                                         C.byref(e), C.byref(it)), "dpg_gn_solve_retract")
        return d.value, e.value, it.value

    def gn_solve_retract_async(self, hb_dev_ptr: int | None = None):
        check(lib().dpg_gn_solve_retract_async(self.handle, C.c_void_p(hb_dev_ptr) if hb_dev_ptr else None),
              "dpg_gn_solve_retract_async")

    def gn_fetch(self, hb_dev_ptr: int | None = None):
        out = np.zeros(3, np.float64)
        check(lib().dpg_gn_fetch(self.handle, C.c_void_p(hb_dev_ptr) if hb_dev_ptr else None, ptr(out, C.c_double)),
              "dpg_gn_fetch")
        return float(out[0]), float(out[1]), int(out[2])

    def gn_factorizations(self) -> int:
        return int(lib().dpg_gn_factorizations(self.handle))

    def loop_closure_candidates(self, est: np.ndarray, passes: np.ndarray, within: float = 5.0,
                                across: float = 2.0) -> np.ndarray:
        e, ps = _f32(est).reshape(-1, 3), np.ascontiguousarray(passes, np.int32)
        L = lib()
        n = L.dpg_loop_closure_candidates(self.handle, len(e), ptr(ps, C.c_int32), ptr(e, C.c_float), within, across,
                                          None, 0)
        if n < 0:
            check(int(n), "dpg_loop_closure_candidates")
        out = np.zeros((max(n, 1), 2), np.int32)
        n2 = L.dpg_loop_closure_candidates(self.handle, len(e), ptr(ps, C.c_int32), ptr(e, C.c_float), within, across,
                                           ptr(out, C.c_int32), n)
        if n2 < 0:
            check(int(n2), "dpg_loop_closure_candidates")
        return out[:n]

    def get_map(self, est: np.ndarray, display_points_fraction: int = 10) -> np.ndarray:
        e = _f32(est).reshape(-1, 3)
        L = lib()
        n = L.dpg_get_map(self.handle, ptr(e, C.c_float), display_points_fraction, None, 0)
        if n < 0:
            check(int(n), "dpg_get_map")
        out = np.zeros((max(n, 1), 2), np.float32)
        n2 = L.dpg_get_map(self.handle, ptr(e, C.c_float), display_points_fraction, ptr(out, C.c_float), n)
        if n2 < 0:
            check(int(n2), "dpg_get_map")
        return out[:n]

    def get_map_kernel_ms(self) -> float:
        return float(lib().dpg_get_map_kernel_ms(self.handle))

    def reoptimize(self, passes: np.ndarray, est: np.ndarray, odom: np.ndarray, icp_params=None, gn_params=None,
                   reopt_params=None):
        e, o = _f32(est).reshape(-1, 3), _f32(odom).reshape(-1, 3)
        ps = np.ascontiguousarray(passes, np.int32)
        ip = icp_params or _abi.default_icp_params()
        gp = gn_params or _abi.default_gn_params()
        rp = reopt_params or _abi.default_reopt_params()
        X = np.zeros((len(e), 3), np.float64)
        st = _abi.ReoptStats()
        check(lib().dpg_reoptimize(self.handle, len(e), ptr(ps, C.c_int32), ptr(e, C.c_float), ptr(o, C.c_float),
                                   C.byref(ip), C.byref(gp), C.byref(rp), ptr(X, C.c_double), C.byref(st)),
              "dpg_reoptimize")
        self.n_edges = int(st.n_icp_edges)
        return X, st

    def gn_times_ms(self):
        return float(lib().dpg_gn_last_assemble_ms(self.handle)), float(lib().dpg_gn_last_solve_ms(self.handle))


def _ctx_gone(child) -> bool:
    ctx = getattr(child, "ctx", None)
    return ctx is not None and getattr(ctx, "handle", None) is None


class DpgStore:

    def __init__(self, ctx: Context, ranges, geom, offsets=None, params=None):
        r = _f32(ranges)
        if offsets is None:
            V, nb = r.shape
            offsets = np.arange(V + 1, dtype=np.int64) * nb
        off = np.ascontiguousarray(offsets, np.int64)
        self.V = len(off) - 1
        self.B = int(off[-1])
        self.offsets = off.copy()
        g = _f32(geom).reshape(self.V, 3)
        self.params = params or _abi.default_change_params()
        self.ctx = ctx
        self.handle = lib().dpg_dpg_create(ctx.handle, self.V, ptr(off, C.c_int64), ptr(r.reshape(-1), C.c_float),
                                           ptr(g, C.c_float), C.byref(self.params))
        if not self.handle:
            raise _abi.DpgError("dpg_dpg_create failed: " + (lib().dpg_last_error() or b"").decode())
        ctx._children.add(self)

    def close(self):
        if getattr(self, "handle", None):
            if _ctx_gone(self):
                self.handle = None
                return
            lib().dpg_dpg_destroy(self.handle)
            self.handle = None

    def __del__(self):
# ... 292 lines not shown
```

include/dpg_slam_c.h:

```cpp
#ifndef DPG_SLAM_C_H
#define DPG_SLAM_C_H

#include <stddef.h>
#include <stdint.h>

#ifdef __cplusplus
extern "C" {
#endif

#define DPG_OK 0
#define DPG_ERR_ARG (-1)
#define DPG_ERR_HIP (-2)
#define DPG_ERR_STATE (-3)
#define DPG_ERR_SIZE (-4)
#define DPG_ERR_NUMERIC (-5)
#define DPG_ERR_INTERNAL (-6)

#define DPG_ICP_LANES 512

typedef struct dpg_icp_params {
    int32_t icp_maximum_iterations;
    int32_t icp_use_reciprocal_correspondences;
    double icp_maximum_transformation_epsilon;
    double icp_max_correspondence_distance;
// ... 100 lines not shown
    int32_t solve_maxseg;
    int32_t solve_dinv;
    int32_t merge_single;
    int32_t max_supernode_cols;
    int32_t solve_inv_cols;
    double relax_fraction;
} dpg_solver_options;
void dpg_solver_options_default(dpg_solver_options* o);
int dpg_ctx_set_solver_options(dpg_ctx* ctx, const dpg_solver_options* o);
int dpg_ctx_set_stream(dpg_ctx* ctx, void* hip_stream);
int dpg_ctx_synchronize(dpg_ctx* ctx);

int64_t dpg_scan_to_cloud(const float* ranges, int64_t n_ranges, float angle_min, float angle_max,
                          float range_max, float laser_x, float laser_y, float laser_theta,
                          float* xy_out);
int64_t dpg_scans_to_clouds(const float* ranges, int64_t n_nodes, int64_t n_beams, float angle_min,
                            float angle_max, float range_max, float laser_x, float laser_y,
                            float laser_theta, float* xy_out, int64_t* offsets_out);
int64_t dpg_downsample_cloud(const float* xy, int64_t n, int32_t ratio, float* xy_out);
void dpg_inverse_transform_point(const float a[3], const float b[3], float out[3]);
void dpg_transform_point(const float p[3], const float frame[3], float out[3]);
void dpg_icp_guess(const float pose_src[3], const float pose_tgt[3], float guess_out[6]);
int dpg_odometry_factor(const float odom_prev[3], const float odom_cur[3], int32_t i_prev, int32_t i_cur,
                        float transl_from_transl, float transl_from_rot, float rot_from_transl,
                        float rot_from_rot, dpg_factor* out);
void dpg_icp_factor(const dpg_icp_result* r, int32_t from_node, int32_t to_node,
                    const dpg_icp_params* p, dpg_factor* out);
int dpg_odometry_factors(const float* odom, int64_t n_odom, const int32_t* i_prev, const int32_t* i_cur, int64_t n,
                         float transl_from_transl, float transl_from_rot, float rot_from_transl, float rot_from_rot,
                         dpg_factor* out);

int64_t dpg_synth_world(uint64_t seed, float world_size, float* segs_out, int64_t max_segs);
int dpg_synth_trajectory(uint64_t seed, int64_t n_nodes, const float* segs, int64_t n_segs,
                         float world_size, float step, double* gt_out );
int dpg_synth_scans(const double* gt, int64_t n_nodes, const float* segs, int64_t n_segs,
                    int32_t n_beams, float angle_min, float angle_max, float range_max,
                    float laser_x, float laser_y, float laser_theta, float noise_sigma,
                    uint64_t seed, int32_t n_threads, float* ranges_out);

int dpg_run_icp(dpg_ctx* ctx, const float* src_xy, int64_t n_src, const float* tgt_xy, int64_t n_tgt,
                const float pose_src[3], const float pose_tgt[3], const dpg_icp_params* params,
                dpg_icp_result* result, double cov_out[9], double hess_out[9]);

int dpg_scans_upload(dpg_ctx* ctx, const float* pts_xy, const int64_t* node_offsets, int64_t n_nodes,
                     int32_t downsample_ratio);
int dpg_icp_batch_prepare(dpg_ctx* ctx, const int32_t* edges, int64_t n_edges, const float* poses,
                          const dpg_icp_params* params);
int dpg_icp_batch_run(dpg_ctx* ctx, int32_t compute_cov, int32_t trace_iters);
int dpg_icp_batch_fetch(dpg_ctx* ctx, dpg_icp_result* results, double* hess , int64_t cap);
int64_t dpg_icp_batch_size(dpg_ctx* ctx);
int dpg_icp_batch_fetch_trace(dpg_ctx* ctx, int32_t* trace , int64_t trace_cap,
                              int64_t* max_src_out);
float dpg_icp_batch_kernel_ms(dpg_ctx* ctx);
float dpg_cov_batch_kernel_ms(dpg_ctx* ctx);
int32_t dpg_cov_batch_overlapped(dpg_ctx* ctx);
float dpg_kdtree_build_ms(dpg_ctx* ctx);
#define DPG_ICP_ANGULAR 3
#define DPG_ICP_KDTREE 2
#define DPG_ICP_GRID 1
int dpg_ctx_set_icp_variant(dpg_ctx* ctx, int32_t variant);
int dpg_ctx_set_icp_defer_cap(dpg_ctx* ctx, int32_t cap);
int dpg_ctx_set_cov_workgroups(dpg_ctx* ctx, int32_t n);
int dpg_ctx_set_icp_kernel_variant(dpg_ctx* ctx, int32_t variant);
double dpg_icp_batch_algorithmic_bytes(dpg_ctx* ctx);

int dpg_optimize_graph(dpg_ctx* ctx, double* poses_inout, int64_t n_nodes, const dpg_factor* factors,
                       int64_t n_factors, const dpg_gn_params* params, dpg_gn_stats* stats);

int dpg_gn_setup(dpg_ctx* ctx, int64_t n_nodes, const dpg_factor* factors, int64_t n_factors,
                 int64_t shard_begin, int64_t shard_end, const dpg_gn_params* params);
int dpg_gn_take_icp_measurements(dpg_ctx* ctx, int64_t first_factor, int64_t count, int64_t n_always,
                                 const dpg_icp_params* params);
int64_t dpg_gn_hb_size(dpg_ctx* ctx);
int dpg_gn_setup_profile(dpg_ctx* ctx, double out[5]);
int dpg_gn_set_poses(dpg_ctx* ctx, const double* poses);
int dpg_gn_get_poses(dpg_ctx* ctx, double* poses);
int dpg_gn_assemble(dpg_ctx* ctx, double* hb_dev);
int dpg_gn_solve_retract(dpg_ctx* ctx, const double* hb_dev, double* delta_inf, double* error,
                         int32_t* pcg_iterations);
int dpg_gn_solve_retract_async(dpg_ctx* ctx, const double* hb_dev);
int dpg_gn_fetch(dpg_ctx* ctx, const double* hb_dev, double out[3]);
int dpg_gn_run(dpg_ctx* ctx, double* poses_out, dpg_gn_stats* stats);
int32_t dpg_gn_factorizations(dpg_ctx* ctx);
float dpg_gn_last_assemble_ms(dpg_ctx* ctx);
float dpg_gn_last_solve_ms(dpg_ctx* ctx);

int dpg_gn_marginals(dpg_ctx* ctx, const int32_t* nodes, int64_t n, double* cov_out );
int dpg_gn_marginal_pairs(dpg_ctx* ctx, const int32_t* pairs , int64_t n, double* cov_out );
int dpg_gn_cross_covariances(dpg_ctx* ctx, const int32_t* pairs , int64_t n, double* cov_out );
int dpg_gn_joint_marginal(dpg_ctx* ctx, const int32_t* nodes, int64_t n, double* cov_out );
int dpg_gn_relative_covariances(dpg_ctx* ctx, const int32_t* pairs , int64_t n, double* cov_out );
int dpg_gn_joint_profile(dpg_ctx* ctx, const int32_t* pairs , int64_t n, double* out, int64_t cap);
int dpg_marginal_covariances(dpg_ctx* ctx, const double* poses, int64_t n_nodes, const dpg_factor* factors,
                             int64_t n_factors, const int32_t* nodes, int64_t n, double* cov_out);
int64_t dpg_gn_marginals_profile(dpg_ctx* ctx, double* out, int64_t cap);

typedef struct dpg_reopt_params {
    float max_node_dist_within_pass;
    float max_node_dist_across_passes;
    float new_pass_std_dev[3];
    float motion_model[4];
    int32_t odometry_constraints;
} dpg_reopt_params;

typedef struct dpg_reopt_stats {
    int64_t n_factors;
    int64_t n_icp_edges;
    int64_t n_candidates;
    int64_t n_loop_closures;
    double ms_candidates;
    double ms_icp;
    double ms_gn;
    dpg_gn_stats gn;
} dpg_reopt_stats;

void dpg_reopt_params_default(dpg_reopt_params* p);

int64_t dpg_loop_closure_candidates(dpg_ctx* ctx, int64_t n_nodes, const int32_t* pass_numbers,
                                    const float* est_poses , float max_dist_within_pass,
                                    float max_dist_across_passes, int32_t* pairs_out , int64_t cap);

int64_t dpg_get_map(dpg_ctx* ctx, const float* est_poses , int32_t display_points_fraction,
                    float* map_out , int64_t cap);
float dpg_get_map_kernel_ms(dpg_ctx* ctx);

int dpg_reoptimize(dpg_ctx* ctx, int64_t n_nodes, const int32_t* pass_numbers, const float* est_poses,
                   const float* odom_only, const dpg_icp_params* icp_params, const dpg_gn_params* gn_params,
                   const dpg_reopt_params* params, double* poses_out, dpg_reopt_stats* stats);

struct dpg_inc;
int dpg_reoptimize_inc(struct dpg_inc* g, int64_t n_nodes, const int32_t* pass_numbers, const float* est_poses,
                       const float* odom_only, const dpg_icp_params* icp_params, const dpg_reopt_params* params,
                       double* poses_out, dpg_reopt_stats* stats);

#define DPG_INC_ISAM2 0
#define DPG_INC_BATCH 1
typedef struct dpg_inc_params {
    int32_t mode;
    int32_t relinearize_skip;
    double relinearize_threshold;
    int32_t duplicate_factors;
    int32_t reorder_every;
    int32_t reorder_lead;
    int32_t full_refactor;
    dpg_gn_params gn;
} dpg_inc_params;

typedef struct dpg_inc_stats {
    int64_t n_nodes, n_factors;
    int64_t nnz_l;
    int32_t reordered;
    int32_t relinearized;
    int32_t gn_iterations;
    int32_t fronts_kept;
    double error;
    double last_delta_inf;
    double ms_total, ms_symbolic, ms_numeric;
} dpg_inc_stats;

typedef struct dpg_inc dpg_inc;
void dpg_inc_params_default(dpg_inc_params* p);
dpg_inc* dpg_inc_create(dpg_ctx* ctx, const dpg_inc_params* params);
void dpg_inc_destroy(dpg_inc* g);
int dpg_inc_reset(dpg_inc* g);
int dpg_inc_update(dpg_inc* g, int64_t n_new, const double* init, const dpg_factor* factors, int64_t n_factors,
                   dpg_inc_stats* stats);
// ... 224 lines not shown
```

Before: 2.571 million.

## Speculatively prefactor GN Hessian on a side stream during ICP batch

When an ICP batch runs, the Gauss-Newton Hessian is assembled at the speculative poses and its Cholesky factor (and inverse) is computed on a high-priority side stream, overlapping the ICP kernels. The ICP-to-factor kernel now flags whether any information weights changed. If they did not, and the GN poses match the speculative ones, the first GN iteration reuses this precomputed factor instead of refactoring. The cost is extra device memory, a concurrent stream competing with ICP for compute, more state and synchronisation paths, and wasted work when the speculation is invalidated. It is single-device only.

```diff
diff --git a/dpg-slam_amd/csrc/dpg_chol.hip b/dpg-slam_amd/csrc/dpg_chol.hip
--- a/dpg-slam_amd/csrc/dpg_chol.hip
+++ b/dpg-slam_amd/csrc/dpg_chol.hip
@@ -318,6 +318,20 @@
     return hipGetLastError() == hipSuccess ? DPG_OK : DPG_ERR_HIP;
 }
 
+extern "C" int dpg_chol_prefactor(void* h, const double* hb, void* stream) {
+    CholDev* c = reinterpret_cast<CholDev*>(h);
+    if (!dpg_chol_gated_ok(h)) return DPG_ERR_STATE;
+    c->fac_valid = false;
+    c->has_factor = true;
+    hipStream_t st = reinterpret_cast<hipStream_t>(stream);
+    if (hipMemsetAsync(c->status.p, 0, sizeof(int32_t), st) != hipSuccess ||
+        hipMemsetAsync(c->sync.p, 0, c->plan.sync_bytes, st) != hipSuccess)
+        return DPG_ERR_HIP;
+    launch_factor(c, st, hb, nullptr, nullptr);
+    launch_inv(c, st, nullptr);
+    return hipGetLastError() == hipSuccess ? DPG_OK : DPG_ERR_HIP;
+}
+
 extern "C" void dpg_chol_keep_inverse(void* h, int on) {
     if (h) reinterpret_cast<CholDev*>(h)->keep_inv = on != 0;
 }
diff --git a/dpg-slam_amd/csrc/dpg_ctx.h b/dpg-slam_amd/csrc/dpg_ctx.h
--- a/dpg-slam_amd/csrc/dpg_ctx.h
+++ b/dpg-slam_amd/csrc/dpg_ctx.h
@@ -112,9 +112,12 @@
     PinBuf<double> scal3_host;
     DevBuf<uint8_t> mine;
     DevBuf<double> hb_part;
+    DevBuf<double> hb_spec, chi2_spec;
+    DevBuf<int32_t> spec_flag;
     CholPtr chol;
     int build(int64_t n_nodes, const dpg_factor* factors, int64_t n_factors, int64_t shard_begin, int64_t shard_end,
               const dpg_chol_opts* opts, hipStream_t sync_stream);
+    int ensure_spec();
 };
 
 struct dpg_ctx {
@@ -169,6 +172,13 @@
     DevBuf<dpg_gn_ctl> pipe_ctl;
     MappedBuf<dpg_gn_slot> pipe_slot;
     uint32_t pipe_loop = 0;
+    DevStream spec;
+    DevEvent spec_join, spec_done;
+    DevBuf<double> x_spec;
+    std::vector<double> x_spec_host;
+    bool x_spec_ok = false;
+    bool pf_on = true, pf_launched = false, pf_pending = false, pf_live = false, pf_poses = false;
+    int32_t pf_state = 0;
     std::vector<dpg_ctx*> peers;
     std::vector<std::pair<void*, void (*)(void*)>> children;
     std::vector<ncclComm_t> comms;
@@ -232,6 +242,10 @@
 void scans_truncate(dpg_ctx* c, int64_t V);
 int icp_batch_run_from(dpg_ctx* c, int64_t tree_from);
 int batch_fetch(dpg_ctx* c, dpg_icp_result* results, double* hess, bool learn);
+int icp_batch_run(dpg_ctx* c, int32_t compute_cov, int32_t trace_iters, bool prefactor);
+void prefactor_launch(dpg_ctx* c);
+int prefactor_cancel(dpg_ctx* c);
+void prefactor_drain(dpg_ctx* c);
 int gn_loop(dpg_ctx* c, const dpg_gn_params& P, double* poses, double t0, double t1, dpg_gn_stats* st);
 
 #pragma GCC visibility pop
diff --git a/dpg-slam_amd/csrc/dpg_ctx.hip b/dpg-slam_amd/csrc/dpg_ctx.hip
--- a/dpg-slam_amd/csrc/dpg_ctx.hip
+++ b/dpg-slam_amd/csrc/dpg_ctx.hip
@@ -309,6 +309,7 @@
     c->comms.clear();
     (void)hipSetDevice(c->device);
     (void)join_cov(c);
+    prefactor_drain(c);
     (void)hipStreamSynchronize(c->stream);
     c->hc.reset();
     if (c == g_default_ctx) g_default_ctx = nullptr;
@@ -318,6 +319,7 @@
 int dpg_ctx_set_stream(dpg_ctx* c, void* s) {
     if (!c) return fail(DPG_ERR_ARG, "ctx is NULL");
     if (join_cov(c)) return fail(DPG_ERR_HIP, "stream wait failed");
+    prefactor_drain(c);
     HIP_TRY(hipStreamSynchronize(c->stream));
     c->own.release();
     c->stream = reinterpret_cast<hipStream_t>(s);
diff --git a/dpg-slam_amd/csrc/dpg_gn.hip b/dpg-slam_amd/csrc/dpg_gn.hip
--- a/dpg-slam_amd/csrc/dpg_gn.hip
+++ b/dpg-slam_amd/csrc/dpg_gn.hip
@@ -385,12 +385,17 @@
 
 __global__ void icp_to_factor_kernel(const dpg_icp_result* __restrict__ res, dpg_factor* __restrict__ F,
                                      int64_t first, int64_t count, int64_t n_always, double ix, double iy,
-                                     double ith) {
+                                     double ith, int32_t* changed) {
     const int64_t e = (int64_t)blockIdx.x * blockDim.x + threadIdx.x;
     if (e >= count) return;
     dpg_factor& f = F[first + e];
     const dpg_icp_result r = res[e];
+    const long long w0 = __double_as_longlong(f.info[0]), w1 = __double_as_longlong(f.info[1]),
+                    w2 = __double_as_longlong(f.info[2]);
     icp_factor_write(f, r, e, n_always, ix, iy, ith);
+    if (changed && (w0 != __double_as_longlong(f.info[0]) || w1 != __double_as_longlong(f.info[1]) ||
+                    w2 != __double_as_longlong(f.info[2])))
+        *changed = 1;
 }
 
 template <typename B, typename T>
@@ -537,7 +542,8 @@
     if (count <= 0) return DPG_OK;
     if (first < 0 || first + count > g->n_factors) return DPG_ERR_ARG;
     hipLaunchKernelGGL(icp_to_factor_kernel, dim3(nblk(count)), dim3(kRowThreads), 0,
-                       reinterpret_cast<hipStream_t>(stream), res, g->factors, first, count, n_always, ix, iy, ith);
+                       reinterpret_cast<hipStream_t>(stream), res, g->factors, first, count, n_always, ix, iy, ith,
+                       g->spec_flag);
     return hipGetLastError() == hipSuccess ? DPG_OK : DPG_ERR_HIP;
 }
 
@@ -558,6 +564,34 @@
 
 extern "C" int dpg_gn_dev_assemble(dpg_gn_dev* g, double* hb, void* stream) {
     return assemble_gated(g, hb, reinterpret_cast<hipStream_t>(stream), nullptr);
+}
+
+int GnGraph::ensure_spec() {
+    dpg_gn_dev* g = &v;
+    if (g->hb_spec) return DPG_OK;
+    int rc = take(hb_spec, g->hb_spec, (size_t)dpg_gn_dev_hb_size(g));
+    rc |= take(chi2_spec, g->chi2_spec, (size_t)g->n_nodes);
+    rc |= take(spec_flag, g->spec_flag, 1);
+    if (rc) {
+        hb_spec.release();
+        chi2_spec.release();
+        spec_flag.release();
+        g->hb_spec = g->chi2_spec = nullptr;
+        g->spec_flag = nullptr;
+        return DPG_ERR_HIP;
+    }
+    return DPG_OK;
+}
+
+extern "C" int dpg_gn_dev_prefactor(dpg_gn_dev* g, const double* X_spec, void* stream) {
+    if (!g->chol || !g->hb_spec || !X_spec) return DPG_ERR_STATE;
+    const int64_t ng = lg_groups(g->n_nodes, g->nnzb_upper);
+    if (ng > 0)
+        hipLaunchKernelGGL(lin_gather_kernel, dim3((unsigned)ng), dim3(kLgLanes), 0, reinterpret_cast<hipStream_t>(stream),
+                           g->factors, X_spec, g->up_cptr, g->up_clist, g->n_nodes, g->nnzb_upper, g->shard_begin, g->shard_end,
+                           g->mine, g->hb_spec, g->chi2_spec, nullptr);
+    if (hipGetLastError() != hipSuccess) return DPG_ERR_HIP;
+    return dpg_chol_prefactor(g->chol, g->hb_spec, stream);
 }
 
 __global__ void own_kernel(uint8_t* __restrict__ mine, int64_t nf, int32_t world, int32_t rank) {
@@ -697,18 +731,22 @@
 
 __global__ void pipe_init_kernel(dpg_gn_ctl* ctl, int32_t reuse, int32_t last_was_chord, int32_t have_factor,
                                  double last_dinf, double prev_dinf, const double* cur_dev, dpg_gn_slot* init,
-                                 double* max_out, int32_t* sync, int64_t n_words, int32_t* status, uint32_t loop) {
+                                 double* max_out, int32_t* sync, int64_t n_words, int32_t* status, uint32_t loop,
+                                 const int32_t* spec_flag) {
+    const int32_t pre = threadIdx.x == 0 && spec_flag && spec_flag[0] == 0 && *status == 0 ? 1 : 0;
     clear_sync(sync, n_words, status);
     if (threadIdx.x != 0) return;
     const double cur = *cur_dev;
     {
         dpg_gn_slot o{};
         o.error = cur;
+        o.reuse = pre;
         post_slot(init, o, (uint64_t)loop << 32);
     }
     ctl->loop = loop;
     ctl->active = !(cur <= 0.0) ? 1 : 0;
-    ctl->reuse = reuse;
+    ctl->reuse = reuse | pre;
+    ctl->prefactored = pre;
     ctl->last_was_chord = last_was_chord;
     ctl->have_factor = have_factor;
     ctl->it = 0;
@@ -736,8 +774,9 @@
     clear_sync(sync, n_words, status);
     if (threadIdx.x != 0) return;
     *chi2 = sum;
+    const int32_t chord = ctl->reuse && !ctl->prefactored ? 1 : 0;
     dpg_gn_slot o;
-    o.reuse = ctl->reuse;
+    o.reuse = chord;
     o.active = ctl->active;
     o.it = ctl->it;
     o.final_ = 1;
@@ -782,7 +821,8 @@
         o.final_ = fin ? 1 : 0;
         ctl->prev_dinf = ctl->last_dinf;
         ctl->last_dinf = dinf;
-        ctl->last_was_chord = ctl->reuse;
+        ctl->last_was_chord = chord;
+        ctl->prefactored = 0;
         ctl->have_factor = 1;
         ctl->cur_error = nw;
         ctl->it = it;
@@ -795,7 +835,7 @@
 }
 
 extern "C" int dpg_gn_pipe_init(dpg_gn_dev* g, const dpg_gn_params* gp, dpg_gn_ctl* ctl, const double* cur_dev,
-                                dpg_gn_slot* init, uint32_t loop, void* stream) {
+                                dpg_gn_slot* init, uint32_t loop, int prefactored, void* stream) {
     hipStream_t s = reinterpret_cast<hipStream_t>(stream);
     const bool slow = g->last_was_chord && g->last_delta_inf > 0.1 * g->prev_delta_inf;
     const bool reuse = gp->reuse_factorization && g->have_factor && g->last_delta_inf < gp->refactor_delta && !slow;
@@ -804,7 +844,7 @@
     dpg_chol_sync_dev(g->chol, &sync, &n_words);
     hipLaunchKernelGGL(pipe_init_kernel, dim3(1), dim3(1024), 0, s, ctl, reuse ? 1 : 0, g->last_was_chord, g->have_factor,
                        g->last_delta_inf, g->prev_delta_inf, cur_dev, init, g->scal3, sync, n_words,
-                       const_cast<int32_t*>(dpg_chol_status_dev(g->chol)), loop);
+                       const_cast<int32_t*>(dpg_chol_status_dev(g->chol)), loop, prefactored ? g->spec_flag : nullptr);
     return hipGetLastError() == hipSuccess ? DPG_OK : DPG_ERR_HIP;
 }
 
diff --git a/dpg-slam_amd/csrc/dpg_gn_api.hip b/dpg-slam_amd/csrc/dpg_gn_api.hip
--- a/dpg-slam_amd/csrc/dpg_gn_api.hip
+++ b/dpg-slam_amd/csrc/dpg_gn_api.hip
@@ -9,9 +9,12 @@
 static int gn_setup_1(dpg_ctx* c, int64_t V, const dpg_factor* F, int64_t nf, int64_t b, int64_t e,
                       const dpg_gn_params* gp) {
     HIP_TRY(hipSetDevice(c->device));
+    c->pf_launched = false;
+    (void)prefactor_cancel(c);
     GnGraph ng;
     int rc = ng.build(V, F, nf, b, e, &c->copts, c->stream);
     if (rc) return fail(rc, "pose-graph setup failed (invalid factor or out of memory)");
+    prefactor_drain(c);
     c->gn = std::move(ng);
     c->gn_ready = true;
     c->gn_pairs_valid = false;
@@ -25,6 +28,8 @@
     HIP_TRY(hipMemcpyAsync(c->gn.v.poses, poses, sizeof(double) * 3 * (size_t)c->gn.v.n_nodes, hipMemcpyHostToDevice,
                            c->stream));
     HIP_TRY(hipStreamSynchronize(c->stream));
+    c->pf_poses = c->pf_launched && c->pf_live && c->x_spec_host.size() == 3 * (size_t)c->gn.v.n_nodes &&
+                  !memcmp(poses, c->x_spec_host.data(), sizeof(double) * c->x_spec_host.size());
     c->gn.v.have_factor = 0;
     c->gn.v.last_delta_inf = 1e300;
     c->gn.v.prev_delta_inf = 1e300;
@@ -38,6 +43,7 @@
         if (!(c) || !(c)->gn_ready) return fail(DPG_ERR_STATE, "graph not set up");                             \
         if (is_multi(c)) return fail(DPG_ERR_STATE, "the step API is per device: a multi-device context runs "   \
                                                     "dpg_gn_run / dpg_optimize_graph / dpg_reoptimize");         \
+        if (prefactor_cancel(c)) return DPG_ERR_HIP;                                                             \
     } while (0)
 
 static int solve_retract_async_1(dpg_ctx* c, const double* hb_dev) {
@@ -217,9 +223,9 @@
     }
 }
 
-static int gn_loop_pipe_body(dpg_ctx* c, const dpg_gn_params& P, dpg_gn_stats& S, double& nw, double& dinf, int& it);
-static int gn_loop_pipe(dpg_ctx* c, const dpg_gn_params& P, dpg_gn_stats& S, double& nw, double& dinf, int& it) {
-    int rc = gn_loop_pipe_body(c, P, S, nw, dinf, it);
+static int gn_loop_pipe_body(dpg_ctx* c, const dpg_gn_params& P, dpg_gn_stats& S, double& nw, double& dinf, int& it, bool pre);
+static int gn_loop_pipe(dpg_ctx* c, const dpg_gn_params& P, dpg_gn_stats& S, double& nw, double& dinf, int& it, bool pre) {
+    int rc = gn_loop_pipe_body(c, P, S, nw, dinf, it, pre);
     if (c->coll == kCollHost && c->hc) {
         hc_drain(c);
         if (!rc && c->hc->failed.exchange(0)) rc = fail(DPG_ERR_HIP, "the caller's all-reduce of the packed system failed");
@@ -228,7 +234,7 @@
     }
     return rc;
 }
-static int gn_loop_pipe_body(dpg_ctx* c, const dpg_gn_params& P, dpg_gn_stats& S, double& nw, double& dinf, int& it) {
+static int gn_loop_pipe_body(dpg_ctx* c, const dpg_gn_params& P, dpg_gn_stats& S, double& nw, double& dinf, int& it, bool pre) {
     const int L = n_dev(c);
     const int part = is_multi(c) ? 1 : 0;
     int rc;
@@ -237,7 +243,7 @@
         if ((rc = ensure_pipe(q))) return rc;
         ++q->pipe_loop;
         const double* cur_dev = q->gn.v.hb_own + 9 * q->gn.v.nnzb_upper + 3 * q->gn.v.n_nodes;
-        if ((rc = dpg_gn_pipe_init(&q->gn.v, &P, q->pipe_ctl.p, cur_dev, q->pipe_slot.p + 2, q->pipe_loop, q->stream)))
+        if ((rc = dpg_gn_pipe_init(&q->gn.v, &P, q->pipe_ctl.p, cur_dev, q->pipe_slot.p + 2, q->pipe_loop, pre && k == 0, q->stream)))
             return fail(rc, "GN pipeline launch failed");
     }
     auto issue = [&](int i) -> int {
@@ -273,6 +279,7 @@
             if (i == 1) {
                 if ((rc = wait_slot(q, q->pipe_slot.p + 2, (uint64_t)q->pipe_loop << 32))) return rc;
                 const double e0 = static_cast<const volatile dpg_gn_slot*>(q->pipe_slot.p + 2)->error;
+                if (pre && static_cast<const volatile dpg_gn_slot*>(q->pipe_slot.p + 2)->reuse) c->pf_state = 1;
                 if (e0 <= 0.0) {
                     for (int j = 0; j < L; ++j) (void)hipStreamSynchronize(dev_ctx(c, j)->stream);
                     S.initial_error = e0;
@@ -346,6 +353,58 @@
     return true;
 }
 
+void prefactor_launch(dpg_ctx* c) {
+    if (!c->pf_on || is_multi(c) || !c->gn_ready || !c->x_spec_ok) return;
+    dpg_gn_dev* g = &c->gn.v;
+    if (c->gp.max_iterations <= 0 || !pipe_ok(c, c->gp) || c->x_spec_host.size() != 3 * (size_t)g->n_nodes) return;
+    if (prefactor_cancel(c)) return;
+    c->pf_launched = false;
+    if (hipSetDevice(c->device) != hipSuccess) return;
+    if (!c->spec.s) {
+        int lo = 0, hi = 0;
+        if (hipDeviceGetStreamPriorityRange(&lo, &hi) != hipSuccess ||
+            hipStreamCreateWithPriority(&c->spec.s, hipStreamNonBlocking, hi) != hipSuccess) {
+            c->spec.s = nullptr;
+            (void)hipGetLastError();
+            return;
+        }
+    }
+    if (c->spec_join.ensure(hipEventDisableTiming) || c->spec_done.ensure(hipEventDisableTiming) || c->gn.ensure_spec()) {
+        (void)hipGetLastError();
+        return;
+    }
+    if (hipMemsetAsync(g->spec_flag, 0, sizeof(int32_t), c->stream) != hipSuccess ||
+        hipEventRecord(c->spec_join.e, c->stream) != hipSuccess ||
+        hipStreamWaitEvent(c->spec.s, c->spec_join.e, 0) != hipSuccess) {
+        (void)hipGetLastError();
+        return;
+    }
+    const int rc = dpg_gn_dev_prefactor(g, c->x_spec.p, c->spec.s);
+    if (rc) (void)hipGetLastError();
+    if (hipEventRecord(c->spec_done.e, c->spec.s) != hipSuccess) {
+        (void)hipGetLastError();
+        (void)hipStreamSynchronize(c->spec.s);
+        return;
+    }
+    c->pf_pending = true;
+    c->pf_launched = c->pf_live = rc == DPG_OK;
+    c->pf_poses = false;
+}
+
+int prefactor_cancel(dpg_ctx* c) {
+    c->pf_live = c->pf_poses = false;
+    if (!c->pf_pending) return DPG_OK;
+    c->pf_pending = false;
+    HIP_TRY(hipSetDevice(c->device));
+    HIP_TRY(hipStreamWaitEvent(c->stream, c->spec_done.e, 0));
+    return DPG_OK;
+}
+
+void prefactor_drain(dpg_ctx* c) {
+    c->pf_live = c->pf_poses = c->pf_pending = false;
+    if (c->spec.s && hipSetDevice(c->device) == hipSuccess) (void)hipStreamSynchronize(c->spec.s);
+}
+
 int gn_loop(dpg_ctx* c, const dpg_gn_params& P, double* poses, double t0, double t1, dpg_gn_stats* st) {
     dpg_gn_stats S;
     memset(&S, 0, sizeof(S));
@@ -363,12 +422,16 @@
     double cur = 0.0, nw = 0.0, dinf = 0.0;
     int it = 0;
     const bool pipe = pipe_ok(c, P) && P.max_iterations > 0;
+    const bool pre = !multi && pipe && c->pf_launched && c->pf_live && c->pf_poses;
+    c->pf_state = c->pf_launched ? 2 : 0;
+    c->pf_launched = false;
+    if ((rc = prefactor_cancel(c))) return rc;
     if (!pipe) {
         if ((rc = read_error(c, &S.initial_error))) return rc;
         cur = nw = S.initial_error;
     }
     if (pipe) {
-        if ((rc = gn_loop_pipe(c, P, S, nw, dinf, it))) return rc;
+        if ((rc = gn_loop_pipe(c, P, S, nw, dinf, it, pre))) return rc;
     } else if (!(cur <= 0.0) && P.max_iterations > 0) {
         for (;;) {
             for (int k = 0; k < L; ++k) {
@@ -445,6 +508,7 @@
 
 static int gn_factor_at_current_poses(dpg_ctx* c, const char* fn, bool timed) {
     HIP_TRY(hipSetDevice(c->device));
+    if (prefactor_cancel(c)) return DPG_ERR_HIP;
     dpg_gn_dev* g = &c->gn.v;
     int rc;
     if (timed) HIP_TRY(hipEventRecord(c->ev[3].e, c->stream));
@@ -619,6 +683,14 @@
     DPG_STEP_API_1(c);
     return solve_retract_async_1(c, hb_dev);
 }
+
+int dpg_ctx_set_gn_prefactor(dpg_ctx* c, int32_t on) {
+    if (!c) return fail(DPG_ERR_ARG, "ctx is NULL");
+    c->pf_on = on != 0;
+    return DPG_OK;
+}
+
+int32_t dpg_gn_prefactor_state(dpg_ctx* c) { return c ? c->pf_state : -1; }
 
 int32_t dpg_gn_factorizations(dpg_ctx* c) { return (c && c->gn_ready) ? c->gn.v.n_factorizations : -1; }
 
diff --git a/dpg-slam_amd/csrc/dpg_gn_pipe.h b/dpg-slam_amd/csrc/dpg_gn_pipe.h
--- a/dpg-slam_amd/csrc/dpg_gn_pipe.h
+++ b/dpg-slam_amd/csrc/dpg_gn_pipe.h
@@ -15,7 +15,8 @@
     int32_t active, reuse;
     int32_t last_was_chord, have_factor, it;
     uint32_t loop;
-    int32_t pad[2];
+    int32_t prefactored;
+    int32_t pad;
     double last_dinf, prev_dinf, cur_error, pad2;
 };
 struct dpg_gn_slot {
@@ -45,7 +46,7 @@
 int dpg_chol_join_aux(void* chol, void* stream);
 void dpg_chol_sync_dev(void* chol, int32_t** sync, int64_t* n_words);
 int dpg_gn_pipe_init(dpg_gn_dev* g, const dpg_gn_params* gp, dpg_gn_ctl* ctl, const double* cur_dev, dpg_gn_slot* init,
-                     uint32_t loop, void* stream);
+                     uint32_t loop, int prefactored, void* stream);
 int dpg_gn_pipe_issue(dpg_gn_dev* g, const dpg_gn_params* gp, dpg_gn_ctl* ctl, dpg_gn_slot* slot, void* stream);
 int dpg_gn_pipe_issue_solve(dpg_gn_dev* g, dpg_gn_ctl* ctl, int part, void* stream);
 int dpg_gn_pipe_issue_ctl(dpg_gn_dev* g, const dpg_gn_params* gp, dpg_gn_ctl* ctl, dpg_gn_slot* slot, int part,
diff --git a/dpg-slam_amd/csrc/dpg_icp_api.hip b/dpg-slam_amd/csrc/dpg_icp_api.hip
--- a/dpg-slam_amd/csrc/dpg_icp_api.hip
+++ b/dpg-slam_amd/csrc/dpg_icp_api.hip
@@ -145,6 +145,7 @@
     if (!c || !pts || !off || V <= 0) return fail(DPG_ERR_ARG, "dpg_scans_upload: bad arguments");
     if (ratio < 1) ratio = 1;
     HIP_TRY(hipSetDevice(c->device));
+    prefactor_drain(c);
     if (c->cov_pending) {
         HIP_TRY(hipEventSynchronize(c->ev[2].e));
         c->cov_pending = false;
@@ -185,6 +186,7 @@
     if (!c || !pts || !off || k <= 0) return fail(DPG_ERR_ARG, "dpg_scans_append: bad arguments");
     if (ratio < 1) ratio = 1;
     if (c->n_nodes == 0) return scans_upload_1(c, pts, off, k, ratio);
+    prefactor_drain(c);
     if (c->cov_pending) {
         HIP_TRY(hipSetDevice(c->device));
         HIP_TRY(hipEventSynchronize(c->ev[2].e));
@@ -568,6 +570,15 @@
     std::vector<dpg_icp_edge> all;
     int rc = build_batch(c, edges, ne, poses, guesses, p, all, kp, ms, mt);
     if (rc) return rc;
+    prefactor_drain(c);
+    c->x_spec_ok = false;
+    if (poses && !is_multi(c) && c->pf_on) {
+        c->x_spec_host.assign(poses, poses + 3 * (size_t)c->n_nodes);
+        c->x_spec_ok = hipSetDevice(c->device) == hipSuccess && !c->x_spec.reserve(c->x_spec_host.size()) &&
+                       hipMemcpyAsync(c->x_spec.p, c->x_spec_host.data(), sizeof(double) * c->x_spec_host.size(),
+                                      hipMemcpyHostToDevice, c->stream) == hipSuccess;
+        if (!c->x_spec_ok) (void)hipGetLastError();
+    }
     c->batch.swap(all);
     c->kp = kp;
     c->max_src = ms;
@@ -588,6 +599,12 @@
 }
 
 int dpg_icp_batch_run(dpg_ctx* c, int32_t compute_cov, int32_t trace_iters) {
+    return icp_batch_run(c, compute_cov, trace_iters, true);
+}
+
+}
+
+int icp_batch_run(dpg_ctx* c, int32_t compute_cov, int32_t trace_iters, bool prefactor) {
     if (!c) return fail(DPG_ERR_ARG, "ctx is NULL");
     if (trace_iters > 0 && is_multi(c)) return fail(DPG_ERR_STATE, "the correspondence trace is a single-device diagnostic");
     int rc;
@@ -596,6 +613,7 @@
         if (!batch_costs_known(c) && (rc = harvest_costs(c))) return rc;
         if (batch_costs_known(c) && (rc = plan_and_stage(c, true))) return rc;
     }
+    if (prefactor) prefactor_launch(c);
     for (int k = 0; k < n_dev(c); ++k) {
         dpg_ctx* q = dev_ctx(c, k);
         if ((rc = batch_run_1(q, compute_cov, trace_iters, std::min(q->idx_valid, q->n_nodes)))) return rc;
@@ -605,6 +623,8 @@
     HIP_TRY(hipSetDevice(c->device));
     return DPG_OK;
 }
+
+extern "C" {
 
 float dpg_kdtree_build_ms(dpg_ctx* c) {
     float ms = -1.f;
diff --git a/dpg-slam_amd/csrc/dpg_internal.h b/dpg-slam_amd/csrc/dpg_internal.h
--- a/dpg-slam_amd/csrc/dpg_internal.h
+++ b/dpg-slam_amd/csrc/dpg_internal.h
@@ -118,6 +118,9 @@
     int32_t world, rank;
     int32_t n_vote;
     double setup_ms[5];
+    double* hb_spec;
+    double* chi2_spec;
+    int32_t* spec_flag;
 } dpg_gn_dev;
 
 struct dpg_chol_opts;
@@ -126,6 +129,7 @@
 void dpg_chol_destroy(void* chol);
 int dpg_chol_solve(void* chol, const double* hb, void* stream);
 int dpg_chol_resolve(void* chol, const double* hb, void* stream);
+int dpg_chol_prefactor(void* chol, const double* hb, void* stream);
 void dpg_chol_keep_inverse(void* chol, int on);
 void dpg_chol_track_factor(void* chol, int on);
 void dpg_chol_forget_factor(void* chol);
@@ -156,6 +160,7 @@
 int64_t dpg_gn_dev_hb_size(const dpg_gn_dev* g);
 int64_t dpg_gn_dev_vote_offset(const dpg_gn_dev* g);
 int dpg_gn_dev_assemble(dpg_gn_dev* g, double* hb_dev, void* stream);
+int dpg_gn_dev_prefactor(dpg_gn_dev* g, const double* X_spec, void* stream);
 int dpg_gn_dev_solve_async(dpg_gn_dev* g, const double* hb_dev, const dpg_gn_params* gp, void* stream);
 int dpg_gn_dev_fetch(dpg_gn_dev* g, const double* hb_dev, void* stream, double out[3]);
 int dpg_gn_dev_solve(dpg_gn_dev* g, const double* hb_dev, const dpg_gn_params* gp, void* stream,
diff --git a/dpg-slam_amd/csrc/dpg_sweep.hip b/dpg-slam_amd/csrc/dpg_sweep.hip
--- a/dpg-slam_amd/csrc/dpg_sweep.hip
+++ b/dpg-slam_amd/csrc/dpg_sweep.hip
@@ -102,7 +102,7 @@
         F.push_back(f);
     }
     int rc = dpg_icp_batch_prepare(c, edges.data(), E, est, &w.I);
-    if (!rc) rc = dpg_icp_batch_run(c, 0, 0);
+    if (!rc) rc = icp_batch_run(c, 0, 0, false);
     w.S.n_candidates = K;
     w.S.n_icp_edges = E;
     w.S.ms_candidates = w.t1 - t0;
diff --git a/dpg-slam_amd/dpgslam/_abi.py b/dpg-slam_amd/dpgslam/_abi.py
--- a/dpg-slam_amd/dpgslam/_abi.py
+++ b/dpg-slam_amd/dpgslam/_abi.py
@@ -359,6 +359,8 @@
     "dpg_gn_solve_retract_async": (C.c_int, [P, P]),
     "dpg_gn_fetch": (C.c_int, [P, P, F64P]),
     "dpg_gn_factorizations": (C.c_int32, [P]),
+    "dpg_ctx_set_gn_prefactor": (C.c_int, [P, C.c_int32]),
+    "dpg_gn_prefactor_state": (C.c_int32, [P]),
     "dpg_gn_run": (C.c_int, [P, F64P, C.POINTER(GnStats)]),
     "dpg_gn_last_assemble_ms": (C.c_float, [P]),
     "dpg_gn_last_solve_ms": (C.c_float, [P]),
diff --git a/dpg-slam_amd/dpgslam/api.py b/dpg-slam_amd/dpgslam/api.py
--- a/dpg-slam_amd/dpgslam/api.py
+++ b/dpg-slam_amd/dpgslam/api.py
@@ -552,6 +552,12 @@
     def gn_factorizations(self) -> int:
         return int(lib().dpg_gn_factorizations(self.handle))
 
+    def set_gn_prefactor(self, on: bool):
+        check(lib().dpg_ctx_set_gn_prefactor(self.handle, int(bool(on))), "dpg_ctx_set_gn_prefactor")
+
+    def gn_prefactor_state(self) -> int:
+        return int(lib().dpg_gn_prefactor_state(self.handle))
+
     def loop_closure_candidates(self, est: np.ndarray, passes: np.ndarray, within: float = 5.0,
                                 across: float = 2.0) -> np.ndarray:
         e, ps = _f32(est).reshape(-1, 3), np.ascontiguousarray(passes, np.int32)
diff --git a/include/dpg_slam_c.h b/include/dpg_slam_c.h
--- a/include/dpg_slam_c.h
+++ b/include/dpg_slam_c.h
@@ -206,6 +206,8 @@
 int dpg_gn_fetch(dpg_ctx* ctx, const double* hb_dev, double out[3]);
 int dpg_gn_run(dpg_ctx* ctx, double* poses_out, dpg_gn_stats* stats);
 int32_t dpg_gn_factorizations(dpg_ctx* ctx);
+int dpg_ctx_set_gn_prefactor(dpg_ctx* ctx, int32_t on);
+int32_t dpg_gn_prefactor_state(dpg_ctx* ctx);
 float dpg_gn_last_assemble_ms(dpg_ctx* ctx);
 float dpg_gn_last_solve_ms(dpg_ctx* ctx);
 
```

New measurement: 2.543 million. 0.989x the previous value.
